# facebookresearch/multipathnet

Measured on NVIDIA H100. Metric: proposals/sec, higher is better.
Workload: dtype fp32 (wgmma split emulation, fp32 accumulate: 3 bf16 products per MAC, 2 fp16 products in fc6/fc7)

## Files before the change

### include/mpn_abi.h

```cpp
#ifndef MPN_ABI_H
#define MPN_ABI_H
#include <stdint.h>
#ifdef __cplusplus
extern "C" {
#endif

typedef struct mpn_ctx mpn_ctx;
typedef struct mpn_model mpn_model;

int mpn_ctx_create(int device, void *cuda_stream, mpn_ctx **out);
int mpn_ctx_create_stream(int device, int priority, mpn_ctx **out);
void *mpn_ctx_stream(const mpn_ctx *ctx);
int mpn_ctx_wait_ctx(mpn_ctx *ctx, mpn_ctx *other);
void mpn_ctx_destroy(mpn_ctx *ctx);
const char *mpn_last_error(const mpn_ctx *ctx);
int mpn_ctx_synchronize(mpn_ctx *ctx);
int64_t mpn_ctx_launch_count(const mpn_ctx *ctx);
const char *mpn_version(void);
int mpn_ctx_set_option(mpn_ctx *ctx, const char *name, int64_t value);
int mpn_ctx_profile_begin(mpn_ctx *ctx);
int mpn_ctx_profile_end(mpn_ctx *ctx, double *ms_by_cat, int64_t *launches_by_cat);
int mpn_ctx_timeline_begin(mpn_ctx *ctx, int32_t max_launches);
int mpn_ctx_timeline_end(mpn_ctx *ctx, uint64_t *stamps_min, uint64_t *stamps_max, int32_t *n_launches);

// ... 120 lines not shown
int mpn_model_detect_nms(mpn_model *m, const float *image, int32_t H, int32_t W,
                         const float *boxes, int64_t R, float im_scale, float W0, float H0,
                         float score_thresh, float nms_thr, float *scores, float *bboxes,
                         int32_t *keep_idx, int32_t *keep_counts);
int mpn_model_detect_nms_submit(mpn_model *m, const float *image, int32_t H, int32_t W,
                                const float *boxes, int64_t R, float im_scale, float W0, float H0,
                                float score_thresh, float nms_thr, float *scores, float *bboxes,
                                int32_t *keep_idx, int32_t *keep_counts, int32_t *ticket);
int mpn_model_detect_nms_submit_u8(mpn_model *m, const uint8_t *im_hwc, int32_t H0, int32_t W0,
                                   const mpn_image_transform *tf, double scale, double max_size, const float *boxes,
                                   int64_t R, float score_thresh, float nms_thr, float *scores, float *bboxes,
                                   int32_t *keep_idx, int32_t *keep_counts, int32_t *ticket);
int mpn_model_detect_nms_wait(mpn_model *m, int32_t ticket);
typedef struct mpn_test_opts {
  int32_t num_iter;
  int32_t use_rbox_scores;
  int32_t bbox_voting;
  float score_thresh;
  float nms_thr;
  float vote_thr;
  float vote_score_pow;
} mpn_test_opts;
int mpn_model_test_one(mpn_model *m, const float *image, int32_t H, int32_t W, const float *boxes, int64_t R,
                       float im_scale, float W0, float H0, const mpn_test_opts *opts, float *scores, float *bboxes,
                       int32_t *keep_idx, int32_t *keep_counts, float *voted);
int mpn_model_detect_nms_dev(mpn_model *m, const float *image_dev, int32_t H, int32_t W,
                             const float *boxes_dev, int64_t R, float im_scale, float W0, float H0,
                             float score_thresh, float nms_thr, float *scores_dev,
                             float *bboxes_dev, int32_t *keep_idx_dev, int32_t *keep_counts_dev);

int mpn_post_detect_dev(mpn_ctx *ctx, const float *scores_dev, const float *deltas_dev, const float *boxes_dev, int64_t R,
                        int32_t C, const float *mean4, const float *std4, float W0, float H0, float score_thresh,
                        float nms_thr, int32_t c_begin, int32_t c_end, float *bboxes_dev, int32_t *keep_idx_dev,
                        int32_t *keep_counts_dev);

enum { MPN_MAX_DET = 128, MPN_REC_FLOATS = 769, MPN_DIST_ID_BYTES = 128 };
int mpn_pack_detections_dev(mpn_ctx *ctx, const float *scores_dev, const float *bboxes_dev, int64_t R, int32_t C,
                            const int32_t *keep_idx_dev, const int32_t *keep_counts_dev, int64_t cap, int32_t top_k,
                            float *record_dev);
int mpn_pack_detections(mpn_ctx *ctx, const float *scores, const float *bboxes, int64_t R, int32_t C,
                        const int32_t *keep_idx, const int32_t *keep_counts, int64_t cap, int32_t top_k, float *record);
int mpn_select_boxes(mpn_ctx *ctx, const float *classes, const float *ys, int64_t R, int32_t C, const float *mean4,
                     const float *std4, float *out);
int mpn_select_boxes_dev(mpn_ctx *ctx, const float *classes_dev, const float *ys_dev, int64_t R, int32_t C,
                         const float *mean4, const float *std4, float *out_dev);
int mpn_model_set_detection_sink(mpn_model *m, float *records_dev, int64_t capacity, int32_t top_k);
int mpn_model_detection_sink_count(const mpn_model *m, int64_t *n_records);

int mpn_dist_unique_id(mpn_ctx *ctx, uint8_t *id);
int mpn_dist_init(mpn_ctx *ctx, const uint8_t *id, int32_t rank, int32_t world);
int mpn_dist_world(const mpn_ctx *ctx, int32_t *rank, int32_t *world);
int mpn_dist_all_gather_dev(mpn_ctx *ctx, const float *send_dev, int64_t n_floats, float *recv_dev);
int mpn_dist_all_gather(mpn_ctx *ctx, const float *send_dev, int64_t n_floats, float *recv_host);
int mpn_dist_destroy(mpn_ctx *ctx);
int mpn_dist_nccl_version(mpn_ctx *ctx, int32_t *version);

int mpn_coco_eval(mpn_ctx *ctx, int32_t n_images, const int64_t *image_ids, int32_t n_cats, const int64_t *cat_ids,
                  int64_t G, const int32_t *gt_img, const int32_t *gt_cat, const double *gt_box, const double *gt_area,
                  const int32_t *gt_crowd, int64_t D, const float *dets, double *precision, double *recall,
                  double *stats);

int mpn_model_get_pooled(mpn_model *m, int32_t tower, int64_t r0, int64_t n, float *out, int64_t capacity,
                         int64_t *R_total, int32_t *bins, int32_t *Ctot);
int mpn_model_get_trunk_slot(mpn_model *m, int32_t slot, float *out_nchw, int64_t capacity,
                             int32_t *C, int32_t *H, int32_t *W);
int mpn_model_get_slot_planes(mpn_model *m, int32_t tower, int32_t slot, int64_t r0, int64_t n, uint16_t *hi,
                              uint16_t *lo, uint8_t *q8, int32_t *e8, int64_t capacity, int32_t *fmt, int64_t *dims);
int mpn_model_get_head_outputs(mpn_model *m, float *cls_logits, float *bbox_raw, int64_t *R, int32_t *K);
int mpn_debug_detect_tail(mpn_ctx *ctx, const float *logits, int32_t K, int64_t R, int32_t C, int32_t do_softmax, const float *deltas,
                          const float *boxes, int32_t do_clamp, float W0, float H0, int32_t has_norm, const float *mean4,
                          const float *std4, float *scores, float *bboxes);
int mpn_model_set_conv_impl(mpn_model *m, int32_t impl);
int mpn_model_last_flops(const mpn_model *m, double *trunk_flops, double *head_flops);

int mpn_gemm_check(mpn_ctx *ctx, const float *A, const float *B, const float *bias, int64_t M,
                   int64_t N, int64_t K, int32_t relu, int32_t impl, float *C);
int mpn_gemm_bench(mpn_ctx *ctx, int64_t M, int64_t N, int64_t K, int32_t iters, double *ms_per_launch,
                   int32_t *bn, int32_t *cta_group, int32_t *splitk);
int mpn_linear_bench(mpn_ctx *ctx, int64_t M, int64_t N, int64_t K, int32_t w16, int32_t biasless, int32_t iters,
                     double *ms_per_launch, int32_t *bn, int32_t *splitk);
int mpn_conv_bench(mpn_ctx *ctx, int64_t N, int64_t Cin, int64_t H, int64_t W, int64_t Cout, int32_t k, int32_t stride,
                   int32_t pad, int32_t iters, double *ms_per_launch, int32_t *bn, int32_t *cta_group, int32_t *mode,
                   uint64_t *dbg16);
int mpn_debug_plan(int64_t N, int64_t Cin, int64_t H, int64_t W, int64_t Cout, int32_t k, int32_t stride, int32_t pad,
                   int32_t per_roi, int32_t sm_count, int32_t *out);
int mpn_debug_fp8(const float *h, int64_t n_samples, int64_t sample_elems, int32_t *e_out, uint8_t *q_out);
int mpn_conv_check(mpn_ctx *ctx, const float *x, int64_t N, int64_t Cin, int64_t H, int64_t W,
                   const float *w, const float *bias, int64_t Cout, int32_t kh, int32_t kw,
                   int32_t stride, int32_t pad, int32_t relu, int32_t impl, float *y);
int mpn_conv_check_view(mpn_ctx *ctx, const float *x, int64_t N, int64_t Cin, int64_t H, int64_t W, int64_t ld,
                        const float *w, const float *bias, int64_t Cout, int32_t kh, int32_t kw,
                        int32_t stride, int32_t pad, int32_t relu, int32_t impl, float *y);

typedef struct mpn_train_config {
  float lr, momentum, dampening, weight_decay;
  float dropout;
  float bbox_regression;
  uint64_t seed;
} mpn_train_config;
typedef struct mpn_train_spec {
  int32_t trunk_from;
  int32_t phase2;
  int32_t integral;
  int32_t n_fixed;
  const int32_t *fixed_weight;
  const float *const *fixed_scale;
} mpn_train_spec;
enum { MPN_OPTIM_SGD = 0, MPN_OPTIM_ADAM = 1, MPN_OPTIM_ADAMAX = 2, MPN_OPTIM_ADAGRAD = 3, MPN_OPTIM_RMSPROP = 4 };
typedef struct mpn_train_optim {
  int32_t method;
  double lr_decay, beta1, beta2, epsilon, alpha;
} mpn_train_optim;
int mpn_train_check_optim(const mpn_model_desc *d, const mpn_train_spec *s, const mpn_train_optim *o, char *msg, int32_t msg_cap);
int mpn_train_check(const mpn_model_desc *d, const mpn_train_spec *s, char *msg, int32_t msg_cap);
int mpn_model_train_begin_optim(mpn_model *m, const mpn_train_config *cfg, const mpn_train_spec *s, const mpn_train_optim *o);
int mpn_model_train_begin(mpn_model *m, const mpn_train_config *cfg, const mpn_train_spec *s);
int mpn_model_train_step(mpn_model *m, int32_t n_images, const float *const *images, const int32_t *image_hw,
                         const int32_t *rois_per_image, const float *boxes, const int32_t *labels, const float *bbox_targets,
                         float *losses);
int mpn_model_train_step_dev(mpn_model *m, int32_t n_images, const float *const *images_dev, const int32_t *image_hw,
                             const int32_t *rois_per_image, const float *boxes_dev, const int32_t *labels_dev,
                             const float *bbox_targets_dev, float *losses_dev);
int mpn_model_train_phase_ms(mpn_model *m, float *ms);
int mpn_model_train_select_head(mpn_model *m, int32_t k);
int mpn_model_train_set_lr(mpn_model *m, float lr);
int mpn_model_train_decay(mpn_model *m, float factor);
int mpn_model_train_get(mpn_model *m, int32_t weight, int32_t what, float *out, int64_t capacity);
int mpn_model_train_dropout_mask(mpn_model *m, int32_t tower, int32_t layer, uint8_t *out, int64_t capacity, int64_t *n_out);
int mpn_model_train_relu_gate(mpn_model *m, int32_t tower, int32_t layer, uint8_t *out, int64_t capacity, int64_t *n_out);
int mpn_model_train_outputs(mpn_model *m, float *cls_logits, float *bbox_deltas);
int mpn_model_train_trunk_slot(mpn_model *m, int32_t image, int32_t slot, float *out_nchw, int64_t capacity, int32_t *C,
                               int32_t *H, int32_t *W);
int mpn_debug_roi_backward_nhwc(mpn_ctx *ctx, const uint16_t *hi, const uint16_t *lo, int32_t H, int32_t W, int32_t C, const float *rois,
                                int64_t R, int32_t PW, int32_t PH, float scale, int32_t variant, const float *grad_out, float *grad);
int mpn_debug_pool_backward(mpn_ctx *ctx, const uint16_t *y_hi, const uint16_t *y_lo, int32_t H, int32_t W, int32_t C, const float *grad_pool,
                            float *grad);
int mpn_debug_conv_backward(mpn_ctx *ctx, int32_t n_images, const int32_t *image_hw, int32_t cin, int32_t cout, int32_t k, int32_t stride,
                            const uint16_t *x_hi, const uint16_t *x_lo, const float *g, const float *w, float *dw, float *dx);
int mpn_model_train_end(mpn_model *m);
int mpn_debug_dropout(uint64_t seed, uint32_t step, int32_t tower, int32_t layer, uint64_t elem0, int64_t n, float p, uint8_t *out);
int mpn_debug_criteria(const float *x, const float *d, const int32_t *labels, const float *t, int64_t R, int32_t C, float bbox_w,
                       float *gx, float *gd, float *losses);
int mpn_debug_sgd(float *w, const float *g, float *buf, int64_t n, float lr, float momentum, float dampening, float wd, int32_t first);
int mpn_debug_optim(float *w, const float *g, float *s1, float *s2, const float *a, int64_t n, const mpn_train_optim *o, float lr,
                    float momentum, float dampening, float wd, int64_t t);

typedef struct mpn_roidb mpn_roidb;
int mpn_roidb_create(mpn_ctx *ctx, int32_t n_images, const int64_t *ann_off, const double *ann_xywh, const double *ann_area,
                     const int32_t *ann_class, const int32_t *ann_flags, double min_area, const int64_t *prop_off,
                     const float *prop_box, const float *prop_score, int32_t best_number, double min_proposal_area,
                     int32_t num_classes, int32_t n_sets, const float *thresholds, mpn_roidb **out);
void mpn_roidb_destroy(mpn_roidb *db);
int mpn_roidb_counts(mpn_roidb *db, int32_t *counts, int64_t *n_rows);
int mpn_roidb_image_rows(mpn_roidb *db, int32_t image, float *boxes, float *overlap, int32_t *corr, int32_t *label, int64_t capacity,
                         int64_t *n_rows, int32_t *n_gt);
int mpn_roidb_list(mpn_roidb *db, int32_t set, int32_t kind, int32_t image, int32_t *rows, int64_t capacity, int64_t *n_out);
int mpn_roidb_regression_stats(mpn_roidb *db, int32_t set, int32_t n_first, float *mean, float *std_);
int mpn_sample_plan(const int32_t *n_bg, const int32_t *n_fg, int32_t n_images, uint64_t seed, uint32_t step, int32_t set, int32_t n_slots,
                    int32_t *image, int32_t *bg_src, int32_t *fg_src, int32_t *flip);
int mpn_integral_set(uint64_t seed, uint32_t step, int32_t n_sets, int32_t *set);
int mpn_train_images_size(int32_t H0, int32_t W0, double scale, double max_size, int32_t *h, int32_t *w, double *im_scale);
int mpn_roidb_sample_dev(mpn_roidb *db, int32_t set, uint64_t seed, uint32_t step, int32_t n_slots, const int32_t *bg_src,
                         const int32_t *fg_src, const int32_t *flip, const double *im_scale, const int32_t *width, int32_t bg_each,
                         int32_t fg_each, const float *mean, const float *std_, int32_t num_classes, float *boxes_dev,
                         int32_t *labels_dev, float *targets_dev, int32_t *rois_per_image);
int mpn_roidb_sample(mpn_roidb *db, int32_t set, uint64_t seed, uint32_t step, int32_t n_slots, const int32_t *plan,
// ... 32 lines not shown
```

### multipathnet_b200/_lib.py

```python
from __future__ import annotations

import ctypes as C
import os
from dataclasses import dataclass, field
from typing import List, Optional, Sequence

import numpy as np

_HERE = os.path.dirname(os.path.abspath(__file__))
LIB_PATH = os.path.join(_HERE, "libmpn_b200.so")
HEADER_PATH = os.path.join(os.path.dirname(_HERE), "include", "mpn_abi.h")

MPN_LAYER_CONV, MPN_LAYER_MAXPOOL, MPN_LAYER_AVGPOOL, MPN_LAYER_FLATTEN = 1, 2, 3, 4
MPN_MAX_DET, MPN_REC_FLOATS, MPN_DIST_ID_BYTES = 128, 769, 128
MPN_LAYER_LRN = 5


class MpnError(RuntimeError):
    pass


class CLayer(C.Structure):
    _fields_ = [(n, C.c_int32) for n in (
        "kind", "in_slot", "out_slot", "cin", "cout", "kh", "kw", "stride", "pad", "relu",
# ... 95 lines not shown
    "mpn_bbox_norm_dev": (C.c_int, [_vp, _vp, C.c_int64, C.c_int64, _vp, _vp]),
    "mpn_bbox_decode": (C.c_int, [_vp, _vp, _vp, C.c_int64, C.c_int64, _vp]),
    "mpn_roi_pool": (C.c_int, [_vp, _vp, C.c_int64, C.c_int64, C.c_int64, C.c_int64, _vp, C.c_int64,
                               C.c_int32, C.c_int32, C.c_float, C.c_int32, _vp, _vp]),
    "mpn_roi_pool_dev": (C.c_int, [_vp, _vp, C.c_int64, C.c_int64, C.c_int64, C.c_int64, _vp, C.c_int64,
                                   C.c_int32, C.c_int32, C.c_float, C.c_int32, _vp, _vp]),
    "mpn_roi_pool_backward": (C.c_int, [_vp, _vp, _vp, C.c_int64, C.c_int64, C.c_int64, C.c_int64, _vp, C.c_int64,
                                        C.c_int32, C.c_int32, C.c_float, C.c_int32, _vp]),
    "mpn_roi_pool_backward_dev": (C.c_int, [_vp, _vp, _vp, C.c_int64, C.c_int64, C.c_int64, C.c_int64, _vp, C.c_int64,
                                            C.c_int32, C.c_int32, C.c_float, C.c_int32, _vp]),
    "mpn_get_images_size": (C.c_int, [C.c_int32, C.c_int32, C.c_double, C.c_double, _i32p, _i32p, C.POINTER(C.c_double)]),
    "mpn_get_images": (C.c_int, [_vp, _vp, C.c_int32, C.c_int32, _vp, C.c_int32, C.c_int32, _vp]),
    "mpn_get_images_dev": (C.c_int, [_vp, _vp, C.c_int32, C.c_int32, _vp, C.c_int32, C.c_int32, _vp]),
    "mpn_get_images_u8": (C.c_int, [_vp, _vp, C.c_int32, C.c_int32, _vp, C.c_int32, C.c_int32, _vp]),
    "mpn_get_images_u8_dev": (C.c_int, [_vp, _vp, C.c_int32, C.c_int32, _vp, C.c_int32, C.c_int32, _vp]),
    "mpn_get_images_u8_flip": (C.c_int, [_vp, _vp, C.c_int32, C.c_int32, _vp, C.c_int32, C.c_int32, C.c_int32, _vp]),
    "mpn_get_images_u8_flip_dev": (C.c_int, [_vp, _vp, C.c_int32, C.c_int32, _vp, C.c_int32, C.c_int32, C.c_int32, _vp]),
    "mpn_roidb_create": (C.c_int, [_vp, C.c_int32, _vp, _vp, _vp, _vp, _vp, C.c_double, _vp, _vp, _vp, C.c_int32, C.c_double,
                                   C.c_int32, C.c_int32, _vp, C.POINTER(_vp)]),
    "mpn_roidb_destroy": (None, [_vp]),
    "mpn_roidb_counts": (C.c_int, [_vp, _vp, _i64p]),
    "mpn_roidb_image_rows": (C.c_int, [_vp, C.c_int32, _vp, _vp, _vp, _vp, C.c_int64, _i64p, _i32p]),
    "mpn_roidb_list": (C.c_int, [_vp, C.c_int32, C.c_int32, C.c_int32, _vp, C.c_int64, _i64p]),
    "mpn_roidb_regression_stats": (C.c_int, [_vp, C.c_int32, C.c_int32, _vp, _vp]),
    "mpn_sample_plan": (C.c_int, [_vp, _vp, C.c_int32, C.c_uint64, C.c_uint32, C.c_int32, C.c_int32, _vp, _vp, _vp, _vp]),
    "mpn_integral_set": (C.c_int, [C.c_uint64, C.c_uint32, C.c_int32, _i32p]),
    "mpn_train_images_size": (C.c_int, [C.c_int32, C.c_int32, C.c_double, C.c_double, _i32p, _i32p, C.POINTER(C.c_double)]),
    "mpn_roidb_sample_dev": (C.c_int, [_vp, C.c_int32, C.c_uint64, C.c_uint32, C.c_int32, _vp, _vp, _vp, _vp, _vp, C.c_int32, C.c_int32,
                                       _vp, _vp, C.c_int32, _vp, _vp, _vp, _vp]),
    "mpn_roidb_sample": (C.c_int, [_vp, C.c_int32, C.c_uint64, C.c_uint32, C.c_int32, _vp, _vp, _vp, _vp, C.c_double, C.c_double,
                                   C.c_int32, C.c_int32, _vp, _vp, C.c_int32, _vp, _vp]),
    "mpn_roidb_batch_host": (C.c_int, [_vp, _vp, _vp, _vp, _vp]),
    "mpn_model_train_step_batch": (C.c_int, [_vp, _vp, _vp]),
    "mpn_debug_attach_proposals": (C.c_int, [C.c_int64, _vp, _vp, _vp, _vp, C.c_double, C.c_int64, _vp, _vp, C.c_int32, C.c_double,
                                             C.c_int32, _vp, _vp, _vp, _vp, C.c_int64, _i64p, _i32p]),
    "mpn_debug_sample_rows": (C.c_int, [C.c_int64, _vp, _vp, _vp, C.c_double, C.c_int32, C.c_int32, _vp, _vp, C.c_int32, _vp, _vp]),
    "mpn_model_detect_nms_submit_u8": (C.c_int, [_vp, _vp, C.c_int32, C.c_int32, _vp, C.c_double, C.c_double, _vp, C.c_int64, C.c_float, C.c_float,
                                                 _vp, _vp, _vp, _vp, _i32p]),
    "mpn_model_trunk_image": (C.c_int, [_vp, _vp, C.c_int32, C.c_int32, _vp, C.c_double, C.c_double, C.POINTER(C.c_double), _i32p, _i32p]),
    "mpn_model_create": (C.c_int, [_vp, C.POINTER(CModelDesc), C.POINTER(_vp), _i64p, C.c_int32, C.POINTER(_vp)]),
    "mpn_model_destroy": (None, [_vp]),
    "mpn_model_trunk": (C.c_int, [_vp, _vp, C.c_int32, C.c_int32]),
    "mpn_model_trunk_dev": (C.c_int, [_vp, _vp, C.c_int32, C.c_int32]),
    "mpn_model_heads": (C.c_int, [_vp, _vp, C.c_int64, _vp, _vp]),
    "mpn_model_heads_dev": (C.c_int, [_vp, _vp, C.c_int64, _vp, _vp]),
    "mpn_model_detect": (C.c_int, [_vp, _vp, C.c_int32, C.c_int32, _vp, C.c_int64, C.c_float, C.c_int32, _vp, _vp]),
    "mpn_model_detect_nms": (C.c_int, [_vp, _vp, C.c_int32, C.c_int32, _vp, C.c_int64, C.c_float, C.c_float,
                                       C.c_float, C.c_float, C.c_float, _vp, _vp, _vp, _vp]),
    "mpn_model_detect_nms_submit": (C.c_int, [_vp, _vp, C.c_int32, C.c_int32, _vp, C.c_int64, C.c_float, C.c_float,
                                              C.c_float, C.c_float, C.c_float, _vp, _vp, _vp, _vp, _i32p]),
    "mpn_model_detect_nms_wait": (C.c_int, [_vp, C.c_int32]),
    "mpn_model_test_one": (C.c_int, [_vp, _vp, C.c_int32, C.c_int32, _vp, C.c_int64, C.c_float, C.c_float, C.c_float, C.POINTER(CTestOpts),
                                     _vp, _vp, _vp, _vp, _vp]),
    "mpn_model_detect_nms_dev": (C.c_int, [_vp, _vp, C.c_int32, C.c_int32, _vp, C.c_int64, C.c_float, C.c_float,
                                           C.c_float, C.c_float, C.c_float, _vp, _vp, _vp, _vp]),
    "mpn_post_detect_dev": (C.c_int, [_vp, _vp, _vp, _vp, C.c_int64, C.c_int32, _vp, _vp, C.c_float, C.c_float, C.c_float, C.c_float,
                                      C.c_int32, C.c_int32, _vp, _vp, _vp]),
    "mpn_pack_detections_dev": (C.c_int, [_vp, _vp, _vp, C.c_int64, C.c_int32, _vp, _vp, C.c_int64, C.c_int32, _vp]),
    "mpn_pack_detections": (C.c_int, [_vp, _vp, _vp, C.c_int64, C.c_int32, _vp, _vp, C.c_int64, C.c_int32, _vp]),
    "mpn_select_boxes": (C.c_int, [_vp, _vp, _vp, C.c_int64, C.c_int32, _vp, _vp, _vp]),
    "mpn_select_boxes_dev": (C.c_int, [_vp, _vp, _vp, C.c_int64, C.c_int32, _vp, _vp, _vp]),
    "mpn_model_set_detection_sink": (C.c_int, [_vp, _vp, C.c_int64, C.c_int32]),
    "mpn_model_detection_sink_count": (C.c_int, [_vp, _i64p]),
    "mpn_dist_unique_id": (C.c_int, [_vp, _vp]),
    "mpn_dist_init": (C.c_int, [_vp, _vp, C.c_int32, C.c_int32]),
    "mpn_dist_world": (C.c_int, [_vp, _i32p, _i32p]),
    "mpn_dist_all_gather_dev": (C.c_int, [_vp, _vp, C.c_int64, _vp]),
    "mpn_dist_all_gather": (C.c_int, [_vp, _vp, C.c_int64, _vp]),
    "mpn_dist_destroy": (C.c_int, [_vp]),
    "mpn_dist_nccl_version": (C.c_int, [_vp, _i32p]),
    "mpn_coco_eval": (C.c_int, [_vp, C.c_int32, _vp, C.c_int32, _vp, C.c_int64, _vp, _vp, _vp, _vp, _vp, C.c_int64, _vp, _vp, _vp, _vp]),
    "mpn_model_get_pooled":(C.c_int, [_vp, C.c_int32, C.c_int64, C.c_int64, _vp, C.c_int64, _i64p, _i32p, _i32p]),
    "mpn_model_get_trunk_slot": (C.c_int, [_vp, C.c_int32, _vp, C.c_int64, _i32p, _i32p, _i32p]),
    "mpn_model_get_slot_planes": (C.c_int, [_vp, C.c_int32, C.c_int32, C.c_int64, C.c_int64, _vp, _vp, _vp, _vp, C.c_int64, _i32p, _i64p]),
    "mpn_model_get_head_outputs": (C.c_int, [_vp, _vp, _vp, _i64p, _i32p]),
    "mpn_debug_detect_tail": (C.c_int, [_vp, _vp, C.c_int32, C.c_int64, C.c_int32, C.c_int32, _vp, _vp, C.c_int32, C.c_float, C.c_float,
                                        C.c_int32, _vp, _vp, _vp, _vp]),
    "mpn_model_set_conv_impl": (C.c_int, [_vp, C.c_int32]),
    "mpn_model_last_flops": (C.c_int, [_vp, C.POINTER(C.c_double), C.POINTER(C.c_double)]),
    "mpn_gemm_bench": (C.c_int, [_vp, C.c_int64, C.c_int64, C.c_int64, C.c_int32, C.POINTER(C.c_double), _i32p, _i32p, _i32p]),
    "mpn_linear_bench": (C.c_int, [_vp, C.c_int64, C.c_int64, C.c_int64, C.c_int32, C.c_int32, C.c_int32, C.POINTER(C.c_double), _i32p, _i32p]),
    "mpn_conv_bench": (C.c_int, [_vp, C.c_int64, C.c_int64, C.c_int64, C.c_int64, C.c_int64, C.c_int32, C.c_int32, C.c_int32, C.c_int32,
                                 C.POINTER(C.c_double), _i32p, _i32p, _i32p, C.POINTER(C.c_uint64)]),
    "mpn_debug_plan": (C.c_int, [C.c_int64, C.c_int64, C.c_int64, C.c_int64, C.c_int64, C.c_int32, C.c_int32, C.c_int32, C.c_int32, C.c_int32, _i32p]),
    "mpn_debug_fp8": (C.c_int, [_vp, C.c_int64, C.c_int64, _vp, _vp]),
    "mpn_gemm_check": (C.c_int, [_vp, _vp, _vp, _vp, C.c_int64, C.c_int64, C.c_int64, C.c_int32, C.c_int32, _vp]),
    "mpn_conv_check": (C.c_int, [_vp, _vp, C.c_int64, C.c_int64, C.c_int64, C.c_int64, _vp, _vp, C.c_int64,
                                 C.c_int32, C.c_int32, C.c_int32, C.c_int32, C.c_int32, C.c_int32, _vp]),
    "mpn_conv_check_view": (C.c_int, [_vp, _vp, C.c_int64, C.c_int64, C.c_int64, C.c_int64, C.c_int64, _vp, _vp, C.c_int64,
                                      C.c_int32, C.c_int32, C.c_int32, C.c_int32, C.c_int32, C.c_int32, _vp]),
    "mpn_train_check": (C.c_int, [C.POINTER(CModelDesc), C.POINTER(CTrainSpec), C.c_char_p, C.c_int32]),
    "mpn_model_train_begin": (C.c_int, [_vp, C.POINTER(CTrainConfig), C.POINTER(CTrainSpec)]),
    "mpn_train_check_optim": (C.c_int, [C.POINTER(CModelDesc), C.POINTER(CTrainSpec), C.POINTER(CTrainOptim), C.c_char_p, C.c_int32]),
    "mpn_model_train_begin_optim": (C.c_int, [_vp, C.POINTER(CTrainConfig), C.POINTER(CTrainSpec), C.POINTER(CTrainOptim)]),
    "mpn_model_train_step": (C.c_int, [_vp, C.c_int32, C.POINTER(_vp), _i32p, _i32p, _vp, _vp, _vp, _vp]),
    "mpn_model_train_step_dev": (C.c_int, [_vp, C.c_int32, C.POINTER(_vp), _i32p, _i32p, _vp, _vp, _vp, _vp]),
    "mpn_model_train_phase_ms": (C.c_int, [_vp, _f32p]),
    "mpn_model_train_select_head": (C.c_int, [_vp, C.c_int32]),
    "mpn_model_train_set_lr": (C.c_int, [_vp, C.c_float]),
    "mpn_model_train_decay": (C.c_int, [_vp, C.c_float]),
    "mpn_model_train_get": (C.c_int, [_vp, C.c_int32, C.c_int32, _vp, C.c_int64]),
    "mpn_model_train_dropout_mask": (C.c_int, [_vp, C.c_int32, C.c_int32, _vp, C.c_int64, _i64p]),
    "mpn_model_train_relu_gate": (C.c_int, [_vp, C.c_int32, C.c_int32, _vp, C.c_int64, _i64p]),
    "mpn_model_train_outputs": (C.c_int, [_vp, _vp, _vp]),
    "mpn_model_train_trunk_slot": (C.c_int, [_vp, C.c_int32, C.c_int32, _vp, C.c_int64, _i32p, _i32p, _i32p]),
    "mpn_model_train_end": (C.c_int, [_vp]),
    "mpn_debug_roi_backward_nhwc": (C.c_int, [_vp, _vp, _vp, C.c_int32, C.c_int32, C.c_int32, _vp, C.c_int64, C.c_int32, C.c_int32, C.c_float,
                                              C.c_int32, _vp, _vp]),
    "mpn_model_train_phase2": (C.c_int, [_vp, C.c_float]),
    "mpn_model_train_set": (C.c_int, [_vp, C.c_int32, C.c_int32, _vp, C.c_int64]),
    "mpn_model_train_get_state": (C.c_int, [_vp, C.POINTER(CTrainState)]),
    "mpn_model_train_set_state": (C.c_int, [_vp, C.POINTER(CTrainState)]),
    "mpn_debug_roi_backward_jobs": (C.c_int, [_vp, _vp, _vp, C.c_int32, C.c_int32, C.c_int32, _vp, C.c_int64, C.c_int32, C.c_int32, C.c_int32,
                                              C.c_int32, _i32p, _f32p, _i32p, _i64p, _i32p, C.POINTER(_vp), _vp, _vp, _vp]),
    "mpn_debug_pool_backward": (C.c_int, [_vp, _vp, _vp, C.c_int32, C.c_int32, C.c_int32, _vp, _vp]),
    "mpn_debug_conv_backward": (C.c_int, [_vp, C.c_int32, _i32p, C.c_int32, C.c_int32, C.c_int32, C.c_int32, _vp, _vp, _vp, _vp, _vp,
                                          _vp]),
    "mpn_debug_dropout": (C.c_int, [C.c_uint64, C.c_uint32, C.c_int32, C.c_int32, C.c_uint64, C.c_int64, C.c_float, _vp]),
    "mpn_debug_criteria": (C.c_int, [_vp, _vp, _vp, _vp, C.c_int64, C.c_int32, C.c_float, _vp, _vp, _vp]),
    "mpn_debug_sgd": (C.c_int, [_vp, _vp, _vp, C.c_int64, C.c_float, C.c_float, C.c_float, C.c_float, C.c_int32]),
    "mpn_debug_optim": (C.c_int, [_vp, _vp, _vp, _vp, _vp, C.c_int64, C.POINTER(CTrainOptim), C.c_float, C.c_float, C.c_float, C.c_float,
                                  C.c_int64]),
}

_lib = None


def load_library():
    global _lib
    if _lib is not None:
        return _lib
    if not os.path.exists(LIB_PATH):
        raise MpnError(
            f"{LIB_PATH} is missing: build it with `make` (or `python -c 'import __graft_entry__ as g; g.build()'`). "
            "There is no CPU or PyTorch fallback for this path.")
    lib = C.CDLL(LIB_PATH)
    for name, (res, args) in SIGNATURES.items():
        fn = getattr(lib, name)
        fn.restype = res
        fn.argtypes = args
    _lib = lib
    return lib


def _ptr(a) -> Optional[int]:
    if a is None:
        return None
    if isinstance(a, int):
        return a
    if isinstance(a, np.ndarray):
        return a.ctypes.data
    if hasattr(a, "data_ptr"):
        return a.data_ptr()
    raise TypeError(f"cannot take the address of {type(a)}")


def _f32(a) -> np.ndarray:
    return np.ascontiguousarray(a, dtype=np.float32)


class Context:

    def __init__(self, device: int = 0, stream: Optional[int] = None, own_stream: bool = False, priority: int = 0):
        self.lib = load_library()
        h = _vp()
        if own_stream:
# ... 166 lines not shown
        out = np.empty((3, h.value, w.value), np.float32)
        tf = CImageTransform.of(kind)
        self.check(self.lib.mpn_get_images(self.h, _ptr(im), im.shape[1], im.shape[2], C.addressof(tf), h.value, w.value, _ptr(out)),
                   "mpn_get_images")
        return out, float(s.value)

    def get_images_u8(self, im_hwc_u8, kind: str, scale: float = 600, max_size: float = 1000):
        im = np.ascontiguousarray(im_hwc_u8, dtype=np.uint8)
        if im.ndim != 3 or im.shape[2] != 3:
            raise ValueError("expected an H x W x 3 uint8 image")
        h, w, s = C.c_int32(), C.c_int32(), C.c_double()
        self.check(self.lib.mpn_get_images_size(im.shape[0], im.shape[1], float(scale), float(max_size), C.byref(h), C.byref(w), C.byref(s)),
                   "mpn_get_images_size")
        out = np.empty((3, h.value, w.value), np.float32)
        tf = CImageTransform.of(kind)
        self.check(self.lib.mpn_get_images_u8(self.h, _ptr(im), im.shape[0], im.shape[1], C.addressof(tf), h.value, w.value, _ptr(out)),
                   "mpn_get_images_u8")
        return out, float(s.value)

    def bbox_norm(self, deltas, mean, std) -> np.ndarray:
        d = _f32(deltas).copy()
        m, s = _f32(mean).reshape(4), _f32(std).reshape(4)
        self.check(self.lib.mpn_bbox_norm(self.h, _ptr(d), d.shape[0], d.shape[1], _ptr(m), _ptr(s)), "mpn_bbox_norm")
        return d

    def bbox_decode(self, deltas, boxes) -> np.ndarray:
        d, b = _f32(deltas), _f32(boxes)
        out = np.empty_like(d)
        self.check(self.lib.mpn_bbox_decode(self.h, _ptr(d), _ptr(b), d.shape[0], d.shape[1] // 4, _ptr(out)), "mpn_bbox_decode")
        return out

    def roi_pool(self, fmap, rois, pw: int, ph: int, scale: float, variant: int = 2, with_argmax: bool = False):
        f, r = _f32(fmap), _f32(rois)
        n, c, h, w = f.shape
        out = np.empty((r.shape[0], c, ph, pw), dtype=np.float32)
        am = np.empty(out.shape, dtype=np.int32) if with_argmax else None
        self.check(self.lib.mpn_roi_pool(self.h, _ptr(f), n, c, h, w, _ptr(r), r.shape[0], pw, ph, float(scale), variant,
                                         _ptr(out), _ptr(am)), "mpn_roi_pool")
        return (out, am) if with_argmax else out

    def roi_pool_backward(self, grad_out, argmax, rois, data_shape, pw: int, ph: int, scale: float, variant: int = 2) -> np.ndarray:
        g, r = _f32(grad_out), _f32(rois)
        am = np.ascontiguousarray(argmax, dtype=np.int32)
        n, c, h, w = (int(s) for s in data_shape)
        if g.shape != (r.shape[0], c, ph, pw) or am.shape != g.shape:
            raise ValueError(f"grad_out and argmax must be {(r.shape[0], c, ph, pw)}, got {g.shape} and {am.shape}")
        out = np.empty((n, c, h, w), dtype=np.float32)
        self.check(self.lib.mpn_roi_pool_backward(self.h, _ptr(g), _ptr(am), n, c, h, w, _ptr(r), r.shape[0], pw, ph, float(scale),
                                                  variant, _ptr(out)), "mpn_roi_pool_backward")
        return out

    def roi_pool_backward_dev(self, grad_out_dev, argmax_dev, N: int, C_: int, H: int, W: int, rois_dev, R: int, pw: int, ph: int,
                              scale: float, variant: int, grad_data_dev):
        self.check(self.lib.mpn_roi_pool_backward_dev(self.h, _ptr(grad_out_dev), _ptr(argmax_dev), int(N), int(C_), int(H), int(W),
                                                      _ptr(rois_dev), int(R), int(pw), int(ph), float(scale), int(variant),
                                                      _ptr(grad_data_dev)), "mpn_roi_pool_backward_dev")

    def gemm_check(self, A, B, bias=None, relu=False, impl=0) -> np.ndarray:
        A, B = _f32(A), _f32(B)
        m, k = A.shape
        n = B.shape[0]
        bias = None if bias is None else _f32(bias)
        out = np.empty((m, n), dtype=np.float32)
        self.check(self.lib.mpn_gemm_check(self.h, _ptr(A), _ptr(B), _ptr(bias), m, n, k, int(relu), impl, _ptr(out)), "mpn_gemm_check")
        return out

    def gemm_bench(self, M, N, K, iters=20):
        ms = C.c_double(); bn = C.c_int32(); cg = C.c_int32(); sk = C.c_int32()
        self.check(self.lib.mpn_gemm_bench(self.h, M, N, K, iters, C.byref(ms), C.byref(bn), C.byref(cg), C.byref(sk)), "mpn_gemm_bench")
        return ms.value, bn.value, cg.value, sk.value

    def linear_bench(self, M, N, K, w16=False, biasless=False, iters=20):
        ms = C.c_double(); bn = C.c_int32(); sk = C.c_int32()
        self.check(self.lib.mpn_linear_bench(self.h, M, N, K, int(w16), int(biasless), iters, C.byref(ms), C.byref(bn), C.byref(sk)),
                   "mpn_linear_bench")
        return ms.value, bn.value, sk.value

    def conv_bench(self, N, Cin, H, W, Cout, k=3, stride=1, pad=1, iters=20):
        ms = C.c_double(); bn = C.c_int32(); cg = C.c_int32(); mode = C.c_int32(); dbg = (C.c_uint64 * 16)()
        self.check(self.lib.mpn_conv_bench(self.h, N, Cin, H, W, Cout, k, stride, pad, iters, C.byref(ms), C.byref(bn), C.byref(cg),
                                           C.byref(mode), dbg), "mpn_conv_bench")
        return ms.value, bn.value, cg.value, mode.value, [int(x) for x in dbg]

    def conv_check(self, x, w, bias=None, stride=1, pad=0, relu=False, impl=0) -> np.ndarray:
        x, w = _f32(x), _f32(w)
        n, cin, h, ww = x.shape
        cout, _, kh, kw = w.shape
        bias = None if bias is None else _f32(bias)
        ho, wo = (h + 2 * pad - kh) // stride + 1, (ww + 2 * pad - kw) // stride + 1
        y = np.empty((n, cout, ho, wo), dtype=np.float32)
        self.check(self.lib.mpn_conv_check(self.h, _ptr(x), n, cin, h, ww, _ptr(w), _ptr(bias), cout, kh, kw, stride, pad,
                                           int(relu), impl, _ptr(y)), "mpn_conv_check")
        return y

    def conv_check_view(self, x, w, ld, bias=None, stride=1, pad=0, relu=False, impl=0) -> np.ndarray:
        x, w = _f32(x), _f32(w)
        n, cin, h, ww = x.shape
        cout, _, kh, kw = w.shape
        bias = None if bias is None else _f32(bias)
        ho, wo = (h + 2 * pad - kh) // stride + 1, (ww + 2 * pad - kw) // stride + 1
        y = np.empty((n, cout, ho, wo), dtype=np.float32)
        self.check(self.lib.mpn_conv_check_view(self.h, _ptr(x), n, cin, h, ww, int(ld), _ptr(w), _ptr(bias), cout, kh, kw, stride,
                                                pad, int(relu), impl, _ptr(y)), "mpn_conv_check_view")
        return y


@dataclass
class Layer:
    kind: int
    in_slot: int
    out_slot: int
    cin: int = 0
    cout: int = 0
    kh: int = 1
    kw: int = 1
    stride: int = 1
    pad: int = 0
    relu: int = 0
    residual_slot: int = -1
    ceil_mode: int = 0
    weight: int = -1
    bias: int = -1
    groups: int = 1

    def to_c(self) -> CLayer:
        if self.groups != 1 or self.kind == MPN_LAYER_LRN:
            raise MpnError("grouped convolution / LRN (CaffeNet, BASELINE configs[0]) is the CPU plumbing configuration; "
                           "it is not part of the GPU path")
        return CLayer(self.kind, self.in_slot, self.out_slot, self.cin, self.cout, self.kh, self.kw, self.stride,
                      self.pad, self.relu, self.residual_slot, self.ceil_mode, self.weight, self.bias)


@dataclass
class Tower:
    region: int
    levels: List[tuple]
    pooled_w: int
    pooled_h: int
    normalize: int
    layers: List[Layer]
    out_slot: int


@dataclass
class Head:
    col_begin: int
    col_len: int
    cout: int
    weight: int
    bias: int

    def to_c(self) -> CHead:
        return CHead(self.col_begin, self.col_len, self.cout, self.weight, self.bias)


@dataclass
class ModelSpec:
    name: str
    trunk_layers: List[Layer]
    towers: List[Tower]
    cls_heads: List[Head]
    bbox_head: Head
    num_classes: int
    weights: List[np.ndarray]
    roi_variant: int = 2
    no_softmax: int = 0
# ... 242 lines not shown
```

### multipathnet_b200/csrc/abi.cu

```cuda
#include "conv_gemm.cuh"
#include "roi.cuh"
#include <algorithm>
#include <mutex>

int mpn_nms_launch(mpn_ctx *, const float *, int, int, const int32_t *, const int32_t *, float, int32_t *, int32_t *);
int mpn_nms_dense_launch(mpn_ctx *, const float *, int, float, int32_t *, int32_t *);
int mpn_bbox_vote_launch(mpn_ctx *, const float *, int, const float *, int, float, float *);
int mpn_pack_detections_launch(mpn_ctx *, const float *, const float *, int, const int32_t *, const int32_t *, int, int, float *);
int mpn_gather_scored_range_launch(mpn_ctx *, const float *, const float *, int, int, int, int, float, float *, int32_t *, int32_t *);
int mpn_bbox_norm_decode_launch(mpn_ctx *, const float *, const float *, int64_t, int, int, float, float, float *, const float *, const float *);
int mpn_detect_tail_launch(mpn_ctx *, const float *, int64_t, int, int, int, float *, const float *, const float *, int, float, float,
                           float *, int, const float *, const float *);
int mpn_select_boxes_launch(mpn_ctx *, const float *, const float *, int64_t, int, const float *, const float *, float *);
int mpn_foveal_launch(mpn_ctx *, const float *, int64_t, float *);
int mpn_context_region_launch(mpn_ctx *, const float *, int64_t, float, float *);
int mpn_get_images_launch(mpn_ctx *, const float *, int32_t, int32_t, const mpn_image_transform *, int32_t, int32_t, float *);
int mpn_get_images_size_impl(int32_t, int32_t, double, double, int32_t *, int32_t *, double *);
int mpn_get_images_u8_launch(mpn_ctx *, const uint8_t *, int32_t, int32_t, const mpn_image_transform *, int32_t, int32_t, float *);
int mpn_get_images_u8_flip_launch(mpn_ctx *, const uint8_t *, int32_t, int32_t, const mpn_image_transform *, int32_t, int32_t, int32_t, float *);
int mpn_bbox_norm_launch(mpn_ctx *, float *, int64_t, int64_t, const float *, const float *);
int mpn_bbox_decode_launch(mpn_ctx *, const float *, const float *, int64_t, int, int, float, float, float *);
int mpn_split_rows_launch(mpn_ctx *, const float *, int64_t, int64_t, int64_t, __nv_bfloat16 *, __nv_bfloat16 *, int64_t);
int mpn_nchw_to_nhwc_split_launch(mpn_ctx *, const float *, int, int, int, int, DTensor &);
int mpn_nhwc_split_to_nchw_launch(mpn_ctx *, const DTensor &, float *);
// ... 725 lines not shown
  MPN_CUDA(ctx, cudaMemsetAsync(a.at<char>(o_bh), 0x3c, 2 * nb, ctx->stream));
  MPN_CUDA(ctx, cudaMemsetAsync(a.at<char>(o_bl), 0x30, 2 * nb, ctx->stream));
  ConvProblem p;
  p.x.hi = a.at<__nv_bfloat16>(o_ah); p.x.lo = a.at<__nv_bfloat16>(o_al); p.x.N = M; p.x.H = 1; p.x.W = 1; p.x.C = K; p.x.ld = K;
  p.w_hi = a.at<__nv_bfloat16>(o_bh); p.w_lo = a.at<__nv_bfloat16>(o_bl); p.Cout = (int)N; p.relu = 1;
  p.bf16 = ctx->opt_bf16 == 1 ? 1 : 0;
  p.m_invariant = per_roi; p.fill_split = fill_split;
  if (w16) {
    MPN_CHECK_ARG(ctx, !p.bf16, "the bf16 numerics do not take an fp16 weight plane");
    p.x.fmt = 1; p.w16 = p.w_hi; p.w16_inv_scale = 1.f; p.w_hi = p.w_lo = nullptr;
  }
  const int64_t Npad = (N + 7) / 8 * 8;
  (void)Npad;
  if (N % 8 == 0) { p.y.hi = a.at<__nv_bfloat16>(o_ch); p.y.lo = a.at<__nv_bfloat16>(o_cl); }
  else { p.y.f32 = a.at<float>(o_ch); }
  p.y.N = M; p.y.H = 1; p.y.W = 1; p.y.C = N; p.y.ld = N; p.y_f32_ld = N;
  if (!(N % 8 == 0)) MPN_CHECK_ARG(ctx, 4 * nc <= 2 * (2 * nc + 64), "internal");
  ConvPlan pl;
  MPN_TRY(conv_tc_plan(ctx, p, pl));
  if (bn) *bn = pl.BN; if (cta_group) *cta_group = 1; if (splitk) *splitk = pl.splitk;
  for (int i = 0; i < 3; ++i) MPN_TRY(conv_tc_launch(ctx, p, pl));
  cudaEvent_t e0, e1;
  MPN_CUDA(ctx, cudaEventCreate(&e0)); MPN_CUDA(ctx, cudaEventCreate(&e1));
  MPN_CUDA(ctx, cudaEventRecord(e0, ctx->stream));
  for (int i = 0; i < iters; ++i) MPN_TRY(conv_tc_launch(ctx, p, pl));
  MPN_CUDA(ctx, cudaEventRecord(e1, ctx->stream));
  MPN_CUDA(ctx, cudaEventSynchronize(e1));
  float ms = 0.f;
  MPN_CUDA(ctx, cudaEventElapsedTime(&ms, e0, e1));
  cudaEventDestroy(e0); cudaEventDestroy(e1);
  *ms_per_launch = (double)ms / iters;
  return MPN_OK;
}

int mpn_gemm_bench(mpn_ctx *ctx, int64_t M, int64_t N, int64_t K, int32_t iters, double *ms_per_launch, int32_t *bn,
                   int32_t *cta_group, int32_t *splitk) {
  return gemm_bench_impl(ctx, M, N, K, 0, 0, 0, iters, ms_per_launch, bn, cta_group, splitk);
}

int mpn_linear_bench(mpn_ctx *ctx, int64_t M, int64_t N, int64_t K, int32_t w16, int32_t biasless, int32_t iters,
                     double *ms_per_launch, int32_t *bn, int32_t *splitk) {
  return gemm_bench_impl(ctx, M, N, K, 1, w16 ? 1 : 0, biasless ? 1 : 0, iters, ms_per_launch, bn, nullptr, splitk);
}

int mpn_conv_bench(mpn_ctx *ctx, int64_t N, int64_t Cin, int64_t H, int64_t W, int64_t Cout, int32_t k, int32_t stride,
                   int32_t pad, int32_t iters, double *ms_per_launch, int32_t *bn, int32_t *cta_group, int32_t *mode,
                   uint64_t *dbg16) {
  if (!ctx) return MPN_ERR_ARG;
  MPN_CUDA(ctx, cudaSetDevice(ctx->device));
  MPN_CHECK_ARG(ctx, N > 0 && Cin % 8 == 0 && Cout % 8 == 0 && iters > 0 && ms_per_launch, "bad arguments");
  const int64_t Ho = (H + 2 * pad - k) / stride + 1, Wo = (W + 2 * pad - k) / stride + 1;
  const size_t nx = (size_t)(N * H * W * Cin), nw = (size_t)(Cout * conv_k_pad(Cin) * k * k), ny = (size_t)(N * Ho * Wo * Cout);
  Arena a{ctx};
  size_t o_xh = a.reserve(2 * nx), o_xl = a.reserve(2 * nx), o_wh = a.reserve(2 * nw), o_wl = a.reserve(2 * nw),
         o_yh = a.reserve(2 * ny), o_yl = a.reserve(2 * ny);
  MPN_TRY(a.commit());
  MPN_CUDA(ctx, cudaMemsetAsync(a.at<char>(o_xh), 0x3c, 2 * nx, ctx->stream));
  MPN_CUDA(ctx, cudaMemsetAsync(a.at<char>(o_xl), 0x30, 2 * nx, ctx->stream));
  MPN_CUDA(ctx, cudaMemsetAsync(a.at<char>(o_wh), 0x3c, 2 * nw, ctx->stream));
  MPN_CUDA(ctx, cudaMemsetAsync(a.at<char>(o_wl), 0x30, 2 * nw, ctx->stream));
  ConvProblem p;
  p.x.hi = a.at<__nv_bfloat16>(o_xh); p.x.lo = a.at<__nv_bfloat16>(o_xl); p.x.N = N; p.x.H = H; p.x.W = W; p.x.C = Cin; p.x.ld = Cin;
  p.w_hi = a.at<__nv_bfloat16>(o_wh); p.w_lo = a.at<__nv_bfloat16>(o_wl); p.Cout = (int)Cout; p.kh = k; p.kw = k; p.stride = stride; p.pad = pad; p.relu = 1;
  p.bf16 = ctx->opt_bf16 == 1 ? 1 : 0;
  p.y.hi = a.at<__nv_bfloat16>(o_yh); p.y.lo = a.at<__nv_bfloat16>(o_yl); p.y.N = N; p.y.H = Ho; p.y.W = Wo; p.y.C = Cout; p.y.ld = Cout;
  ConvPlan pl;
  MPN_TRY(conv_tc_plan(ctx, p, pl));
  if (bn) *bn = pl.BN; if (cta_group) *cta_group = 1; if (mode) *mode = pl.mode;
  for (int i = 0; i < 3; ++i) MPN_TRY(conv_tc_launch(ctx, p, pl));
  cudaEvent_t e0, e1;
  MPN_CUDA(ctx, cudaEventCreate(&e0)); MPN_CUDA(ctx, cudaEventCreate(&e1));
  MPN_CUDA(ctx, cudaEventRecord(e0, ctx->stream));
  for (int i = 0; i < iters; ++i) MPN_TRY(conv_tc_launch(ctx, p, pl));
  MPN_CUDA(ctx, cudaEventRecord(e1, ctx->stream));
  MPN_CUDA(ctx, cudaEventSynchronize(e1));
  float ms = 0.f;
  MPN_CUDA(ctx, cudaEventElapsedTime(&ms, e0, e1));
  cudaEventDestroy(e0); cudaEventDestroy(e1);
  *ms_per_launch = (double)ms / iters;
  if (dbg16) memset(dbg16, 0, 128);
  return MPN_OK;
}

int mpn_gemm_check(mpn_ctx *ctx, const float *A, const float *B, const float *bias, int64_t M, int64_t N, int64_t K,
                   int32_t relu, int32_t impl, float *C) {
  if (!ctx) return MPN_ERR_ARG;
  MPN_CUDA(ctx, cudaSetDevice(ctx->device));
  MPN_CHECK_ARG(ctx, A && B && C && M > 0 && N > 0 && K > 0, "bad arguments");
  MPN_CHECK_ARG(ctx, !(ctx->opt_fp8 == 1 && ctx->opt_bf16 == 1), "the \"fp8\" and \"bf16\" options are both on");
  const size_t na = (size_t)(M * K), nb = (size_t)(N * K), nc = (size_t)(M * N);
  const int64_t Kp = conv_k_pad(K);
  const size_t nbp = (size_t)(N * Kp);
  Arena a{ctx};
  size_t o_a = a.reserve(4 * na), o_b = a.reserve(4 * nb), o_bias = a.reserve(4 * (size_t)N), o_c = a.reserve(4 * nc),
         o_ah = a.reserve(2 * na), o_al = a.reserve(2 * na), o_bh = a.reserve(2 * nbp), o_bl = a.reserve(2 * nbp),
         o_a8 = a.reserve(na), o_ae = a.reserve(4 * (size_t)M), o_b8 = a.reserve(nbp), o_be = a.reserve(4 * (size_t)(N + 127) / 128 * 128);
  MPN_TRY(a.commit());
  MPN_CUDA(ctx, cudaMemcpyAsync(a.at<float>(o_a), A, 4 * na, cudaMemcpyHostToDevice, ctx->stream));
  MPN_CUDA(ctx, cudaMemcpyAsync(a.at<float>(o_b), B, 4 * nb, cudaMemcpyHostToDevice, ctx->stream));
  if (bias) MPN_CUDA(ctx, cudaMemcpyAsync(a.at<float>(o_bias), bias, 4 * (size_t)N, cudaMemcpyHostToDevice, ctx->stream));
  MPN_TRY(mpn_split_rows_launch(ctx, a.at<float>(o_a), M, K, K, a.at<__nv_bfloat16>(o_ah), a.at<__nv_bfloat16>(o_al), K));
  if (Kp != K) {
    MPN_CUDA(ctx, cudaMemsetAsync(a.at<__nv_bfloat16>(o_bh), 0, 2 * nbp, ctx->stream));
    MPN_CUDA(ctx, cudaMemsetAsync(a.at<__nv_bfloat16>(o_bl), 0, 2 * nbp, ctx->stream));
  }
  MPN_TRY(mpn_split_rows_launch(ctx, a.at<float>(o_b), N, K, K, a.at<__nv_bfloat16>(o_bh), a.at<__nv_bfloat16>(o_bl), Kp));
  ConvProblem p;
  p.x.hi = a.at<__nv_bfloat16>(o_ah); p.x.lo = a.at<__nv_bfloat16>(o_al); p.x.N = M; p.x.H = 1; p.x.W = 1; p.x.C = K; p.x.ld = K;
  p.w_hi = a.at<__nv_bfloat16>(o_bh); p.w_lo = a.at<__nv_bfloat16>(o_bl); p.bias = bias ? a.at<float>(o_bias) : nullptr;
  p.Cout = (int)N; p.relu = relu; p.bf16 = ctx->opt_bf16 == 1 ? 1 : 0;
  p.m_invariant = 1;
  p.y.f32 = a.at<float>(o_c); p.y.N = M; p.y.H = 1; p.y.W = 1; p.y.C = N; p.y.ld = N; p.y_f32_ld = N;
  if (ctx->opt_fp8 == 1 && impl != 2) {
    p.fp8 = 1;
    p.x8 = a.at<uint8_t>(o_a8); p.x8_exp = a.at<int>(o_ae); p.w8 = a.at<uint8_t>(o_b8); p.w8_exp = a.at<int>(o_be);
    MPN_TRY(mpn_fp8_quantize_launch(ctx, p.x, a.at<uint8_t>(o_a8), a.at<int>(o_ae)));
    MPN_TRY(mpn_fp8_weight_launch(ctx, p.w_hi, N, Kp, (N + 127) / 128 * 128, a.at<uint8_t>(o_b8), a.at<int>(o_be)));
  }
  if (impl == 1) { MPN_TRY(conv_ref_launch(ctx, p)); }
  else {
    if (impl == 2) {
      float amax = 0.f;
      MPN_TRY(mpn_absmax(ctx, a.at<float>(o_b), (int64_t)nb, &amax));
      int e = 0;
      if (amax > 0.f) { (void)frexpf(amax, &e); e = 14 - e; }
      const float sc = ldexpf(1.0f, e);
      MPN_TRY(mpn_weight_permute_half_launch(ctx, a.at<float>(o_b), N, (int)K, 1, 1, sc, a.at<void>(o_bh)));
      p.w16 = a.at<void>(o_bh); p.w16_inv_scale = 1.0f / sc; p.w_hi = p.w_lo = nullptr;
      MPN_TRY(mpn_split_rows_f16_launch(ctx, a.at<float>(o_a), M, K, K, a.at<__nv_bfloat16>(o_ah), a.at<__nv_bfloat16>(o_al), K));
      p.x.fmt = 1; p.bf16 = 0;
    }
    ConvPlan pl; MPN_TRY(conv_tc_plan(ctx, p, pl)); MPN_TRY(conv_tc_launch(ctx, p, pl));
  }
  MPN_CUDA(ctx, cudaMemcpyAsync(C, a.at<float>(o_c), 4 * nc, cudaMemcpyDeviceToHost, ctx->stream));
  if (ctx->opt_fp8 == 1) MPN_TRY(mpn_ovf_copy_async(ctx, ctx->stream));
  MPN_CUDA(ctx, cudaStreamSynchronize(ctx->stream));
  return ctx->opt_fp8 == 1 ? mpn_ovf_test(ctx) : MPN_OK;
}

}
```

### multipathnet_b200/csrc/conv_gemm.cuh

```cuda
#pragma once
#include "common.cuh"
#include <cuda.h>

struct OutSeg { int c0, c1; float *ptr; long long ld; };
struct OutScatter { int n = 0; OutSeg seg[8]; };

enum class OperandScheme : int { BF16X3 = 0, FP16X2 = 1, BF16X1 = 2, FP8X1 = 3 };

struct ConvProblem {
  DTensor x;
  const __nv_bfloat16 *w_hi = nullptr, *w_lo = nullptr;
  const float *bias = nullptr;
  int Cout = 0, kh = 1, kw = 1, stride = 1, pad = 0;
  int relu = 0;
  DTensor res;
  DTensor y;
  int64_t y_f32_ld = 0;
  DTensor pool;
  int pool_only = 0;
  int m_invariant = 0;
  const void *w16 = nullptr; float w16_inv_scale = 1.f;
  int bf16 = 0;
  int fp8 = 0;
  const uint8_t *x8 = nullptr; const int *x8_exp = nullptr;
  const uint8_t *w8 = nullptr; const int *w8_exp = nullptr;
  OutScatter scatter;
  int wide_k_split = 0;
  int fill_split = 0;
};

struct ConvPlan {
  CUtensorMap tmA_hi, tmA_lo, tmB_hi, tmB_lo;
  int BN = 0;
  int tn = 0, th = 0, tw = 0;
  int tiles_img = 0, tiles_h = 0, tiles_w = 0, tiles_n = 0;
  int splitk = 1, kb_per_split = 0;
  int mode = 0;
  int flat = 0;
  OperandScheme ops = OperandScheme::BF16X3;
  int valid = 0;
};

int conv_tc_plan(mpn_ctx *ctx, const ConvProblem &p, ConvPlan &plan);
int conv_tc_launch(mpn_ctx *ctx, const ConvProblem &p, const ConvPlan &plan);
int conv_ref_launch(mpn_ctx *ctx, const ConvProblem &p);
int conv_direct_nchw_launch(mpn_ctx *ctx, const float *x_nchw, int N, int Cin, int H, int W, const float *w,
                            const float *bias, int Cout, int kh, int kw, int stride, int pad, int relu,
                            DTensor &y, const float *w_host = nullptr, const float *bias_host = nullptr);
int conv1_tc_launch(mpn_ctx *ctx, const float *x_nchw, int N, int H, int W, const float *w_dev, const float *bias_dev, int relu,
                    DTensor &y);
double conv_flops(const ConvProblem &p);
int mpn_fp8_quantize_launch(mpn_ctx *ctx, const DTensor &x, uint8_t *q8, int *exps);
int mpn_fp8_weight_launch(mpn_ctx *ctx, const __nv_bfloat16 *w_hi, int64_t rows, int64_t K, int64_t rows_pad, uint8_t *q8, int *exps);
```

### multipathnet_b200/csrc/gemm_tc.cu

```cuda
#include "conv_gemm.cuh"
#include "wgmma.cuh"
#include "fp8_e4m3.cuh"
#include <algorithm>
#include <stdlib.h>
#include <string.h>

namespace {

constexpr int BM = 128;
constexpr int BK = 64;
constexpr int TC_THREADS = 384;
constexpr int CONS_THREADS = 256;
constexpr int A_TILE_BYTES = BM * BK * 2;
constexpr int SMEM_BUDGET = 196608;

__host__ __device__ constexpr int a_planes(OperandScheme ops) { return (ops == OperandScheme::BF16X1 || ops == OperandScheme::FP8X1) ? 1 : 2; }
__host__ __device__ constexpr int b_planes(OperandScheme ops) { return ops == OperandScheme::BF16X3 ? 2 : 1; }
__host__ __device__ constexpr int elem_bytes(OperandScheme ops) { return ops == OperandScheme::FP8X1 ? 1 : 2; }
__host__ __device__ constexpr int row_bytes(int BN, OperandScheme ops) { return (ops == OperandScheme::FP8X1 || BN == 256) ? 64 : 128; }
__host__ __device__ constexpr int stage_k(int BN, OperandScheme ops) { return row_bytes(BN, ops) / elem_bytes(ops); }
__host__ __device__ constexpr int kb_steps(int BN, OperandScheme ops) { return BK / stage_k(BN, ops); }
__host__ __device__ constexpr int a_tile_bytes(int BN, OperandScheme ops) { return BM * row_bytes(BN, ops); }
__host__ __device__ constexpr int stage_bytes(int BN, OperandScheme ops = OperandScheme::BF16X3) {
  return (a_planes(ops) * BM + b_planes(ops) * BN) * row_bytes(BN, ops);
// ... 375 lines not shown
        const int s = it % S; const uint32_t ph = (uint32_t)(it / S) & 1u;
        mbar_wait(full_bar(s), ph);
        if (it == 0 && e == 0) tl_min_stamp(p.tl_min, 2);
        const uint32_t sa = smem_base + (uint32_t)s * STAGE;
        auto desc = [](uint32_t a) { return row_bytes(BN, OPS) == 64 ? make_smem_desc_64b(a) : make_smem_desc(a); };
        const uint64_t a_hi = desc(sa + (uint32_t)g * (A_TILE / 2));
        const uint64_t a_lo = desc(sa + A_TILE + (uint32_t)g * (A_TILE / 2));
        const uint64_t b_hi = desc(sa + B_OFF);
        const uint64_t b_lo = desc(sa + B_OFF + B_TILE_BYTES);
        wgmma_fence_acc(acc);
        wgmma_fence();
        mma_kstep<BN, OPS>(acc, a_hi, a_lo, b_hi, b_lo, i == 0);
        wgmma_commit();
        wgmma_wait<1>();
        wgmma_fence_acc(acc);
        if (i > 0 && lane == 0) mbar_arrive(empty_bar((it - 1) % S));
      }
      wgmma_wait<0>();
      wgmma_fence_acc(acc);
      if (lane == 0) mbar_arrive(empty_bar((it - 1) % S));
    }
    if (e == 0) tl_max_stamp(p.tl_max, 0);
    const uint32_t t_epi = (p.tl_max && e == 0) ? (uint32_t)gtimer() : 0u;
    tile_epilogue<BN, OPS>(p, u, acc, g, wq, lane, so);
    if (e == 0) {
      tl_max_stamp(p.tl_max, 1);
      if (p.tl_max) atomicAdd(p.tl_max + 3, (unsigned long long)((uint32_t)gtimer() - t_epi));
    }
  }
}


constexpr int C1_THREADS = 256;
constexpr int C1_A_BYTES = 2 * A_TILE_BYTES;
constexpr int C1_B_BYTES = 2 * 64 * 128;
constexpr int C1_OUT_WARP = 16 * 128;
constexpr int C1_SMEM = 2 * C1_A_BYTES + C1_B_BYTES + (C1_THREADS / 32) * C1_OUT_WARP + 1024;

__device__ __forceinline__ void conv1_gather(const float *__restrict__ x, int pix, int pixels, int H, int W, int bhalf,
                                             float (&in)[16]) {
#pragma unroll
  for (int k = 0; k < 16; ++k) in[k] = 0.f;
  if (pix < pixels) {
    const int HW = H * W;
    const int n = pix / HW, rem = pix - n * HW;
    const int ho = rem / W, wo = rem - ho * W;
    const float *x0 = x + ((size_t)n * 3 * HW + (size_t)(ho - 1) * W + (wo - 1));
    const bool rok[3] = {ho >= 1, true, ho + 1 < H}, cok[3] = {wo >= 1, true, wo + 1 < W};
#pragma unroll
    for (int k = 0; k < 16; ++k) {
      const int kk = 16 * bhalf + k;
      if (kk < 27) {
        const int ci = kk / 9, r = (kk / 3) % 3, q = kk % 3;
        in[k] = (rok[r] && cok[q]) ? __ldg(x0 + ci * HW + r * W + q) : 0.f;
      }
    }
  }
}

__device__ __forceinline__ void conv1_store_plane(uint32_t so, const uint32_t (&v)[16], __nv_bfloat16 *out, int pix0,
                                                  int pixels, int lane) {
  const int r = lane >> 2;
  const uint32_t wr = so + (uint32_t)(r * 128 + 4 * (lane & 3));
  __syncwarp();
#pragma unroll
  for (int j = 0; j < 8; ++j) {
    const uint32_t a = wr + (uint32_t)((j ^ r) * 16);
    asm volatile("st.shared.b32 [%0], %1;" ::"r"(a), "r"(v[j]) : "memory");
    asm volatile("st.shared.b32 [%0], %1;" ::"r"(a + 8 * 128), "r"(v[8 + j]) : "memory");
  }
  __syncwarp();
  const int row0 = lane >> 3, ch = lane & 7;
  const uint32_t rd0 = so + (uint32_t)(row0 * 128 + ((ch ^ row0) * 16)), rd1 = so + (uint32_t)(row0 * 128 + ((ch ^ row0 ^ 4) * 16));
  __nv_bfloat16 *o = out + (size_t)(pix0 + row0) * 64 + ch * 8;
#pragma unroll
  for (int q = 0; q < 4; ++q) {
    uint4 d;
    asm volatile("ld.shared.v4.b32 {%0, %1, %2, %3}, [%4];" : "=r"(d.x), "=r"(d.y), "=r"(d.z), "=r"(d.w)
                 : "r"(((q & 1) ? rd1 : rd0) + (uint32_t)(q * 4 * 128)) : "memory");
    if (pix0 + row0 + 4 * q < pixels) *reinterpret_cast<uint4 *>(o + q * 4 * 64) = d;
  }
}

__global__ void __launch_bounds__(C1_THREADS, 2)
conv1_tc_kernel(const float *__restrict__ x, int N, int H, int W, const float *__restrict__ w, const float *__restrict__ bias,
                int relu, __nv_bfloat16 *__restrict__ out_hi, __nv_bfloat16 *__restrict__ out_lo) {
  extern __shared__ uint8_t smem_raw[];
  uint8_t *smem = reinterpret_cast<uint8_t *>((reinterpret_cast<uintptr_t>(smem_raw) + 1023) & ~(uintptr_t)1023);
  uint8_t *sB = smem + 2 * C1_A_BYTES;
  const int tid = threadIdx.x, lane = tid & 31, warp = tid >> 5;
  const uint32_t so = smem_u32(sB + C1_B_BYTES) + (uint32_t)(warp * C1_OUT_WARP);
  const uint32_t b_base = smem_u32(sB);
  const int g = tid >> 7;
  const int pixels = N * H * W;
  const int total_tiles = (pixels + BM - 1) / BM;
  asm volatile("griddepcontrol.wait;" ::: "memory");
  asm volatile("griddepcontrol.launch_dependents;" ::: "memory");
  const int c0 = 2 * (lane & 3);
  for (int i = tid; i < 64 * 4; i += C1_THREADS) {
    const int row = i >> 2, j = i & 3;
    uint32_t hh[4], ll[4];
#pragma unroll
    for (int q = 0; q < 4; ++q) {
      const int k0 = j * 8 + 2 * q;
      const float v0 = (k0 < 27) ? __ldg(w + row * 27 + k0) : 0.f, v1 = (k0 + 1 < 27) ? __ldg(w + row * 27 + k0 + 1) : 0.f;
      split_bf16x2(v0, v1, hh[q], ll[q]);
    }
    const uint32_t off = (uint32_t)row * 128u + (uint32_t)((j ^ (row & 7)) * 16);
    *reinterpret_cast<uint4 *>(sB + off) = make_uint4(hh[0], hh[1], hh[2], hh[3]);
    *reinterpret_cast<uint4 *>(sB + 64 * 128 + off) = make_uint4(ll[0], ll[1], ll[2], ll[3]);
  }
  const int brow = tid & 127, bhalf = tid >> 7;
  float in[16];
  conv1_gather(x, (int)blockIdx.x * BM + brow, pixels, H, W, bhalf, in);
  for (int tile = blockIdx.x, it = 0; tile < total_tiles; tile += gridDim.x, ++it) {
    uint8_t *sa = smem + (it & 1) * C1_A_BYTES;
    uint8_t *pa = sa + (size_t)brow * 128;
#pragma unroll
    for (int jj = 0; jj < 2; ++jj) {
      const int j = 2 * bhalf + jj;
      uint32_t hh[4], ll[4];
#pragma unroll
      for (int q = 0; q < 4; ++q) split_bf16x2(in[jj * 8 + 2 * q], in[jj * 8 + 2 * q + 1], hh[q], ll[q]);
      const int pj = (j ^ (brow & 7)) * 16;
      *reinterpret_cast<uint4 *>(pa + pj) = make_uint4(hh[0], hh[1], hh[2], hh[3]);
      *reinterpret_cast<uint4 *>(pa + A_TILE_BYTES + pj) = make_uint4(ll[0], ll[1], ll[2], ll[3]);
    }
    asm volatile("fence.proxy.async.shared::cta;" ::: "memory");
    __syncthreads();
    float acc[32];
#pragma unroll
    for (int i = 0; i < 32; ++i) acc[i] = 0.f;
    const uint32_t a_base = smem_u32(sa);
    const uint64_t a_hi = make_smem_desc(a_base + (uint32_t)g * (A_TILE_BYTES / 2));
    const uint64_t a_lo = make_smem_desc(a_base + A_TILE_BYTES + (uint32_t)g * (A_TILE_BYTES / 2));
    const uint64_t b_hi = make_smem_desc(b_base), b_lo = make_smem_desc(b_base + 64 * 128);
    wgmma_fence_acc(acc);
    wgmma_fence();
#pragma unroll
    for (int k = 0; k < 2; ++k) {
      const uint64_t adv = (uint64_t)((k * 16 * 2) >> 4);
      wgmma_nk16<64, false>(acc, a_lo + adv, b_hi + adv, k ? 1u : 0u);
      wgmma_nk16<64, false>(acc, a_hi + adv, b_lo + adv, 1u);
      wgmma_nk16<64, false>(acc, a_hi + adv, b_hi + adv, 1u);
    }
    wgmma_commit();
    const int next = tile + (int)gridDim.x;
    conv1_gather(x, next < total_tiles ? next * BM + brow : pixels, pixels, H, W, bhalf, in);
    wgmma_wait<0>();
    wgmma_fence_acc(acc);
#pragma unroll
    for (int j = 0; j < 8; ++j) {
      const float2 b = __ldg(reinterpret_cast<const float2 *>(bias + 8 * j + c0));
#pragma unroll
      for (int h = 0; h < 2; ++h) {
        float &f0 = acc[4 * j + 2 * h], &f1 = acc[4 * j + 2 * h + 1];
        f0 += b.x; f1 += b.y;
        if (relu) { f0 = fmaxf(f0, 0.f); f1 = fmaxf(f1, 0.f); }
      }
    }
    const int pix0 = tile * BM + 64 * g + 16 * (warp & 3);
#pragma unroll 1
    for (int plane = 0; plane < 2; ++plane) {
      uint32_t v[16];
#pragma unroll
      for (int j = 0; j < 8; ++j)
#pragma unroll
        for (int h = 0; h < 2; ++h) {
          uint32_t hi2, lo2;
          split_bf16x2(acc[4 * j + 2 * h], acc[4 * j + 2 * h + 1], hi2, lo2);
          v[8 * h + j] = plane ? lo2 : hi2;
        }
      conv1_store_plane(so, v, plane ? out_lo : out_hi, pix0, pixels, lane);
    }
  }
}

struct ReduceParams {
  const float *ws; long long split_stride; int splitk; long long pixels; int Cout;
  const float *bias; const __nv_bfloat16 *res_hi, *res_lo; long long res_ld; int relu;
  __nv_bfloat16 *out_hi, *out_lo; long long out_ld; float *out_f32; long long out_f32_ld;
  OutScatter scatter;
};
__global__ void __launch_bounds__(256) splitk_reduce_kernel(const ReduceParams r) {
  MPN_PDL_SYNC();
  const long long idx = (long long)blockIdx.x * blockDim.x + threadIdx.x;
  if (idx >= r.pixels * r.Cout) return;
  const long long pix = idx / r.Cout; const int c = (int)(idx - pix * r.Cout);
  float acc = 0.f;
  for (int s = 0; s < r.splitk; ++s) acc += r.ws[(long long)s * r.split_stride + idx];
  if (r.bias) acc += __ldg(r.bias + c);
  if (r.res_hi) acc += join_bf16(r.res_hi[pix * r.res_ld + c], r.res_lo[pix * r.res_ld + c]);
  if (r.relu) acc = fmaxf(acc, 0.f);
  if (r.out_hi) { __nv_bfloat16 h, l; split_bf16(acc, h, l); r.out_hi[pix * r.out_ld + c] = h; r.out_lo[pix * r.out_ld + c] = l; }
  if (r.scatter.n > 0) {
#pragma unroll 1
    for (int g = 0; g < r.scatter.n; ++g)
      if (c >= r.scatter.seg[g].c0 && c < r.scatter.seg[g].c1) { r.scatter.seg[g].ptr[pix * r.scatter.seg[g].ld + (c - r.scatter.seg[g].c0)] = acc; break; }
  } else if (r.out_f32) r.out_f32[pix * r.out_f32_ld + c] = acc;
}

typedef CUresult (*PFN_encodeTiled)(CUtensorMap *, CUtensorMapDataType, cuuint32_t, void *, const cuuint64_t *,
                                    const cuuint64_t *, const cuuint32_t *, const cuuint32_t *, CUtensorMapInterleave,
                                    CUtensorMapSwizzle, CUtensorMapL2promotion, CUtensorMapFloatOOBfill);
PFN_encodeTiled get_encode_fn() {
  static PFN_encodeTiled fn = nullptr;
  if (!fn) {
    void *p = nullptr; cudaDriverEntryPointQueryResult q;
    if (cudaGetDriverEntryPoint("cuTensorMapEncodeTiled", &p, cudaEnableDefault, &q) == cudaSuccess &&
        q == cudaDriverEntryPointSuccess)
      fn = reinterpret_cast<PFN_encodeTiled>(p);
  }
  return fn;
}

int encode_map(mpn_ctx *ctx, CUtensorMap *tm, const void *base, int rank, const cuuint64_t *dims,
               const cuuint64_t *strides_bytes , const cuuint32_t *box, const cuuint32_t *estr, int BN, OperandScheme ops) {
  const bool fp8 = ops == OperandScheme::FP8X1;
  PFN_encodeTiled fn = get_encode_fn();
  if (!fn) return mpn_fail(ctx, MPN_ERR_CUDA, "cuTensorMapEncodeTiled entry point unavailable");
  CUresult r = fn(tm, fp8 ? CU_TENSOR_MAP_DATA_TYPE_UINT8 : CU_TENSOR_MAP_DATA_TYPE_BFLOAT16, (cuuint32_t)rank, const_cast<void *>(base), dims,
                  strides_bytes, box, estr, CU_TENSOR_MAP_INTERLEAVE_NONE, row_bytes(BN, ops) == 64 ? CU_TENSOR_MAP_SWIZZLE_64B : CU_TENSOR_MAP_SWIZZLE_128B,
                  CU_TENSOR_MAP_L2_PROMOTION_L2_256B, CU_TENSOR_MAP_FLOAT_OOB_FILL_NONE);
  if (r != CUDA_SUCCESS) {
    char b[256];
    snprintf(b, sizeof b, "cuTensorMapEncodeTiled failed (%d): rank %d dims %llu %llu box %u %u", (int)r, rank,
             (unsigned long long)dims[0], (unsigned long long)dims[1], box[0], box[1]);
    return mpn_fail(ctx, MPN_ERR_CUDA, b);
  }
  return MPN_OK;
}

inline bool tc_use_pdl() {
  static const int on = [] { const char *e = getenv("MPN_TC_PDL"); return (e && e[0] == '0') ? 0 : 1; }();
  return on != 0;
}

template <int BN, OperandScheme OPS = OperandScheme::BF16X3>
int launch_bn(mpn_ctx *ctx, const ConvPlan &pl, const TcParams &tp) {
  const int smem = tc_smem_bytes(BN, OPS);
  constexpr int bslot = BN == 256 ? 2 : (BN == 128 ? 1 : 0);
  constexpr int slot = OPS == OperandScheme::FP16X2 ? 3 : (OPS == OperandScheme::BF16X1 ? 5 + bslot
                                                         : (OPS == OperandScheme::FP8X1 ? 8 + bslot : bslot));
  if (!ctx->tc_attr_set[slot]) {
    MPN_CUDA(ctx, cudaFuncSetAttribute(conv_gemm_tc_kernel<BN, OPS>, cudaFuncAttributeMaxDynamicSharedMemorySize, smem));
    ctx->tc_attr_set[slot] = 1;
  }
  const long long units = (long long)pl.tiles_img * pl.tiles_h * pl.tiles_w * pl.tiles_n * pl.splitk;
  MPN_CHECK_ARG(ctx, units > 0 && units < (1ll << 31), "conv_tc: grid size out of range");
  TcParams tpu = tp;
  tpu.units = (int)units;
  cudaLaunchConfig_t cfg = {};
  cfg.gridDim = dim3((unsigned)std::min<long long>(units, ctx->sm_count));
  cfg.blockDim = dim3(TC_THREADS); cfg.dynamicSmemBytes = (size_t)smem; cfg.stream = ctx->stream;
  cudaLaunchAttribute attr[1];
  int na = 0;
  if (tc_use_pdl()) {
    attr[na].id = cudaLaunchAttributeProgrammaticStreamSerialization;
    attr[na].val.programmaticStreamSerializationAllowed = 1;
    ++na;
  }
  cfg.attrs = attr; cfg.numAttrs = na;
  MPN_CUDA(ctx, cudaLaunchKernelEx(&cfg, conv_gemm_tc_kernel<BN, OPS>, pl.tmA_hi, pl.tmA_lo, pl.tmB_hi, pl.tmB_lo, tpu));
  MPN_LAUNCHED(ctx);
  return MPN_OK;
}

int launch_ops(mpn_ctx *ctx, const ConvPlan &pl, const TcParams &tp) {
  if (pl.ops == OperandScheme::FP16X2) return launch_bn<256, OperandScheme::FP16X2>(ctx, pl, tp);
  if (pl.ops == OperandScheme::FP8X1)
    return pl.BN == 128 ? launch_bn<128, OperandScheme::FP8X1>(ctx, pl, tp) : launch_bn<64, OperandScheme::FP8X1>(ctx, pl, tp);
  if (pl.ops == OperandScheme::BF16X1) {
    switch (pl.BN) {
      case 256: return launch_bn<256, OperandScheme::BF16X1>(ctx, pl, tp);
      case 128: return launch_bn<128, OperandScheme::BF16X1>(ctx, pl, tp);
      default: return launch_bn<64, OperandScheme::BF16X1>(ctx, pl, tp);
    }
  }
  switch (pl.BN) {
    case 256: return launch_bn<256>(ctx, pl, tp);
    case 128: return launch_bn<128>(ctx, pl, tp);
    default: return launch_bn<64>(ctx, pl, tp);
  }
}

}

int conv1_tc_launch(mpn_ctx *ctx, const float *x_nchw, int N, int H, int W, const float *w_dev, const float *bias_dev, int relu,
                    DTensor &y) {
  MPN_CHECK_ARG(ctx, y.hi && y.lo && y.C == 64 && y.ld % 8 == 0, "conv1_tc: output must be 64-channel split planes");
  MPN_CHECK_ARG(ctx, bias_dev, "conv1_tc: bias missing");
  MPN_CHECK_ARG(ctx, y.ld == 64 && (long long)N * H * W < (1ll << 31) - 256, "conv1_tc: dense 64-channel output and < 2^31 pixels");
  if (!ctx->tc_attr_set[4]) {
    MPN_CUDA(ctx, cudaFuncSetAttribute(conv1_tc_kernel, cudaFuncAttributeMaxDynamicSharedMemorySize, C1_SMEM));
    ctx->tc_attr_set[4] = 1;
  }
  const long long tiles = ((long long)N * H * W + BM - 1) / BM;
  cudaLaunchConfig_t cfg = {};
  cfg.gridDim = dim3((unsigned)std::min<long long>(tiles, 2ll * ctx->sm_count)); cfg.blockDim = dim3(C1_THREADS);
  cfg.dynamicSmemBytes = (size_t)C1_SMEM; cfg.stream = ctx->stream;
  cudaLaunchAttribute attr[1];
  int na = 0;
  if (tc_use_pdl()) { attr[na].id = cudaLaunchAttributeProgrammaticStreamSerialization; attr[na].val.programmaticStreamSerializationAllowed = 1; ++na; }
  cfg.attrs = attr; cfg.numAttrs = na;
  MPN_CUDA(ctx, cudaLaunchKernelEx(&cfg, conv1_tc_kernel, x_nchw, N, H, W, w_dev, bias_dev, relu, y.hi, y.lo));
  MPN_LAUNCHED(ctx);
  return MPN_OK;
}

double conv_flops(const ConvProblem &p) {
  const double Ho = (double)p.y.H, Wo = (double)p.y.W;
  return 2.0 * (double)p.x.C * p.Cout * p.kh * p.kw * Ho * Wo * (double)p.y.N;
}

static int conv_tc_plan_impl(mpn_ctx *ctx, int sm_count, const ConvProblem &p, ConvPlan &pl, bool choose_only) {
  pl.valid = 0;
  MPN_CHECK_ARG(ctx, choose_only || (p.x.hi && (p.x.lo || p.bf16) && ((p.w_hi && (p.w_lo || p.bf16)) || p.w16)),
                "conv_tc: operands must be split-bf16 (or an fp16 weight plane)");
  MPN_CHECK_ARG(ctx, !(p.w16 && p.bf16), "conv_tc: the bf16 numerics do not take an fp16 weight plane");
  MPN_CHECK_ARG(ctx, !(p.fp8 && (p.w16 || p.bf16)), "conv_tc: the fp8 numerics take neither an fp16 weight plane nor the bf16 numerics");
  MPN_CHECK_ARG(ctx, choose_only || !p.fp8 || (p.x8 && p.x8_exp && p.w8 && p.w8_exp), "conv_tc: the fp8 numerics need e4m3 planes and exponents");
  pl.ops = p.w16 ? OperandScheme::FP16X2 : (p.fp8 ? OperandScheme::FP8X1 : (p.bf16 ? OperandScheme::BF16X1 : OperandScheme::BF16X3));
  const bool w16 = pl.ops == OperandScheme::FP16X2, fp8 = pl.ops == OperandScheme::FP8X1;
  MPN_CHECK_ARG(ctx, choose_only || (p.x.fmt == 1) == w16, "conv_tc: fp16 activation planes go with the fp16 weight plane (and only with it)");
  MPN_CHECK_ARG(ctx, p.x.C % 8 == 0, "conv_tc: Cin must be a multiple of 8");
  MPN_CHECK_ARG(ctx, !fp8 || p.x.C % BK == 0, "conv_tc: the fp8 numerics need Cin a multiple of 64 (their quantizer groups are 64 channels wide)");
  MPN_CHECK_ARG(ctx, !w16 || p.x.C % BK == 0, "conv_tc: the fp16-weight path needs Cin a multiple of 64");
  const int cblocks = (int)(conv_k_pad(p.x.C) / BK);
  MPN_CHECK_ARG(ctx, p.x.ld % 8 == 0, "conv_tc: input pixel stride must be a multiple of 8 elements");
  MPN_CHECK_ARG(ctx, p.stride >= 1 && p.stride <= 2, "conv_tc: stride must be 1 or 2");
  const int Ho = (int)p.y.H, Wo = (int)p.y.W, N = (int)p.y.N;
  pl.flat = (p.kh == 1 && p.kw == 1 && p.stride == 1 && p.pad == 0) ? 1 : 0;
  pl.mode = 0; pl.splitk = 1;
  cuuint64_t dims[4], strides[3]; cuuint32_t box[4], estr[4];
  int gtn = 1, gth = 1, gtw = BM;
  if (!pl.flat) {
    double best = -1.0;
    for (int tw = 1; tw <= 128; tw <<= 1)
      for (int th = 1; th * tw <= 128; th <<= 1) {
        const int tn = 128 / (tw * th);
        if (tw * p.stride > 256 || th * p.stride > 256) continue;
        const long long tiles = (long long)((Wo + tw - 1) / tw) * ((Ho + th - 1) / th) * ((N + tn - 1) / tn);
        const double util = (double)N * Ho * Wo / (double)(tiles * 128) + 1e-6 * tw;
        if (util > best) { best = util; gtn = tn; gth = th; gtw = tw; }
      }
  }
  const long long P = (long long)p.x.N * p.x.H * p.x.W;
  {
    const bool r3_ok = (p.kh == 3 && p.kw == 3 && p.stride == 1 && p.pad == 1);
    const char *env3 = getenv("MPN_TC_R3");
    const char *env3m = getenv("MPN_TC_R3_MINPIX");
    const long long r3_minpix = env3m ? atoll(env3m) : 0;
    pl.mode = (r3_ok && !(env3 && env3[0] == '0') && P >= r3_minpix) ? 1 : 0;
  }
  const long long tiles_m = pl.flat ? (P + BM - 1) / BM
                                    : (pl.mode ? (long long)((Wo + 7) / 8) * ((Ho + 15) / 16) * N
                                               : (long long)((Wo + gtw - 1) / gtw) * ((Ho + gth - 1) / gth) * ((N + gtn - 1) / gtn));
  {
    const int taps = p.kh * p.kw;
    const double kblocks = (double)taps * (double)cblocks;
    double best = 1e300; int best_bn = 64;
    for (int bi = 0; bi < 3; ++bi) {
      const int bn = bi == 0 ? 256 : (bi == 1 ? 128 : 64);
      if (w16 && bn != 256) continue;
      if (fp8 && bn == 256) continue;
      if (!p.m_invariant && bn > 64 && bn > ((p.Cout + 63) / 64) * 64) continue;
      const int roi_bn = p.Cout > 128 ? 256 : (p.Cout > 64 ? 128 : 64);
      if (p.m_invariant && bn != (fp8 ? std::min(roi_bn, 128) : roi_bn)) continue;
      const long long units = tiles_m * ((p.Cout + bn - 1) / bn);
      const long long rounds = (units + sm_count - 1) / sm_count;
      const double mma = (w16 ? 2.0 : (pl.ops == OperandScheme::BF16X1 ? 1.0 : (fp8 ? 0.5 : 3.0))) * 128.0 * bn * 64.0 / 1024.0;
      const double ingest = ((double)a_planes(pl.ops) * 128 + (double)b_planes(pl.ops) * bn) * (fp8 ? 64.0 : 128.0) / 48.0;
      const double cost = (double)rounds * (kblocks * std::max(mma, ingest) + 1500.0 + 8.0 * bn);
      if (cost < best * 0.999) { best = cost; best_bn = bn; }
    }
    pl.BN = best_bn;
    pl.tiles_n = (p.Cout + pl.BN - 1) / pl.BN;
  }
  if (pl.flat) {
    pl.tn = 1; pl.th = 1; pl.tw = BM;
    pl.tiles_img = 1; pl.tiles_h = 1; pl.tiles_w = (int)((P + BM - 1) / BM);
    dims[0] = (cuuint64_t)p.x.C; dims[1] = (cuuint64_t)P; dims[2] = 1; dims[3] = 1;
    strides[0] = (cuuint64_t)p.x.ld * 2; strides[1] = (cuuint64_t)P * p.x.ld * 2; strides[2] = strides[1];
    box[0] = (cuuint32_t)stage_k(pl.BN, pl.ops); box[1] = BM; box[2] = 1; box[3] = 1;
    estr[0] = estr[1] = estr[2] = estr[3] = 1;
  } else {
    if (pl.mode == 1) { pl.tn = 1; pl.th = 16; pl.tw = 8; }
    else { pl.tn = gtn; pl.th = gth; pl.tw = gtw; }
// ... 29 lines not shown
  if (fp8) {
    const cuuint64_t C8 = (cuuint64_t)p.x.C;
    if (pl.flat) { strides[0] = C8; strides[1] = (cuuint64_t)P * C8; strides[2] = strides[1]; }
    else { strides[0] = C8; strides[1] = (cuuint64_t)p.x.W * C8; strides[2] = (cuuint64_t)p.x.H * p.x.W * C8; }
    bs[0] = (cuuint64_t)Ktot;
    MPN_TRY(encode_map(ctx, &pl.tmA_hi, p.x8, 4, dims, strides, box, estr, pl.BN, pl.ops));
    MPN_TRY(encode_map(ctx, &pl.tmB_hi, p.w8, 2, bd, bs, bb, be, pl.BN, pl.ops));
    pl.tmA_lo = pl.tmA_hi; pl.tmB_lo = pl.tmB_hi;
    pl.valid = 1;
    return MPN_OK;
  }
  MPN_TRY(encode_map(ctx, &pl.tmA_hi, p.x.hi, 4, dims, strides, box, estr, pl.BN, pl.ops));
  if (a_planes(pl.ops) == 2) { MPN_TRY(encode_map(ctx, &pl.tmA_lo, p.x.lo, 4, dims, strides, box, estr, pl.BN, pl.ops)); }
  else pl.tmA_lo = pl.tmA_hi;
  if (w16) {
    MPN_CHECK_ARG(ctx, pl.mode == 0 && pl.flat && pl.BN == 256, "conv_tc: the fp16-weight path is for wide flat GEMMs");
    MPN_TRY(encode_map(ctx, &pl.tmB_hi, p.w16, 2, bd, bs, bb, be, pl.BN, pl.ops));
    pl.tmB_lo = pl.tmB_hi;
  } else {
    MPN_TRY(encode_map(ctx, &pl.tmB_hi, p.w_hi, 2, bd, bs, bb, be, pl.BN, pl.ops));
    if (b_planes(pl.ops) == 2) { MPN_TRY(encode_map(ctx, &pl.tmB_lo, p.w_lo, 2, bd, bs, bb, be, pl.BN, pl.ops)); }
    else pl.tmB_lo = pl.tmB_hi;
  }
  pl.valid = 1;
  return MPN_OK;
}

int conv_tc_plan(mpn_ctx *ctx, const ConvProblem &p, ConvPlan &pl) { return conv_tc_plan_impl(ctx, ctx->sm_count, p, pl, false); }

int conv_tc_launch(mpn_ctx *ctx, const ConvProblem &p, const ConvPlan &pl) {
  MpnProfScope prof_scope__(ctx, MPN_CAT_CONV_TC);
  MPN_CHECK_ARG(ctx, pl.valid, "conv_tc_launch: invalid plan");
  TcParams tp;
  memset(&tp, 0, sizeof(tp));
  if (pl.flat) { tp.N = 1; tp.Ho = 1; tp.Wo = (int)(p.y.N * p.y.H * p.y.W); }
  else { tp.N = (int)p.y.N; tp.Ho = (int)p.y.H; tp.Wo = (int)p.y.W; }
  tp.Cout = p.Cout; tp.kh = p.kh; tp.kw = p.kw; tp.stride = p.stride; tp.pad = p.pad;
  tp.cblocks = (int)(conv_k_pad(p.x.C) / BK);
  tp.tn = pl.tn; tp.th = pl.th; tp.tw = pl.tw;
  tp.tiles_img = pl.tiles_img; tp.tiles_h = pl.tiles_h; tp.tiles_w = pl.tiles_w; tp.tiles_n = pl.tiles_n;
  tp.bias = p.bias;
  tp.res_hi = p.res.hi; tp.res_lo = p.res.lo; tp.res_ld = p.res.ld;
  tp.out_hi = p.y.hi; tp.out_lo = p.y.lo; tp.out_ld = p.y.ld;
  tp.out_f32 = p.y.f32; tp.out_f32_ld = p.y_f32_ld;
  tp.relu = p.relu;
  tp.splitk = pl.splitk; tp.kb_per_split = pl.kb_per_split; tp.split_stride = 0;
  tp.acc_scale = pl.ops == OperandScheme::FP16X2 ? p.w16_inv_scale : 1.f;
  tp.out_fmt = p.y.fmt; tp.ovf = nullptr;
  if (p.y.fmt) MPN_TRY(mpn_ovf_flag(ctx, &tp.ovf));
  if (pl.ops == OperandScheme::FP8X1) { tp.a_exp = p.x8_exp; tp.b_exp = p.w8_exp; tp.sample_pix = p.y.H * p.y.W; }
  MPN_CHECK_ARG(ctx, !p.pool.hi || p.pool.fmt == p.y.fmt, "conv_tc: pooled output must share the output's plane format");
  MPN_CHECK_ARG(ctx, !(p.y.fmt && pl.splitk > 1), "conv_tc: fp16 output planes are not written by the split-K reduce");
  MPN_CHECK_ARG(ctx, !p.res.hi || p.res.fmt == 0, "conv_tc: residual inputs are bf16 split planes");
  if (ctx->tl_on && ctx->tl_n < ctx->tl_cap) { tp.tl_min = ctx->tl_min + 4 * ctx->tl_n; tp.tl_max = ctx->tl_max + 4 * ctx->tl_n; ++ctx->tl_n; }
  if (p.pool.hi) {
    MPN_CHECK_ARG(ctx, pl.mode == 1 && pl.splitk == 1 && !p.res.hi && p.Cout % 8 == 0 && p.pool.ld % 8 == 0,
                  "conv_tc: fused pooling needs the 3x3 kernel, no residual, Cout multiple of 8");
    MPN_CHECK_ARG(ctx, p.pool.H == (p.y.H + 1) / 2 && p.pool.W == (p.y.W + 1) / 2 && p.pool.N == p.y.N, "conv_tc: pooled geometry mismatch");
    tp.pool_hi = p.pool.hi; tp.pool_lo = p.pool.lo; tp.pool_ld = p.pool.ld; tp.Hp = (int)p.pool.H; tp.Wp = (int)p.pool.W;
    if (p.pool_only) { tp.out_hi = tp.out_lo = nullptr; tp.out_f32 = nullptr; }
  }
  if (p.y.hi) MPN_CHECK_ARG(ctx, p.Cout % 8 == 0 && p.y.ld % 8 == 0, "conv_tc: split output needs Cout, ld multiples of 8");
  MPN_CHECK_ARG(ctx, p.scatter.n == 0 || pl.splitk > 1, "conv_tc: scattered outputs need a split-K plan");
  if (pl.splitk > 1) {
    const long long pixels = (long long)p.y.N * p.y.H * p.y.W;
    float *ws = nullptr;
    MPN_TRY(mpn_scratch3(ctx, sizeof(float) * (size_t)pl.splitk * pixels * p.Cout, (void **)&ws));
    tp.bias = nullptr; tp.res_hi = tp.res_lo = nullptr; tp.relu = 0; tp.out_hi = tp.out_lo = nullptr;
    tp.out_f32 = ws; tp.out_f32_ld = p.Cout; tp.split_stride = pixels * p.Cout;
    MPN_TRY(launch_ops(ctx, pl, tp));
    ReduceParams r;
    r.ws = ws; r.split_stride = tp.split_stride; r.splitk = pl.splitk; r.pixels = pixels; r.Cout = p.Cout;
    r.bias = p.bias; r.res_hi = p.res.hi; r.res_lo = p.res.lo; r.res_ld = p.res.ld; r.relu = p.relu;
    r.out_hi = p.y.hi; r.out_lo = p.y.lo; r.out_ld = p.y.ld; r.out_f32 = p.y.f32; r.out_f32_ld = p.y_f32_ld;
    r.scatter = p.scatter;
    const long long total = pixels * p.Cout;
    MPN_CUDA(ctx, mpn_launch_pdl(ctx, splitk_reduce_kernel, dim3((unsigned)((total + 255) / 256)), dim3(256), 0, r));
    MPN_LAUNCHED(ctx);
    return MPN_OK;
  }
  return launch_ops(ctx, pl, tp);
}

extern "C" int mpn_debug_plan(int64_t N, int64_t Cin, int64_t H, int64_t W, int64_t Cout, int32_t k, int32_t stride, int32_t pad,
                              int32_t per_roi, int32_t sm_count, int32_t *out) {
  if (!out || N <= 0 || Cin <= 0 || Cin % 8 || H <= 0 || W <= 0 || Cout <= 0 || k <= 0 || stride < 1 || stride > 2 || pad < 0 || sm_count < 2 ||
      per_roi < 0 || per_roi > 2)
    return MPN_ERR_ARG;
  ConvProblem p;
  p.x.N = N; p.x.H = H; p.x.W = W; p.x.C = Cin; p.x.ld = Cin;
  p.Cout = (int)Cout; p.kh = p.kw = k; p.stride = stride; p.pad = pad; p.m_invariant = per_roi ? 1 : 0;
  p.fill_split = per_roi == 2 ? 1 : 0;
  p.y.N = N; p.y.H = (H + 2 * pad - k) / stride + 1; p.y.W = (W + 2 * pad - k) / stride + 1; p.y.C = Cout; p.y.ld = Cout;
  if (p.y.H <= 0 || p.y.W <= 0) return MPN_ERR_ARG;
  ConvPlan pl;
  const int rc = conv_tc_plan_impl(nullptr, sm_count, p, pl, true);
  if (rc != MPN_OK) return rc;
  out[0] = pl.mode; out[1] = 1; out[2] = pl.BN; out[3] = pl.splitk; out[4] = 0; out[5] = pl.tn; out[6] = pl.th; out[7] = pl.tw;
  return MPN_OK;
}
```

### multipathnet_b200/csrc/model.cu

```cuda
#include "conv_gemm.cuh"
#include "roi.cuh"
#include <algorithm>
#include <cmath>
#include <map>
#include <memory>
#include <set>
#include "train_rule.cuh"

int mpn_maxpool_launch(mpn_ctx *, const DTensor &, int, int, int, DTensor &);
int mpn_avgpool_launch(mpn_ctx *, const DTensor &, DTensor &);
int mpn_weight_permute_split_launch(mpn_ctx *, const float *, int64_t, int, int, int, __nv_bfloat16 *, __nv_bfloat16 *, int);
int mpn_nhwc_split_to_nchw_launch(mpn_ctx *, const DTensor &, float *);
int mpn_project_rois_launch(mpn_ctx *, const float *, int64_t, float, float *);
int mpn_get_images_launch(mpn_ctx *, const float *, int32_t, int32_t, const mpn_image_transform *, int32_t, int32_t, float *);
int mpn_get_images_size_impl(int32_t, int32_t, double, double, int32_t *, int32_t *, double *);
int mpn_get_images_u8_launch(mpn_ctx *, const uint8_t *, int32_t, int32_t, const mpn_image_transform *, int32_t, int32_t, float *);
int mpn_bbox_norm_launch(mpn_ctx *, float *, int64_t, int64_t, const float *, const float *);
int mpn_bbox_decode_launch(mpn_ctx *, const float *, const float *, int64_t, int, int, float, float, float *);
int mpn_softmax_mean_launch(mpn_ctx *, const float *, int64_t, int, int, int, float *);
int mpn_detect_tail_launch(mpn_ctx *, const float *, int64_t, int, int, int, float *, const float *, const float *, int, float, float,
                           float *, int, const float *, const float *);
int mpn_gather_scored_launch(mpn_ctx *, const float *, const float *, int, int, float, float *, int32_t *, int32_t *);
int mpn_nms_launch(mpn_ctx *, const float *, int, int, const int32_t *, const int32_t *, float, int32_t *, int32_t *);
int mpn_pack_detections_launch(mpn_ctx *, const float *, const float *, int, const int32_t *, const int32_t *, int, int, float *);
// ... 7 lines not shown
int mpn_train_rois5_launch(mpn_ctx *, const float *, int64_t, float *);
int mpn_train_dropout_launch(mpn_ctx *, const DTensor &, int64_t, int64_t, uint64_t, uint32_t, int, int, float);
int mpn_train_dropout_mask_launch(mpn_ctx *, int64_t, uint64_t, uint32_t, int, int, float, uint8_t *);
int mpn_train_gate_mask_launch(mpn_ctx *, const DTensor &, int64_t, int64_t, uint8_t *);
int mpn_train_gate_split_launch(mpn_ctx *, float *, int64_t, int64_t, int64_t, const DTensor *, float, __nv_bfloat16 *, __nv_bfloat16 *,
                                int64_t, int64_t);
int mpn_train_transpose_launch(mpn_ctx *, const float *, const __nv_bfloat16 *, const __nv_bfloat16 *, int64_t, int64_t, int64_t, int, int, int,
                               __nv_bfloat16 *, __nv_bfloat16 *, int64_t, int64_t);
int mpn_train_colsum_launch(mpn_ctx *, const float *, int64_t, int64_t, int64_t, float *);
int mpn_train_sgd_launch(mpn_ctx *, int, float *, const float *, float *, int64_t, float, float, float, float, int, float *, const mpn_optim_step &);
int mpn_train_scale_launch(mpn_ctx *, float *, int64_t, float);
int mpn_train_sgd_split_launch(mpn_ctx *, int, float *, const float *, float *, int, int, int, float, float, float, float, int, __nv_bfloat16 *,
                               __nv_bfloat16 *, __nv_bfloat16 *, __nv_bfloat16 *, int64_t, int64_t, int, const float *, float *,
                               const mpn_optim_step &);
int mpn_train_split_planes_launch(mpn_ctx *, const float *, int, int, int, __nv_bfloat16 *, __nv_bfloat16 *, __nv_bfloat16 *, __nv_bfloat16 *,
                                  int64_t, int64_t, int);
int mpn_train_pool_gate_split_launch(mpn_ctx *, const float *, const DTensor &, float *, __nv_bfloat16 *, __nv_bfloat16 *);
int mpn_train_tap_transpose_launch(mpn_ctx *, const DTensor &, int, int, int, int64_t, int64_t, __nv_bfloat16 *, __nv_bfloat16 *, int64_t,
                                   int64_t);
int mpn_train_col2im_add_launch(mpn_ctx *, const float *, const DTensor &, int, int, int, int64_t, int64_t, float *);
int mpn_train_avgpool_backward_launch(mpn_ctx *, const float *, int64_t, int64_t, int, int, float *);
int mpn_train_add_launch(mpn_ctx *, float *, const float *, int64_t);
int mpn_train_gemm(mpn_ctx *, const __nv_bfloat16 *, const __nv_bfloat16 *, int64_t, int64_t, int64_t, const __nv_bfloat16 *,
                   const __nv_bfloat16 *, int64_t, float *, int64_t, int = 0, int = 0);

namespace {

struct DevBuf {
  void *p = nullptr; size_t bytes = 0;
  DevBuf() = default;
  DevBuf(const DevBuf &) = delete;
  DevBuf &operator=(const DevBuf &) = delete;
  DevBuf(DevBuf &&o) noexcept : p(o.p), bytes(o.bytes) { o.p = nullptr; o.bytes = 0; }
  DevBuf &operator=(DevBuf &&o) noexcept {
    if (this != &o) {
      if (p) cudaFree(p);
      p = o.p; bytes = o.bytes; o.p = nullptr; o.bytes = 0;
    }
    return *this;
  }
  ~DevBuf() { if (p) cudaFree(p); }
  int ensure(mpn_ctx *ctx, size_t n) {
    if (n <= bytes) return MPN_OK;
    if (p) { cudaFree(p); p = nullptr; bytes = 0; }
    MPN_CUDA(ctx, cudaMalloc(&p, n));
    bytes = n;
    return MPN_OK;
  }
};

struct SplitBuf {
  DevBuf hi, lo;
  int ensure(mpn_ctx *ctx, size_t elems, bool with_lo = true) {
    MPN_TRY(hi.ensure(ctx, elems * 2 + 256));
    return with_lo ? lo.ensure(ctx, elems * 2 + 256) : MPN_OK;
  }
};

struct WeightDev {
  DevBuf hi, lo;
  DevBuf h16; float h16_scale = 0.f;
  DevBuf f32;
  DevBuf q8, e8; bool has8 = false;
  int64_t n = 0;
  int64_t row = 0;
};

struct Fp8Buf {
  DevBuf q, e;
  int ensure(mpn_ctx *ctx, const DTensor &x) {
    MPN_TRY(q.ensure(ctx, (size_t)(x.N * x.H * x.W * x.C) + 256));
    return e.ensure(ctx, sizeof(int) * (size_t)x.N + 256);
  }
};

struct LayerExec {
  mpn_layer L;
  ConvProblem prob;
  ConvPlan plan;
  bool is_direct = false;
  DTensor in, out;
  bool fused_pool = false, pool_only = false;
  DTensor pool_out_t;
  bool quant = false;
};

struct TrainParam {
  int w = -1; int64_t n = 0; bool bias = false;
  int cout = 0, cin = 0, kh = 1, kw = 1;
  DevBuf grad, buf, buf2;
  __nv_bfloat16 *wt_hi = nullptr, *wt_lo = nullptr; int64_t wt_ld = 0, wt_col0 = 0; bool flip = false;
  int head = -1;
  bool fixed = false; DevBuf a2;
  bool idle = false;
};
struct TrainState {
  mpn_train_config cfg;
  mpn_train_optim optim = {MPN_OPTIM_SGD, 0.0, 0.0, 0.0, 0.0, 0.0};
  int trunk_from = 0;
  int phase2_from = 0; bool phase2 = false;
  uint32_t step = 0;
  int head = 0, last_head = 0;
  bool plan = false;
  bool bf16 = false;
  int64_t last_R = 0; int last_images = 0;
  std::vector<TrainParam> params; std::map<int, int> param_of;
  std::vector<DevBuf> images;
  DevBuf boxes, rois5, labels, targets, losses, dlogits, dbbox, dconcat, dx[2];
  SplitBuf opA, opGT, opXT;
  std::vector<std::unique_ptr<SplitBuf>> wt_bufs;
  std::vector<std::map<int, std::unique_ptr<SplitBuf>>> img_bufs; std::vector<std::map<int, DTensor>> img_slots;
  std::vector<std::unique_ptr<DevBuf>> dpooled;
  DevBuf roi_argmax, roi_ab;
  SplitBuf grad_split, opTap;
  std::set<int> fixed;
  std::vector<bool> graph_tower;
  std::vector<std::unique_ptr<DevBuf>> grad_bufs; std::multimap<size_t, DevBuf *> grad_free;
  DevBuf dtmp;
  cudaEvent_t ev[5] = {};
  ~TrainState() { for (cudaEvent_t e : ev) if (e) cudaEventDestroy(e); }
};

int pool_out(int in, int k, int s, int p, int ceil_mode) {
  int o = ceil_mode ? (in + 2 * p - k + s - 1) / s + 1 : (in + 2 * p - k) / s + 1;
  if (ceil_mode && (o - 1) * s >= in + p) --o;
  return o;
}

}

struct mpn_model {
  mpn_ctx *ctx = nullptr;
  mpn_model_desc d;
  std::vector<mpn_layer> trunk_layers, tower_layers;
  std::vector<mpn_tower> towers;
  std::vector<mpn_head> cls_heads;
  std::vector<std::unique_ptr<WeightDev>> weights;
  std::vector<int64_t> w_elems;
  std::vector<std::vector<float>> w_host_small;
  std::vector<int> w_prepared;
  int conv_impl = 0;

  int tH = 0, tW = 0; bool trunk_valid = false;
  std::vector<LayerExec> trunk_exec;
  std::map<int, DTensor> trunk_slots; std::map<int, std::unique_ptr<SplitBuf>> trunk_bufs;
  std::map<int, std::unique_ptr<Fp8Buf>> trunk_q8;
  DevBuf image_dev, raw_image_dev;
  int merged_w = -1, merged_b = -1;
  bool merged_stale = false;
  std::set<int> elided_slots;
  double trunk_flops = 0, head_flops = 0;
  struct Pyramid { std::vector<std::unique_ptr<DevBuf>> lv; int nlev = 1; };
  std::map<int, Pyramid> pyramids;

  int64_t hR = 0; bool heads_planned = false;
  struct TowerExec {
    std::unique_ptr<SplitBuf> pooled_buf; DTensor pooled; int ctot = 0;
    std::vector<LayerExec> layers; std::map<int, DTensor> slots; std::map<int, std::unique_ptr<SplitBuf>> bufs;
    int out_features = 0, col_off = 0;
    std::map<int, int> slot_fmt;
    std::map<int, std::unique_ptr<Fp8Buf>> q8;
  };
  std::vector<TowerExec> tex;
  SplitBuf concat_buf; int concat_width = 0;
  std::vector<LayerExec> head_exec;
  DevBuf rois_dev, boxes_dev, cls_logits, bbox_raw, scores_dev, bboxes_dev;
  DevBuf sb_dev, src_idx_dev, counts_dev, keep_idx_dev, keep_counts_dev;
  RoiJobs jobs;
  struct PipeSlot {
    DevBuf image, raw_u8, boxes, scores, bboxes, keep_idx, keep_counts;
    cudaEvent_t h2d = nullptr, compute = nullptr, done = nullptr;
    bool busy = false; int ticket = -1;
  };
  PipeSlot pipe[2];
  cudaStream_t s_h2d = nullptr, s_d2h = nullptr;
  int next_ticket = 0;
  DevBuf to_pass_scores, to_pass_bboxes, to_new_boxes, to_scores, to_bboxes, to_sb, to_src, to_counts, to_keep, to_keep_counts, to_voted;
  float *sink = nullptr; int64_t sink_cap = 0, sink_n = 0; int sink_top_k = 100;
  std::unique_ptr<TrainState> train;
  bool plan_split_only = false;
  bool plan_train_bf16 = false, trunk_train_bf16 = false;
  ~mpn_model() {
    for (auto &q : pipe) { if (q.h2d) cudaEventDestroy(q.h2d); if (q.compute) cudaEventDestroy(q.compute); if (q.done) cudaEventDestroy(q.done); }
    if (s_h2d) cudaStreamDestroy(s_h2d);
    if (s_d2h) cudaStreamDestroy(s_d2h);
  }
};

namespace {

int upload_weight_raw(mpn_model *m, int idx, const float *host, int64_t n) {
  WeightDev &w = *m->weights[idx];
  w.n = n;
  MPN_TRY(w.f32.ensure(m->ctx, sizeof(float) * (size_t)std::max<int64_t>(n, 1)));
  MPN_CUDA(m->ctx, cudaMemcpyAsync(w.f32.p, host, sizeof(float) * (size_t)n, cudaMemcpyHostToDevice, m->ctx->stream));
  return MPN_OK;
}

int prepare_conv_weight(mpn_model *m, int idx, int Cout, int Cin, int kh, int kw, bool flat = false) {
  mpn_ctx *ctx = m->ctx;
  MPN_CHECK_ARG(ctx, idx >= 0 && idx < (int)m->weights.size(), "layer weight index out of range");
  WeightDev &w = *m->weights[idx];
  MPN_CHECK_ARG(ctx, w.n == (int64_t)Cout * Cin * kh * kw, "weight element count does not match layer geometry");
  if (m->w_prepared[idx] == 1) return MPN_OK;
  MPN_CHECK_ARG(ctx, m->w_prepared[idx] == 0, "weight already prepared as an fp16 plane");
  w.row = conv_weight_row(Cin, kh, kw, flat ? 1 : 0);
  const size_t elems = (size_t)((int64_t)Cout * w.row);
  MPN_TRY(w.hi.ensure(ctx, elems * 2 + 256));
  MPN_TRY(w.lo.ensure(ctx, elems * 2 + 256));
  MPN_TRY(mpn_weight_permute_split_launch(ctx, (const float *)w.f32.p, Cout, Cin, kh, kw, (__nv_bfloat16 *)w.hi.p,
                                          (__nv_bfloat16 *)w.lo.p, flat ? 1 : 0));
  m->w_prepared[idx] = 1;
  if (!m->train || !m->train->param_of.count(idx)) { cudaFree(w.f32.p); w.f32.p = nullptr; w.f32.bytes = 0; }
  return MPN_OK;
}

int prepare_conv_weight_w16(mpn_model *m, int idx, int Cout, int Cin, int kh, int kw) {
  mpn_ctx *ctx = m->ctx;
  MPN_CHECK_ARG(ctx, idx >= 0 && idx < (int)m->weights.size(), "layer weight index out of range");
  WeightDev &w = *m->weights[idx];
  MPN_CHECK_ARG(ctx, w.n == (int64_t)Cout * Cin * kh * kw, "weight element count does not match layer geometry");
  if (m->w_prepared[idx] == 2) return MPN_OK;
  MPN_CHECK_ARG(ctx, m->w_prepared[idx] == 0, "weight already prepared in the split-bf16 layout");
  float amax = 0.f;
  MPN_TRY(mpn_absmax(ctx, (const float *)w.f32.p, w.n, &amax));
  MPN_CHECK_ARG(ctx, std::isfinite(amax), "weight holds a non-finite value");
  int e = 0;
  if (amax > 0.f) { (void)std::frexp(amax, &e); e = 14 - e; }
  e = std::max(-60, std::min(60, e));
  w.h16_scale = std::ldexp(1.0f, e);
  MPN_TRY(w.h16.ensure(ctx, (size_t)w.n * 2 + 256));
  MPN_TRY(mpn_weight_permute_half_launch(ctx, (const float *)w.f32.p, Cout, Cin, kh, kw, w.h16_scale, w.h16.p));
  m->w_prepared[idx] = 2;
// ... 79 lines not shown
  if (e.quant) MPN_TRY(mpn_fp8_quantize_launch(m->ctx, e.prob.x, const_cast<uint8_t *>(e.prob.x8), const_cast<int *>(e.prob.x8_exp)));
  if (m->conv_impl == 1) return conv_ref_launch(m->ctx, e.prob);
  return conv_tc_launch(m->ctx, e.prob, e.plan);
}

int plan_trunk(mpn_model *m, int H, int W) {
  mpn_ctx *ctx = m->ctx;
  m->trunk_exec.clear(); m->trunk_slots.clear();
  m->trunk_flops = 0;
  MPN_CHECK_ARG(ctx, !(ctx->opt_fp8 == 1 && ctx->opt_bf16 == 1), "the \"fp8\" and \"bf16\" options are both on");
  const bool fp8 = ctx->opt_fp8 == 1;
  std::set<int> quantized;
  DTensor img; img.N = 1; img.H = H; img.W = W; img.C = 3; img.ld = 3;
  m->trunk_slots[0] = img;
  for (const mpn_layer &L : m->trunk_layers) {
    MPN_CHECK_ARG(ctx, m->trunk_slots.count(L.in_slot), "trunk layer reads an undefined slot");
    const DTensor in = m->trunk_slots[L.in_slot];
    LayerExec e; e.L = L;
    DTensor out; out.N = in.N;
    if (L.kind == MPN_LAYER_CONV) {
      MPN_CHECK_ARG(ctx, L.cin == in.C, "trunk conv cin does not match its input");
      out.H = (in.H + 2 * L.pad - L.kh) / L.stride + 1; out.W = (in.W + 2 * L.pad - L.kw) / L.stride + 1; out.C = L.cout;
    } else if (L.kind == MPN_LAYER_MAXPOOL) {
      out.H = pool_out((int)in.H, L.kh, L.stride, L.pad, L.ceil_mode);
      out.W = pool_out((int)in.W, L.kw, L.stride, L.pad, L.ceil_mode); out.C = in.C;
    } else {
      return mpn_fail(ctx, MPN_ERR_ARG, "unsupported trunk layer kind");
    }
    MPN_CHECK_ARG(ctx, out.H > 0 && out.W > 0, "trunk layer output is empty");
    MPN_CHECK_ARG(ctx, L.out_slot > 0, "trunk layers may not write slot 0");
    auto &buf = m->trunk_bufs[L.out_slot];
    if (!buf) buf.reset(new SplitBuf());
    MPN_TRY(buf->ensure(ctx, (size_t)(out.N * out.H * out.W * out.C)));
    out = make_split_view(*buf, out.N, out.H, out.W, out.C);
    if (L.kind == MPN_LAYER_CONV) {
      if (L.in_slot == 0) {
        e.is_direct = true; e.in = in; e.out = out;
        MPN_CHECK_ARG(ctx, L.weight >= 0 && m->weights[L.weight]->n == (int64_t)L.cout * L.cin * L.kh * L.kw,
                      "first-layer weight size mismatch");
      } else {
        DTensor o2 = out;
        Fp8Buf *q8 = nullptr;
        if (fp8) {
          auto &qb = m->trunk_q8[L.in_slot];
          if (!qb) qb.reset(new Fp8Buf());
          q8 = qb.get();
          e.quant = quantized.insert(L.in_slot).second;
        }
        MPN_TRY(build_conv(m, e, in, o2, 0, 0, 0, false, q8));
        if (L.residual_slot >= 0) {
          MPN_CHECK_ARG(ctx, m->trunk_slots.count(L.residual_slot), "residual slot undefined");
          e.prob.res = m->trunk_slots[L.residual_slot];
        }
      }
      m->trunk_flops += 2.0 * L.cin * L.cout * L.kh * L.kw * (double)out.H * out.W * out.N;
    } else {
      e.in = in; e.out = out;
    }
    m->trunk_slots[L.out_slot] = out;
    quantized.erase(L.out_slot);
    m->trunk_exec.push_back(e);
  }
  {
    const char *envf = getenv("MPN_TC_FUSE_POOL");
    const bool allow = !(envf && envf[0] == '0');
    for (size_t i = 0; allow && i + 1 < m->trunk_exec.size(); ++i) {
      LayerExec &c = m->trunk_exec[i]; const LayerExec &q = m->trunk_exec[i + 1];
      if (c.L.kind != MPN_LAYER_CONV || c.is_direct || q.L.kind != MPN_LAYER_MAXPOOL) continue;
      if (q.L.in_slot != c.L.out_slot || q.L.kh != 2 || q.L.kw != 2 || q.L.stride != 2 || q.L.pad != 0) continue;
      if (c.plan.mode != 1 || c.plan.splitk != 1 || c.L.residual_slot >= 0 || (c.L.cout % 8) != 0) continue;
      if (q.out.H != (c.out.H + 1) / 2 || q.out.W != (c.out.W + 1) / 2) continue;
      bool other_reader = false;
      for (size_t j = 0; j < m->trunk_exec.size(); ++j) {
        if (j == i + 1) continue;
        const mpn_layer &L2 = m->trunk_exec[j].L;
        if (j > i && (L2.in_slot == c.L.out_slot || L2.residual_slot == c.L.out_slot)) other_reader = true;
      }
      for (const mpn_tower &T : m->towers)
        for (int l = 0; l < T.n_levels; ++l) if (T.level_slot[l] == c.L.out_slot) other_reader = true;
      if (m->train && m->train->trunk_from > 0 && (int)i >= m->train->trunk_from) other_reader = true;
      c.fused_pool = true; c.pool_only = !other_reader; c.pool_out_t = q.out;
    }
  }
  for (const mpn_tower &T : m->towers)
    for (int l = 0; l < T.n_levels; ++l) {
      const int slot = T.level_slot[l];
      MPN_CHECK_ARG(ctx, m->trunk_slots.count(slot) && slot > 0, "tower level reads an undefined trunk slot");
      const DTensor &f = m->trunk_slots[slot];
      mpn_model::Pyramid &P = m->pyramids[slot];
      const double rs = T.region == 0 ? 1.0 : (T.region == 1 ? 1.5 : (T.region == 2 ? 2.0 : 4.0));
      const long long max_bin = std::min<long long>(std::min(f.H, f.W),
          (long long)std::ceil(rs * (double)std::max(f.H, f.W) / (double)std::min(T.pooled_h, T.pooled_w)) + 2);
      int nlev = 1;
      while (nlev < ROI_MAX_LEVELS && (1ll << nlev) <= max_bin) ++nlev;
      nlev = std::max(nlev, P.nlev);
      P.nlev = nlev;
      P.lv.resize(nlev);
      for (int k = 0; k < nlev; ++k) {
        if (!P.lv[k]) P.lv[k].reset(new DevBuf());
        MPN_TRY(P.lv[k]->ensure(ctx, sizeof(float) * (size_t)(f.N * f.H * f.W * f.C) + 256));
      }
    }
  m->tH = H; m->tW = W; m->trunk_valid = false; m->heads_planned = false;
  m->trunk_train_bf16 = m->plan_train_bf16;
  return MPN_OK;
}

int run_trunk(mpn_model *m, const float *image_dev) {
  mpn_ctx *ctx = m->ctx;
  m->elided_slots.clear();
  for (size_t li = 0; li < m->trunk_exec.size(); ++li) {
    LayerExec &e = m->trunk_exec[li];
    const mpn_layer &L = e.L;
    if (e.fused_pool && m->conv_impl == 0) {
      if (e.quant) MPN_TRY(mpn_fp8_quantize_launch(ctx, e.prob.x, const_cast<uint8_t *>(e.prob.x8), const_cast<int *>(e.prob.x8_exp)));
      ConvProblem pf = e.prob;
      pf.pool = e.pool_out_t; pf.pool_only = e.pool_only ? 1 : 0;
      MPN_TRY(conv_tc_launch(ctx, pf, e.plan));
      if (e.pool_only) m->elided_slots.insert(L.out_slot);
      ++li;
      continue;
    }
    if (L.kind == MPN_LAYER_CONV) {
      if (e.is_direct) {
        const float *bias = L.bias >= 0 ? (const float *)m->weights[L.bias]->f32.p : nullptr;
        MPN_TRY(conv_direct_nchw_launch(ctx, image_dev, 1, L.cin, (int)e.in.H, (int)e.in.W,
                                        (const float *)m->weights[L.weight]->f32.p, bias, L.cout, L.kh, L.kw, L.stride,
                                        L.pad, L.relu, e.out,
                                        m->w_host_small[L.weight].empty() ? nullptr : m->w_host_small[L.weight].data(),
                                        (L.bias >= 0 && !m->w_host_small[L.bias].empty()) ? m->w_host_small[L.bias].data() : nullptr));
      } else {
        MPN_TRY(run_conv(m, e));
      }
    } else {
      MPN_TRY(mpn_maxpool_launch(ctx, e.in, L.kh, L.stride, L.pad, e.out));
    }
  }
  for (auto &kv : m->pyramids) {
    const DTensor &f = m->trunk_slots[kv.first];
    float *lv[ROI_MAX_LEVELS] = {nullptr};
    for (int k = 0; k < kv.second.nlev; ++k) lv[k] = (float *)kv.second.lv[k]->p;
    int too_big = 0;
    MPN_TRY(mpn_maxpyr_all_launch(ctx, f.hi, f.lo, (int)f.N, (int)f.H, (int)f.W, (int)f.C, f.ld, kv.second.nlev, lv, &too_big));
    if (!too_big) continue;
    MPN_TRY(mpn_pyr_level0_launch(ctx, f.hi, f.lo, (int)f.N, (int)f.H, (int)f.W, (int)f.C, f.ld, lv[0]));
    for (int k = 1; k < kv.second.nlev; ++k)
      MPN_TRY(mpn_maxpyr_launch(ctx, lv[k - 1], (int)f.N, (int)f.H, (int)f.W, (int)f.C, 1 << (k - 1), lv[k]));
  }
  m->trunk_valid = true;
  return MPN_OK;
}

int plan_heads(mpn_model *m, int64_t R) {
  mpn_ctx *ctx = m->ctx;
  const int C = m->d.num_classes;
  m->head_flops = 0;
  MPN_CHECK_ARG(ctx, !(ctx->opt_fp8 == 1 && ctx->opt_bf16 == 1), "the \"fp8\" and \"bf16\" options are both on");
  const bool fp8 = ctx->opt_fp8 == 1;
  m->tex.clear(); m->tex.resize(m->towers.size());
  m->jobs.n = 0;
  int width = 0;
  std::vector<int> feat(m->towers.size(), 0);
  for (size_t t = 0; t < m->towers.size(); ++t) {
    const mpn_tower &T = m->towers[t];
    int f = -1;
    for (int i = 0; i < T.n_layers; ++i) {
      const mpn_layer &L = m->tower_layers[T.first_layer + i];
      if (L.out_slot == T.out_slot) f = (L.kind == MPN_LAYER_CONV) ? L.cout : -2;
    }
    MPN_CHECK_ARG(ctx, f != -1, "tower out_slot is never written");
    feat[t] = f;
  }
  for (size_t t = 0; t < m->towers.size(); ++t) {
    const mpn_tower &T = m->towers[t];
    mpn_model::TowerExec &X = m->tex[t];
    X.ctot = 0;
    for (int l = 0; l < T.n_levels; ++l) {
      MPN_CHECK_ARG(ctx, m->trunk_slots.count(T.level_slot[l]) && T.level_slot[l] > 0, "tower level reads an undefined trunk slot");
      X.ctot += (int)m->trunk_slots[T.level_slot[l]].C;
    }
    X.pooled_buf.reset(new SplitBuf());
    MPN_TRY(X.pooled_buf->ensure(ctx, (size_t)R * T.pooled_h * T.pooled_w * X.ctot));
    X.pooled = make_split_view(*X.pooled_buf, R, T.pooled_h, T.pooled_w, X.ctot);
    int ch_off = 0;
    for (int l = 0; l < T.n_levels; ++l) {
      MPN_CHECK_ARG(ctx, m->jobs.n < MAX_ROI_JOBS, "too many (tower, level) ROI jobs");
      const DTensor &f = m->trunk_slots[T.level_slot[l]];
      RoiJob &j = m->jobs.j[m->jobs.n++];
      j.H = (int)f.H; j.W = (int)f.W; j.C = (int)f.C; j.scale = T.level_scale[l];
      j.region = T.region; j.out_hi = X.pooled.hi; j.out_lo = X.pooled.lo; j.out_ld = X.ctot; j.out_ch_off = ch_off;
      j.normalize = T.normalize; j.out_fmt = 0; j.ovf = nullptr; j.tower = (int)t;
      const mpn_model::Pyramid &P = m->pyramids[T.level_slot[l]];
      j.nlev = P.nlev;
      for (int k = 0; k < ROI_MAX_LEVELS; ++k) j.lv[k] = (const float *)P.lv[std::min(k, P.nlev - 1)]->p;
      ch_off += (int)f.C;
    }
    std::map<int, DTensor> shp; shp[0] = X.pooled;
    for (int i = 0; i < T.n_layers; ++i) {
      const mpn_layer &L = m->tower_layers[T.first_layer + i];
      MPN_CHECK_ARG(ctx, shp.count(L.in_slot), "tower layer reads an undefined slot");
      const DTensor in = shp[L.in_slot]; DTensor out; out.N = R;
      if (L.kind == MPN_LAYER_CONV) {
        MPN_CHECK_ARG(ctx, L.cin == in.C, "tower conv cin does not match its input");
        out.H = (in.H + 2 * L.pad - L.kh) / L.stride + 1; out.W = (in.W + 2 * L.pad - L.kw) / L.stride + 1; out.C = L.cout;
      } else if (L.kind == MPN_LAYER_FLATTEN) { out.H = 1; out.W = 1; out.C = in.H * in.W * in.C; }
      else if (L.kind == MPN_LAYER_AVGPOOL) { out.H = 1; out.W = 1; out.C = in.C; }
      else if (L.kind == MPN_LAYER_MAXPOOL) {
        out.H = pool_out((int)in.H, L.kh, L.stride, L.pad, L.ceil_mode); out.W = pool_out((int)in.W, L.kw, L.stride, L.pad, L.ceil_mode);
        out.C = in.C;
      } else return mpn_fail(ctx, MPN_ERR_ARG, "unsupported tower layer kind");
      shp[L.out_slot] = out;
    }
    {
// ... 592 lines not shown
  MPN_TRY(m->boxes_dev.ensure(ctx, sizeof(float) * 4 * (size_t)R));
  MPN_TRY(m->to_pass_scores.ensure(ctx, bs * n_it)); MPN_TRY(m->to_pass_bboxes.ensure(ctx, bb * n_it));
  MPN_TRY(m->to_new_boxes.ensure(ctx, sizeof(float) * 4 * (size_t)R));
  MPN_TRY(m->to_scores.ensure(ctx, sizeof(float) * (size_t)n_out * C)); MPN_TRY(m->to_bboxes.ensure(ctx, sizeof(float) * (size_t)n_out * 4 * C));
  MPN_TRY(m->to_sb.ensure(ctx, sizeof(float) * 5 * (size_t)(C - 1) * n_out)); MPN_TRY(m->to_src.ensure(ctx, sizeof(int32_t) * (size_t)(C - 1) * n_out));
  MPN_TRY(m->to_counts.ensure(ctx, sizeof(int32_t) * (size_t)C)); MPN_TRY(m->to_keep.ensure(ctx, sizeof(int32_t) * (size_t)(C - 1) * n_out));
  MPN_TRY(m->to_keep_counts.ensure(ctx, sizeof(int32_t) * (size_t)C));
  if (o->bbox_voting) MPN_TRY(m->to_voted.ensure(ctx, sizeof(float) * 5 * (size_t)(C - 1) * n_out));
  MPN_CUDA(ctx, cudaMemcpyAsync(m->image_dev.p, image, sizeof(float) * 3 * (size_t)H * W, cudaMemcpyHostToDevice, ctx->stream));
  MPN_CUDA(ctx, cudaMemcpyAsync(m->boxes_dev.p, boxes, sizeof(float) * 4 * (size_t)R, cudaMemcpyHostToDevice, ctx->stream));
  MPN_TRY(mpn_model_trunk_dev(m, (const float *)m->image_dev.p, H, W));
  auto ps = [&](int it) { return (float *)((char *)m->to_pass_scores.p + bs * it); };
  auto pb = [&](int it) { return (float *)((char *)m->to_pass_bboxes.p + bb * it); };
  MPN_TRY(run_detect_pass(m, (const float *)m->boxes_dev.p, R, im_scale, 1, W0, H0, ps(0), pb(0)));
  for (int it = 1; it < n_it; ++it) {
    MPN_TRY(mpn_select_boxes_launch(ctx, ps(it - 1), pb(it - 1), R, C, nullptr, nullptr, (float *)m->to_new_boxes.p));
    MPN_TRY(run_detect_pass(m, (const float *)m->to_new_boxes.p, R, im_scale, 0, 0.f, 0.f, ps(it), pb(it)));
  }
  const int s0 = o->use_rbox_scores ? 1 : 0, n_blocks = n_it - s0;
  MPN_CUDA(ctx, cudaMemcpyAsync(m->to_scores.p, ps(s0), bs * n_blocks, cudaMemcpyDeviceToDevice, ctx->stream));
  MPN_CUDA(ctx, cudaMemcpyAsync(m->to_bboxes.p, pb(0), bb * n_blocks, cudaMemcpyDeviceToDevice, ctx->stream));
  MPN_TRY(mpn_gather_scored_launch(ctx, (const float *)m->to_scores.p, (const float *)m->to_bboxes.p, (int)n_out, C, o->score_thresh,
                                   (float *)m->to_sb.p, (int32_t *)m->to_src.p, (int32_t *)m->to_counts.p));
  MPN_TRY(mpn_nms_launch(ctx, (const float *)m->to_sb.p, (int)n_out, C - 1, (const int32_t *)m->to_counts.p, (const int32_t *)m->to_src.p,
                         o->nms_thr, (int32_t *)m->to_keep.p, (int32_t *)m->to_keep_counts.p));
  if (o->bbox_voting)
    MPN_TRY(mpn_bbox_vote_batched_launch(ctx, (const float *)m->to_sb.p, (const int32_t *)m->to_counts.p, (const int32_t *)m->to_keep.p,
                                         (const int32_t *)m->to_keep_counts.p, (const float *)m->to_scores.p, (const float *)m->to_bboxes.p, C,
                                         (int)n_out, o->vote_thr, o->vote_score_pow, (float *)m->to_voted.p));
  if (scores) MPN_CUDA(ctx, cudaMemcpyAsync(scores, m->to_scores.p, sizeof(float) * (size_t)n_out * C, cudaMemcpyDeviceToHost, ctx->stream));
  if (bboxes) MPN_CUDA(ctx, cudaMemcpyAsync(bboxes, m->to_bboxes.p, sizeof(float) * (size_t)n_out * 4 * C, cudaMemcpyDeviceToHost, ctx->stream));
  if (keep_idx) MPN_CUDA(ctx, cudaMemcpyAsync(keep_idx, m->to_keep.p, sizeof(int32_t) * (size_t)(C - 1) * n_out, cudaMemcpyDeviceToHost, ctx->stream));
  if (keep_counts) MPN_CUDA(ctx, cudaMemcpyAsync(keep_counts, m->to_keep_counts.p, sizeof(int32_t) * (size_t)(C - 1), cudaMemcpyDeviceToHost, ctx->stream));
  if (voted && o->bbox_voting) MPN_CUDA(ctx, cudaMemcpyAsync(voted, m->to_voted.p, sizeof(float) * 5 * (size_t)(C - 1) * n_out, cudaMemcpyDeviceToHost, ctx->stream));
  MPN_TRY(mpn_ovf_copy_async(ctx, ctx->stream));
  MPN_CUDA(ctx, cudaStreamSynchronize(ctx->stream));
  return mpn_ovf_test(ctx);
}

int mpn_model_set_detection_sink(mpn_model *m, float *records_dev, int64_t capacity, int32_t top_k) {
  if (!m) return MPN_ERR_ARG;
  mpn_ctx *ctx = m->ctx;
  MPN_CHECK_ARG(ctx, !records_dev || (capacity > 0 && top_k >= 1 && top_k <= MPN_MAX_DET), "detection sink: capacity > 0 and 1 <= top_k <= MPN_MAX_DET");
  m->sink = records_dev; m->sink_cap = records_dev ? capacity : 0; m->sink_n = 0; m->sink_top_k = records_dev ? top_k : 100;
  return MPN_OK;
}

int mpn_model_detection_sink_count(const mpn_model *m, int64_t *n_records) {
  if (!m || !n_records) return MPN_ERR_ARG;
  *n_records = m->sink_n;
  return MPN_OK;
}

int mpn_model_get_pooled(mpn_model *m, int32_t tower, int64_t r0, int64_t n, float *out, int64_t capacity, int64_t *R_total,
                         int32_t *bins, int32_t *Ctot) {
  if (!m) return MPN_ERR_ARG;
  mpn_ctx *ctx = m->ctx;
  MPN_CUDA(ctx, cudaSetDevice(ctx->device));
  MPN_CHECK_ARG(ctx, m->heads_planned && tower >= 0 && tower < (int)m->tex.size(), "no heads pass yet, or unknown tower");
  const DTensor &t = m->tex[tower].pooled;
  const int64_t row = t.H * t.W * t.C;
  if (R_total) *R_total = t.N;
  if (bins) *bins = (int32_t)(t.H * t.W);
  if (Ctot) *Ctot = (int32_t)t.C;
  if (!out) return MPN_OK;
  MPN_CHECK_ARG(ctx, r0 >= 0 && n > 0 && r0 + n <= t.N && capacity >= n * row, "row range outside the pooled tensor, or buffer too small");
  void *tmp = nullptr;
  MPN_TRY(mpn_scratch(ctx, sizeof(float) * (size_t)(n * row), &tmp));
  MPN_TRY(mpn_join_rows_launch(ctx, t.hi + r0 * row, t.lo + r0 * row, n, row, row, t.fmt, (float *)tmp));
  MPN_CUDA(ctx, cudaMemcpyAsync(out, tmp, sizeof(float) * (size_t)(n * row), cudaMemcpyDeviceToHost, ctx->stream));
  MPN_TRY(mpn_ovf_copy_async(ctx, ctx->stream));
  MPN_CUDA(ctx, cudaStreamSynchronize(ctx->stream));
  return mpn_ovf_test(ctx);
}

int mpn_model_get_trunk_slot(mpn_model *m, int32_t slot, float *out_nchw, int64_t capacity, int32_t *C, int32_t *H,
                             int32_t *W) {
  if (!m) return MPN_ERR_ARG;
  mpn_ctx *ctx = m->ctx;
  MPN_CUDA(ctx, cudaSetDevice(ctx->device));
  MPN_CHECK_ARG(ctx, m->trunk_valid && slot > 0 && m->trunk_slots.count(slot), "unknown trunk slot or no trunk forward yet");
  MPN_CHECK_ARG(ctx, !m->elided_slots.count(slot),
                "trunk slot was fused into the following max pool and never written (mpn_model_set_conv_impl(m, 2) disables the fusion)");
  const DTensor &t = m->trunk_slots[slot];
  const int64_t n = t.N * t.C * t.H * t.W;
  if (C) *C = (int32_t)t.C; if (H) *H = (int32_t)t.H; if (W) *W = (int32_t)t.W;
  if (!out_nchw) return MPN_OK;
  MPN_CHECK_ARG(ctx, capacity >= n, "output buffer too small");
  void *tmp = nullptr;
  MPN_TRY(mpn_scratch(ctx, sizeof(float) * (size_t)n, &tmp));
  MPN_TRY(mpn_nhwc_split_to_nchw_launch(ctx, t, (float *)tmp));
  MPN_CUDA(ctx, cudaMemcpyAsync(out_nchw, tmp, sizeof(float) * (size_t)n, cudaMemcpyDeviceToHost, ctx->stream));
  MPN_CUDA(ctx, cudaStreamSynchronize(ctx->stream));
  return MPN_OK;
}

int mpn_model_get_slot_planes(mpn_model *m, int32_t tower, int32_t slot, int64_t r0, int64_t n, uint16_t *hi, uint16_t *lo,
                              uint8_t *q8, int32_t *e8, int64_t capacity, int32_t *fmt, int64_t *dims) {
  if (!m) return MPN_ERR_ARG;
  mpn_ctx *ctx = m->ctx;
  MPN_CUDA(ctx, cudaSetDevice(ctx->device));
  const DTensor *t = nullptr;
  const Fp8Buf *qb = nullptr;
  if (tower == -1) {
    MPN_CHECK_ARG(ctx, m->trunk_valid && slot > 0 && m->trunk_slots.count(slot), "unknown trunk slot or no trunk forward yet");
    MPN_CHECK_ARG(ctx, !m->elided_slots.count(slot), "trunk slot was fused into the following max pool and never written");
    t = &m->trunk_slots[slot];
    for (const LayerExec &e : m->trunk_exec)
      if (e.L.kind == MPN_LAYER_CONV && !e.is_direct && e.prob.fp8 && e.L.in_slot == slot) qb = m->trunk_q8[slot].get();
  } else {
    MPN_CHECK_ARG(ctx, m->heads_planned && tower >= 0 && tower < (int)m->tex.size(), "no heads pass yet, or unknown tower");
    mpn_model::TowerExec &X = m->tex[tower];
    MPN_CHECK_ARG(ctx, X.slots.count(slot), "unknown tower slot");
    t = &X.slots[slot];
    auto it = X.q8.find(slot);
    if (it != X.q8.end()) qb = it->second.get();
  }
  const int64_t px = t->H * t->W;
  if (fmt) *fmt = t->fmt;
  if (dims) { dims[0] = t->N; dims[1] = t->H; dims[2] = t->W; dims[3] = t->C; }
  if (!hi) return MPN_OK;
  MPN_CHECK_ARG(ctx, lo && r0 >= 0 && n > 0 && r0 + n <= t->N, "rows outside the slot, or lo plane missing");
  MPN_CHECK_ARG(ctx, capacity >= n * px * t->C, "output buffer too small");
  MPN_CHECK_ARG(ctx, !(q8 || e8) || (q8 && e8 && qb), "the current plan keeps no e4m3 plane for this slot");
  const size_t w = sizeof(uint16_t) * (size_t)t->C, pitch = sizeof(uint16_t) * (size_t)t->ld, rows = (size_t)(n * px);
  const __nv_bfloat16 *src[2] = {t->hi + r0 * px * t->ld, t->lo + r0 * px * t->ld};
  uint16_t *dst[2] = {hi, lo};
  for (int p = 0; p < 2; ++p) {
    if (t->ld == t->C) MPN_CUDA(ctx, cudaMemcpyAsync(dst[p], src[p], w * rows, cudaMemcpyDeviceToHost, ctx->stream));
    else MPN_CUDA(ctx, cudaMemcpy2DAsync(dst[p], w, src[p], pitch, w, rows, cudaMemcpyDeviceToHost, ctx->stream));
  }
  if (q8) {
    MPN_CUDA(ctx, cudaMemcpyAsync(q8, (const uint8_t *)qb->q.p + r0 * px * t->C, (size_t)(n * px * t->C), cudaMemcpyDeviceToHost, ctx->stream));
    MPN_CUDA(ctx, cudaMemcpyAsync(e8, (const int *)qb->e.p + r0, sizeof(int32_t) * (size_t)n, cudaMemcpyDeviceToHost, ctx->stream));
  }
  MPN_CUDA(ctx, cudaStreamSynchronize(ctx->stream));
  return MPN_OK;
}

int mpn_model_get_head_outputs(mpn_model *m, float *cls_logits, float *bbox_raw, int64_t *R, int32_t *K) {
  if (!m) return MPN_ERR_ARG;
  mpn_ctx *ctx = m->ctx;
  MPN_CUDA(ctx, cudaSetDevice(ctx->device));
  MPN_CHECK_ARG(ctx, m->heads_planned, "no heads pass yet");
  const int C = m->d.num_classes, nk = (int)m->cls_heads.size();
  if (R) *R = m->hR;
  if (K) *K = nk;
  if (cls_logits)
    MPN_CUDA(ctx, cudaMemcpyAsync(cls_logits, m->cls_logits.p, sizeof(float) * (size_t)nk * m->hR * C, cudaMemcpyDeviceToHost, ctx->stream));
  if (bbox_raw)
    MPN_CUDA(ctx, cudaMemcpyAsync(bbox_raw, m->bbox_raw.p, sizeof(float) * (size_t)m->hR * 4 * C, cudaMemcpyDeviceToHost, ctx->stream));
  MPN_CUDA(ctx, cudaStreamSynchronize(ctx->stream));
  return MPN_OK;
}

}


int mpn_model_n_cls_heads(const mpn_model *m) { return (int)m->cls_heads.size(); }

static bool fixed_conv_ok(const mpn_layer &L) {
  return L.kind == MPN_LAYER_CONV && L.kh == L.kw && (L.kh == 1 || L.kh == 3) && (L.stride == 1 || L.stride == 2) &&
         L.pad == (L.kh - 1) / 2 && L.weight >= 0 && L.cout > 0 && L.cout % 64 == 0;
}
static const char *const FIXED_CONV_MSG = "training: a fixed-batch-norm layer must be a 1x1 or 3x3 convolution with stride 1 or 2, pad "
                                          "(k - 1) / 2 and a multiple of 64 output channels";
static const char *const TAIL_MSG = "training: a trained layer must read a multiple of 64 input channels (a Linear after a FLATTEN: "
                                    "channels x pooled area); a layer with a K tail, such as NIN's 96-channel block 1, runs forward only";
static bool recorded(const std::set<int> *rec, const mpn_layer &L) {
  return rec && L.kind == MPN_LAYER_CONV && L.weight >= 0 && rec->count(L.weight);
}
static bool graph_tower(const mpn_model_desc *d, const mpn_tower &T, const std::set<int> *rec) {
  for (int i = 0; i < T.n_layers; ++i) if (recorded(rec, d->tower_layers[T.first_layer + i])) return true;
  return false;
}

static int train_check_graph(const mpn_model_desc *d, bool integral, const char **msg, const std::set<int> *rec) {
  *msg = nullptr;
  if (d->n_cls_heads < 1) { *msg = "training: the graph has no class head"; return MPN_ERR_ARG; }
  if (d->n_cls_heads != 1 && !integral) {
    *msg = "training: an integral head (K > 1 class heads) trains only with the integral loss (mpn_train_spec.integral = 1, "
           "Trainer(integral=True))";
    return MPN_ERR_ARG;
  }
  std::set<int> seen;
  auto own = [&](int w) { if (w < 0) return true; return seen.insert(w).second; };
  for (int t = 0; t < d->n_towers; ++t) {
    const mpn_tower &T = d->towers[t];
    const bool graph = graph_tower(d, T, rec);
// ... 1280 lines not shown
```

### multipathnet_b200/csrc/wgmma.cuh

```cuda
#pragma once
#include <stdint.h>

__device__ __forceinline__ void wgmma_bf16_n64(float (&d)[32], uint64_t da, uint64_t db, uint32_t scale_d) {
  asm volatile("{\n.reg .pred p;\nsetp.ne.b32 p, %34, 0;\n"
               "wgmma.mma_async.sync.aligned.m64n64k16.f32.bf16.bf16 {%0, %1, %2, %3, %4, %5, %6, %7, %8, %9, %10, %11, %12, %13, %14, %15, %16, %17, %18, %19, %20, %21, %22, %23, %24, %25, %26, %27, %28, %29, %30, %31}, %32, %33, p, 1, 1, 0, 0;\n}\n"
               : "+f"(d[0]), "+f"(d[1]), "+f"(d[2]), "+f"(d[3]), "+f"(d[4]), "+f"(d[5]), "+f"(d[6]), "+f"(d[7]), "+f"(d[8]), "+f"(d[9]), "+f"(d[10]), "+f"(d[11]), "+f"(d[12]), "+f"(d[13]), "+f"(d[14]), "+f"(d[15]), "+f"(d[16]), "+f"(d[17]), "+f"(d[18]), "+f"(d[19]), "+f"(d[20]), "+f"(d[21]), "+f"(d[22]), "+f"(d[23]), "+f"(d[24]), "+f"(d[25]), "+f"(d[26]), "+f"(d[27]), "+f"(d[28]), "+f"(d[29]), "+f"(d[30]), "+f"(d[31])
               : "l"(da), "l"(db), "r"(scale_d));
}
__device__ __forceinline__ void wgmma_bf16_n128(float (&d)[64], uint64_t da, uint64_t db, uint32_t scale_d) {
  asm volatile("{\n.reg .pred p;\nsetp.ne.b32 p, %66, 0;\n"
               "wgmma.mma_async.sync.aligned.m64n128k16.f32.bf16.bf16 {%0, %1, %2, %3, %4, %5, %6, %7, %8, %9, %10, %11, %12, %13, %14, %15, %16, %17, %18, %19, %20, %21, %22, %23, %24, %25, %26, %27, %28, %29, %30, %31, %32, %33, %34, %35, %36, %37, %38, %39, %40, %41, %42, %43, %44, %45, %46, %47, %48, %49, %50, %51, %52, %53, %54, %55, %56, %57, %58, %59, %60, %61, %62, %63}, %64, %65, p, 1, 1, 0, 0;\n}\n"
               : "+f"(d[0]), "+f"(d[1]), "+f"(d[2]), "+f"(d[3]), "+f"(d[4]), "+f"(d[5]), "+f"(d[6]), "+f"(d[7]), "+f"(d[8]), "+f"(d[9]), "+f"(d[10]), "+f"(d[11]), "+f"(d[12]), "+f"(d[13]), "+f"(d[14]), "+f"(d[15]), "+f"(d[16]), "+f"(d[17]), "+f"(d[18]), "+f"(d[19]), "+f"(d[20]), "+f"(d[21]), "+f"(d[22]), "+f"(d[23]), "+f"(d[24]), "+f"(d[25]), "+f"(d[26]), "+f"(d[27]), "+f"(d[28]), "+f"(d[29]), "+f"(d[30]), "+f"(d[31]), "+f"(d[32]), "+f"(d[33]), "+f"(d[34]), "+f"(d[35]), "+f"(d[36]), "+f"(d[37]), "+f"(d[38]), "+f"(d[39]), "+f"(d[40]), "+f"(d[41]), "+f"(d[42]), "+f"(d[43]), "+f"(d[44]), "+f"(d[45]), "+f"(d[46]), "+f"(d[47]), "+f"(d[48]), "+f"(d[49]), "+f"(d[50]), "+f"(d[51]), "+f"(d[52]), "+f"(d[53]), "+f"(d[54]), "+f"(d[55]), "+f"(d[56]), "+f"(d[57]), "+f"(d[58]), "+f"(d[59]), "+f"(d[60]), "+f"(d[61]), "+f"(d[62]), "+f"(d[63])
               : "l"(da), "l"(db), "r"(scale_d));
}
__device__ __forceinline__ void wgmma_bf16_n256(float (&d)[128], uint64_t da, uint64_t db, uint32_t scale_d) {
  asm volatile("{\n.reg .pred p;\nsetp.ne.b32 p, %130, 0;\n"
               "wgmma.mma_async.sync.aligned.m64n256k16.f32.bf16.bf16 {%0, %1, %2, %3, %4, %5, %6, %7, %8, %9, %10, %11, %12, %13, %14, %15, %16, %17, %18, %19, %20, %21, %22, %23, %24, %25, %26, %27, %28, %29, %30, %31, %32, %33, %34, %35, %36, %37, %38, %39, %40, %41, %42, %43, %44, %45, %46, %47, %48, %49, %50, %51, %52, %53, %54, %55, %56, %57, %58, %59, %60, %61, %62, %63, %64, %65, %66, %67, %68, %69, %70, %71, %72, %73, %74, %75, %76, %77, %78, %79, %80, %81, %82, %83, %84, %85, %86, %87, %88, %89, %90, %91, %92, %93, %94, %95, %96, %97, %98, %99, %100, %101, %102, %103, %104, %105, %106, %107, %108, %109, %110, %111, %112, %113, %114, %115, %116, %117, %118, %119, %120, %121, %122, %123, %124, %125, %126, %127}, %128, %129, p, 1, 1, 0, 0;\n}\n"
               : "+f"(d[0]), "+f"(d[1]), "+f"(d[2]), "+f"(d[3]), "+f"(d[4]), "+f"(d[5]), "+f"(d[6]), "+f"(d[7]), "+f"(d[8]), "+f"(d[9]), "+f"(d[10]), "+f"(d[11]), "+f"(d[12]), "+f"(d[13]), "+f"(d[14]), "+f"(d[15]), "+f"(d[16]), "+f"(d[17]), "+f"(d[18]), "+f"(d[19]), "+f"(d[20]), "+f"(d[21]), "+f"(d[22]), "+f"(d[23]), "+f"(d[24]), "+f"(d[25]), "+f"(d[26]), "+f"(d[27]), "+f"(d[28]), "+f"(d[29]), "+f"(d[30]), "+f"(d[31]), "+f"(d[32]), "+f"(d[33]), "+f"(d[34]), "+f"(d[35]), "+f"(d[36]), "+f"(d[37]), "+f"(d[38]), "+f"(d[39]), "+f"(d[40]), "+f"(d[41]), "+f"(d[42]), "+f"(d[43]), "+f"(d[44]), "+f"(d[45]), "+f"(d[46]), "+f"(d[47]), "+f"(d[48]), "+f"(d[49]), "+f"(d[50]), "+f"(d[51]), "+f"(d[52]), "+f"(d[53]), "+f"(d[54]), "+f"(d[55]), "+f"(d[56]), "+f"(d[57]), "+f"(d[58]), "+f"(d[59]), "+f"(d[60]), "+f"(d[61]), "+f"(d[62]), "+f"(d[63]), "+f"(d[64]), "+f"(d[65]), "+f"(d[66]), "+f"(d[67]), "+f"(d[68]), "+f"(d[69]), "+f"(d[70]), "+f"(d[71]), "+f"(d[72]), "+f"(d[73]), "+f"(d[74]), "+f"(d[75]), "+f"(d[76]), "+f"(d[77]), "+f"(d[78]), "+f"(d[79]), "+f"(d[80]), "+f"(d[81]), "+f"(d[82]), "+f"(d[83]), "+f"(d[84]), "+f"(d[85]), "+f"(d[86]), "+f"(d[87]), "+f"(d[88]), "+f"(d[89]), "+f"(d[90]), "+f"(d[91]), "+f"(d[92]), "+f"(d[93]), "+f"(d[94]), "+f"(d[95]), "+f"(d[96]), "+f"(d[97]), "+f"(d[98]), "+f"(d[99]), "+f"(d[100]), "+f"(d[101]), "+f"(d[102]), "+f"(d[103]), "+f"(d[104]), "+f"(d[105]), "+f"(d[106]), "+f"(d[107]), "+f"(d[108]), "+f"(d[109]), "+f"(d[110]), "+f"(d[111]), "+f"(d[112]), "+f"(d[113]), "+f"(d[114]), "+f"(d[115]), "+f"(d[116]), "+f"(d[117]), "+f"(d[118]), "+f"(d[119]), "+f"(d[120]), "+f"(d[121]), "+f"(d[122]), "+f"(d[123]), "+f"(d[124]), "+f"(d[125]), "+f"(d[126]), "+f"(d[127])
               : "l"(da), "l"(db), "r"(scale_d));
}
__device__ __forceinline__ void wgmma_f16_n64(float (&d)[32], uint64_t da, uint64_t db, uint32_t scale_d) {
  asm volatile("{\n.reg .pred p;\nsetp.ne.b32 p, %34, 0;\n"
               "wgmma.mma_async.sync.aligned.m64n64k16.f32.f16.f16 {%0, %1, %2, %3, %4, %5, %6, %7, %8, %9, %10, %11, %12, %13, %14, %15, %16, %17, %18, %19, %20, %21, %22, %23, %24, %25, %26, %27, %28, %29, %30, %31}, %32, %33, p, 1, 1, 0, 0;\n}\n"
               : "+f"(d[0]), "+f"(d[1]), "+f"(d[2]), "+f"(d[3]), "+f"(d[4]), "+f"(d[5]), "+f"(d[6]), "+f"(d[7]), "+f"(d[8]), "+f"(d[9]), "+f"(d[10]), "+f"(d[11]), "+f"(d[12]), "+f"(d[13]), "+f"(d[14]), "+f"(d[15]), "+f"(d[16]), "+f"(d[17]), "+f"(d[18]), "+f"(d[19]), "+f"(d[20]), "+f"(d[21]), "+f"(d[22]), "+f"(d[23]), "+f"(d[24]), "+f"(d[25]), "+f"(d[26]), "+f"(d[27]), "+f"(d[28]), "+f"(d[29]), "+f"(d[30]), "+f"(d[31])
               : "l"(da), "l"(db), "r"(scale_d));
}
__device__ __forceinline__ void wgmma_f16_n128(float (&d)[64], uint64_t da, uint64_t db, uint32_t scale_d) {
  asm volatile("{\n.reg .pred p;\nsetp.ne.b32 p, %66, 0;\n"
               "wgmma.mma_async.sync.aligned.m64n128k16.f32.f16.f16 {%0, %1, %2, %3, %4, %5, %6, %7, %8, %9, %10, %11, %12, %13, %14, %15, %16, %17, %18, %19, %20, %21, %22, %23, %24, %25, %26, %27, %28, %29, %30, %31, %32, %33, %34, %35, %36, %37, %38, %39, %40, %41, %42, %43, %44, %45, %46, %47, %48, %49, %50, %51, %52, %53, %54, %55, %56, %57, %58, %59, %60, %61, %62, %63}, %64, %65, p, 1, 1, 0, 0;\n}\n"
               : "+f"(d[0]), "+f"(d[1]), "+f"(d[2]), "+f"(d[3]), "+f"(d[4]), "+f"(d[5]), "+f"(d[6]), "+f"(d[7]), "+f"(d[8]), "+f"(d[9]), "+f"(d[10]), "+f"(d[11]), "+f"(d[12]), "+f"(d[13]), "+f"(d[14]), "+f"(d[15]), "+f"(d[16]), "+f"(d[17]), "+f"(d[18]), "+f"(d[19]), "+f"(d[20]), "+f"(d[21]), "+f"(d[22]), "+f"(d[23]), "+f"(d[24]), "+f"(d[25]), "+f"(d[26]), "+f"(d[27]), "+f"(d[28]), "+f"(d[29]), "+f"(d[30]), "+f"(d[31]), "+f"(d[32]), "+f"(d[33]), "+f"(d[34]), "+f"(d[35]), "+f"(d[36]), "+f"(d[37]), "+f"(d[38]), "+f"(d[39]), "+f"(d[40]), "+f"(d[41]), "+f"(d[42]), "+f"(d[43]), "+f"(d[44]), "+f"(d[45]), "+f"(d[46]), "+f"(d[47]), "+f"(d[48]), "+f"(d[49]), "+f"(d[50]), "+f"(d[51]), "+f"(d[52]), "+f"(d[53]), "+f"(d[54]), "+f"(d[55]), "+f"(d[56]), "+f"(d[57]), "+f"(d[58]), "+f"(d[59]), "+f"(d[60]), "+f"(d[61]), "+f"(d[62]), "+f"(d[63])
               : "l"(da), "l"(db), "r"(scale_d));
}
__device__ __forceinline__ void wgmma_f16_n256(float (&d)[128], uint64_t da, uint64_t db, uint32_t scale_d) {
  asm volatile("{\n.reg .pred p;\nsetp.ne.b32 p, %130, 0;\n"
               "wgmma.mma_async.sync.aligned.m64n256k16.f32.f16.f16 {%0, %1, %2, %3, %4, %5, %6, %7, %8, %9, %10, %11, %12, %13, %14, %15, %16, %17, %18, %19, %20, %21, %22, %23, %24, %25, %26, %27, %28, %29, %30, %31, %32, %33, %34, %35, %36, %37, %38, %39, %40, %41, %42, %43, %44, %45, %46, %47, %48, %49, %50, %51, %52, %53, %54, %55, %56, %57, %58, %59, %60, %61, %62, %63, %64, %65, %66, %67, %68, %69, %70, %71, %72, %73, %74, %75, %76, %77, %78, %79, %80, %81, %82, %83, %84, %85, %86, %87, %88, %89, %90, %91, %92, %93, %94, %95, %96, %97, %98, %99, %100, %101, %102, %103, %104, %105, %106, %107, %108, %109, %110, %111, %112, %113, %114, %115, %116, %117, %118, %119, %120, %121, %122, %123, %124, %125, %126, %127}, %128, %129, p, 1, 1, 0, 0;\n}\n"
               : "+f"(d[0]), "+f"(d[1]), "+f"(d[2]), "+f"(d[3]), "+f"(d[4]), "+f"(d[5]), "+f"(d[6]), "+f"(d[7]), "+f"(d[8]), "+f"(d[9]), "+f"(d[10]), "+f"(d[11]), "+f"(d[12]), "+f"(d[13]), "+f"(d[14]), "+f"(d[15]), "+f"(d[16]), "+f"(d[17]), "+f"(d[18]), "+f"(d[19]), "+f"(d[20]), "+f"(d[21]), "+f"(d[22]), "+f"(d[23]), "+f"(d[24]), "+f"(d[25]), "+f"(d[26]), "+f"(d[27]), "+f"(d[28]), "+f"(d[29]), "+f"(d[30]), "+f"(d[31]), "+f"(d[32]), "+f"(d[33]), "+f"(d[34]), "+f"(d[35]), "+f"(d[36]), "+f"(d[37]), "+f"(d[38]), "+f"(d[39]), "+f"(d[40]), "+f"(d[41]), "+f"(d[42]), "+f"(d[43]), "+f"(d[44]), "+f"(d[45]), "+f"(d[46]), "+f"(d[47]), "+f"(d[48]), "+f"(d[49]), "+f"(d[50]), "+f"(d[51]), "+f"(d[52]), "+f"(d[53]), "+f"(d[54]), "+f"(d[55]), "+f"(d[56]), "+f"(d[57]), "+f"(d[58]), "+f"(d[59]), "+f"(d[60]), "+f"(d[61]), "+f"(d[62]), "+f"(d[63]), "+f"(d[64]), "+f"(d[65]), "+f"(d[66]), "+f"(d[67]), "+f"(d[68]), "+f"(d[69]), "+f"(d[70]), "+f"(d[71]), "+f"(d[72]), "+f"(d[73]), "+f"(d[74]), "+f"(d[75]), "+f"(d[76]), "+f"(d[77]), "+f"(d[78]), "+f"(d[79]), "+f"(d[80]), "+f"(d[81]), "+f"(d[82]), "+f"(d[83]), "+f"(d[84]), "+f"(d[85]), "+f"(d[86]), "+f"(d[87]), "+f"(d[88]), "+f"(d[89]), "+f"(d[90]), "+f"(d[91]), "+f"(d[92]), "+f"(d[93]), "+f"(d[94]), "+f"(d[95]), "+f"(d[96]), "+f"(d[97]), "+f"(d[98]), "+f"(d[99]), "+f"(d[100]), "+f"(d[101]), "+f"(d[102]), "+f"(d[103]), "+f"(d[104]), "+f"(d[105]), "+f"(d[106]), "+f"(d[107]), "+f"(d[108]), "+f"(d[109]), "+f"(d[110]), "+f"(d[111]), "+f"(d[112]), "+f"(d[113]), "+f"(d[114]), "+f"(d[115]), "+f"(d[116]), "+f"(d[117]), "+f"(d[118]), "+f"(d[119]), "+f"(d[120]), "+f"(d[121]), "+f"(d[122]), "+f"(d[123]), "+f"(d[124]), "+f"(d[125]), "+f"(d[126]), "+f"(d[127])
               : "l"(da), "l"(db), "r"(scale_d));
}

__device__ __forceinline__ void wgmma_e4m3_n64(float (&d)[32], uint64_t da, uint64_t db, uint32_t scale_d) {
  asm volatile("{\n.reg .pred p;\nsetp.ne.b32 p, %34, 0;\n"
               "wgmma.mma_async.sync.aligned.m64n64k32.f32.e4m3.e4m3 {%0, %1, %2, %3, %4, %5, %6, %7, %8, %9, %10, %11, %12, %13, %14, %15, %16, %17, %18, %19, %20, %21, %22, %23, %24, %25, %26, %27, %28, %29, %30, %31}, %32, %33, p, 1, 1;\n}\n"
               : "+f"(d[0]), "+f"(d[1]), "+f"(d[2]), "+f"(d[3]), "+f"(d[4]), "+f"(d[5]), "+f"(d[6]), "+f"(d[7]), "+f"(d[8]), "+f"(d[9]), "+f"(d[10]), "+f"(d[11]), "+f"(d[12]), "+f"(d[13]), "+f"(d[14]), "+f"(d[15]), "+f"(d[16]), "+f"(d[17]), "+f"(d[18]), "+f"(d[19]), "+f"(d[20]), "+f"(d[21]), "+f"(d[22]), "+f"(d[23]), "+f"(d[24]), "+f"(d[25]), "+f"(d[26]), "+f"(d[27]), "+f"(d[28]), "+f"(d[29]), "+f"(d[30]), "+f"(d[31])
               : "l"(da), "l"(db), "r"(scale_d));
}
__device__ __forceinline__ void wgmma_e4m3_n128(float (&d)[64], uint64_t da, uint64_t db, uint32_t scale_d) {
  asm volatile("{\n.reg .pred p;\nsetp.ne.b32 p, %66, 0;\n"
               "wgmma.mma_async.sync.aligned.m64n128k32.f32.e4m3.e4m3 {%0, %1, %2, %3, %4, %5, %6, %7, %8, %9, %10, %11, %12, %13, %14, %15, %16, %17, %18, %19, %20, %21, %22, %23, %24, %25, %26, %27, %28, %29, %30, %31, %32, %33, %34, %35, %36, %37, %38, %39, %40, %41, %42, %43, %44, %45, %46, %47, %48, %49, %50, %51, %52, %53, %54, %55, %56, %57, %58, %59, %60, %61, %62, %63}, %64, %65, p, 1, 1;\n}\n"
               : "+f"(d[0]), "+f"(d[1]), "+f"(d[2]), "+f"(d[3]), "+f"(d[4]), "+f"(d[5]), "+f"(d[6]), "+f"(d[7]), "+f"(d[8]), "+f"(d[9]), "+f"(d[10]), "+f"(d[11]), "+f"(d[12]), "+f"(d[13]), "+f"(d[14]), "+f"(d[15]), "+f"(d[16]), "+f"(d[17]), "+f"(d[18]), "+f"(d[19]), "+f"(d[20]), "+f"(d[21]), "+f"(d[22]), "+f"(d[23]), "+f"(d[24]), "+f"(d[25]), "+f"(d[26]), "+f"(d[27]), "+f"(d[28]), "+f"(d[29]), "+f"(d[30]), "+f"(d[31]), "+f"(d[32]), "+f"(d[33]), "+f"(d[34]), "+f"(d[35]), "+f"(d[36]), "+f"(d[37]), "+f"(d[38]), "+f"(d[39]), "+f"(d[40]), "+f"(d[41]), "+f"(d[42]), "+f"(d[43]), "+f"(d[44]), "+f"(d[45]), "+f"(d[46]), "+f"(d[47]), "+f"(d[48]), "+f"(d[49]), "+f"(d[50]), "+f"(d[51]), "+f"(d[52]), "+f"(d[53]), "+f"(d[54]), "+f"(d[55]), "+f"(d[56]), "+f"(d[57]), "+f"(d[58]), "+f"(d[59]), "+f"(d[60]), "+f"(d[61]), "+f"(d[62]), "+f"(d[63])
               : "l"(da), "l"(db), "r"(scale_d));
}
template <int N> __device__ __forceinline__ void wgmma_e4m3_nk32(float (&d)[N / 2], uint64_t da, uint64_t db, uint32_t scale_d) {
  static_assert(N == 64 || N == 128, "fp8 tiles are 64 or 128 channels wide");
  if constexpr (N == 64) wgmma_e4m3_n64(d, da, db, scale_d); else wgmma_e4m3_n128(d, da, db, scale_d);
}

template <int N, bool F16> __device__ __forceinline__ void wgmma_nk16(float (&d)[N / 2], uint64_t da, uint64_t db, uint32_t scale_d) {
  if constexpr (F16) {
    if constexpr (N == 64) wgmma_f16_n64(d, da, db, scale_d); else if constexpr (N == 128) wgmma_f16_n128(d, da, db, scale_d); else wgmma_f16_n256(d, da, db, scale_d);
  } else {
    if constexpr (N == 64) wgmma_bf16_n64(d, da, db, scale_d); else if constexpr (N == 128) wgmma_bf16_n128(d, da, db, scale_d); else wgmma_bf16_n256(d, da, db, scale_d);
  }
}
__device__ __forceinline__ void wgmma_fence() { asm volatile("wgmma.fence.sync.aligned;" ::: "memory"); }
__device__ __forceinline__ void wgmma_commit() { asm volatile("wgmma.commit_group.sync.aligned;" ::: "memory"); }
template <int K> __device__ __forceinline__ void wgmma_wait() { asm volatile("wgmma.wait_group.sync.aligned %0;" ::"n"(K) : "memory"); }
template <int R> __device__ __forceinline__ void wgmma_fence_acc(float (&d)[R]) {
#pragma unroll
  for (int i = 0; i < R; ++i) asm volatile("" : "+f"(d[i])::"memory");
}
```

Measured before the change: 416,000.

## Fuse first conv, second conv and max pool into one persistent kernel

Adds a persistent kernel that computes conv1 (3->64) into a shared-memory halo tile and feeds it straight into the 64->64 3x3 conv with fused max pool. The full-resolution conv1 activation is no longer written to or read back from global memory, and one launch is removed. Conv1 is materialised lazily only if a debug accessor asks for that slot. The cost is redundant halo recompute of conv1, a large shared-memory footprint that allows only one CTA per SM, and register-sourced wgmma for the first layer.

```diff
diff --git a/include/mpn_abi.h b/include/mpn_abi.h
--- a/include/mpn_abi.h
+++ b/include/mpn_abi.h
@@ -226,6 +226,10 @@
 int mpn_conv_bench(mpn_ctx *ctx, int64_t N, int64_t Cin, int64_t H, int64_t W, int64_t Cout, int32_t k, int32_t stride,
                    int32_t pad, int32_t iters, double *ms_per_launch, int32_t *bn, int32_t *cta_group, int32_t *mode,
                    uint64_t *dbg16);
+int mpn_debug_conv1_block(mpn_ctx *ctx, const float *x, int64_t N, int64_t H, int64_t W, const float *w1, const float *b1,
+                          const float *w2, const float *b2, int32_t fused, int32_t iters, uint16_t *pool_hi, uint16_t *pool_lo,
+                          double *ms_per_launch);
+int mpn_debug_conv1_block_smem(int32_t *bytes);
 int mpn_debug_plan(int64_t N, int64_t Cin, int64_t H, int64_t W, int64_t Cout, int32_t k, int32_t stride, int32_t pad,
                    int32_t per_roi, int32_t sm_count, int32_t *out);
 int mpn_debug_fp8(const float *h, int64_t n_samples, int64_t sample_elems, int32_t *e_out, uint8_t *q_out);
diff --git a/multipathnet_b200/_lib.py b/multipathnet_b200/_lib.py
--- a/multipathnet_b200/_lib.py
+++ b/multipathnet_b200/_lib.py
@@ -201,6 +201,9 @@
     "mpn_linear_bench": (C.c_int, [_vp, C.c_int64, C.c_int64, C.c_int64, C.c_int32, C.c_int32, C.c_int32, C.POINTER(C.c_double), _i32p, _i32p]),
     "mpn_conv_bench": (C.c_int, [_vp, C.c_int64, C.c_int64, C.c_int64, C.c_int64, C.c_int64, C.c_int32, C.c_int32, C.c_int32, C.c_int32,
                                  C.POINTER(C.c_double), _i32p, _i32p, _i32p, C.POINTER(C.c_uint64)]),
+    "mpn_debug_conv1_block": (C.c_int, [_vp, _vp, C.c_int64, C.c_int64, C.c_int64, _vp, _vp, _vp, _vp, C.c_int32, C.c_int32, _vp, _vp,
+                                        C.POINTER(C.c_double)]),
+    "mpn_debug_conv1_block_smem": (C.c_int, [_i32p]),
     "mpn_debug_plan": (C.c_int, [C.c_int64, C.c_int64, C.c_int64, C.c_int64, C.c_int64, C.c_int32, C.c_int32, C.c_int32, C.c_int32, C.c_int32, _i32p]),
     "mpn_debug_fp8": (C.c_int, [_vp, C.c_int64, C.c_int64, _vp, _vp]),
     "mpn_gemm_check": (C.c_int, [_vp, _vp, _vp, _vp, C.c_int64, C.c_int64, C.c_int64, C.c_int32, C.c_int32, _vp]),
@@ -533,6 +536,17 @@
                                            C.byref(mode), dbg), "mpn_conv_bench")
         return ms.value, bn.value, cg.value, mode.value, [int(x) for x in dbg]
 
+    def conv1_block(self, x, w1, b1, w2, b2, fused: bool, iters: int = 0):
+        x = _f32(x)
+        n, _, h, w = x.shape
+        hi = np.zeros((n, (h + 1) // 2, (w + 1) // 2, 64), np.uint16)
+        lo = np.zeros_like(hi)
+        ms = C.c_double(0.0)
+        args = [_f32(a) for a in (w1, b1, w2, b2)]
+        self.check(self.lib.mpn_debug_conv1_block(self.h, _ptr(x), n, h, w, *[_ptr(a) for a in args], 1 if fused else 0, iters,
+                                                  _ptr(hi), _ptr(lo), C.byref(ms)), "mpn_debug_conv1_block")
+        return hi, lo, (ms.value if iters > 0 else None)
+
     def conv_check(self, x, w, bias=None, stride=1, pad=0, relu=False, impl=0) -> np.ndarray:
         x, w = _f32(x), _f32(w)
         n, cin, h, ww = x.shape
diff --git a/multipathnet_b200/csrc/abi.cu b/multipathnet_b200/csrc/abi.cu
--- a/multipathnet_b200/csrc/abi.cu
+++ b/multipathnet_b200/csrc/abi.cu
@@ -831,6 +831,63 @@
   return MPN_OK;
 }
 
+int mpn_debug_conv1_block(mpn_ctx *ctx, const float *x, int64_t N, int64_t H, int64_t W, const float *w1, const float *b1,
+                          const float *w2, const float *b2, int32_t fused, int32_t iters, uint16_t *pool_hi, uint16_t *pool_lo,
+                          double *ms_per_launch) {
+  if (!ctx) return MPN_ERR_ARG;
+  MPN_CUDA(ctx, cudaSetDevice(ctx->device));
+  MPN_CHECK_ARG(ctx, x && w1 && b1 && w2 && b2 && N > 0 && H > 0 && W > 0 && N * H * W < (1ll << 30) && iters >= 0 &&
+                     (fused == 0 || fused == 1), "bad arguments");
+  const int64_t Hp = (H + 1) / 2, Wp = (W + 1) / 2;
+  const size_t nx = (size_t)(N * 3 * H * W), ny = (size_t)(N * H * W * 64), np = (size_t)(N * Hp * Wp * 64);
+  Arena a{ctx};
+  size_t o_x = a.reserve(4 * nx), o_w1 = a.reserve(4 * 64 * 27), o_b1 = a.reserve(4 * 64), o_w2 = a.reserve(4 * 64 * 64 * 9),
+         o_b2 = a.reserve(4 * 64), o_wh = a.reserve(2 * 64 * 576), o_wl = a.reserve(2 * 64 * 576),
+         o_yh = a.reserve(fused ? 0 : 2 * ny), o_yl = a.reserve(fused ? 0 : 2 * ny), o_ph = a.reserve(2 * np), o_pl = a.reserve(2 * np);
+  MPN_TRY(a.commit());
+  MPN_CUDA(ctx, cudaMemcpyAsync(a.at<float>(o_x), x, 4 * nx, cudaMemcpyHostToDevice, ctx->stream));
+  MPN_CUDA(ctx, cudaMemcpyAsync(a.at<float>(o_w1), w1, 4 * 64 * 27, cudaMemcpyHostToDevice, ctx->stream));
+  MPN_CUDA(ctx, cudaMemcpyAsync(a.at<float>(o_b1), b1, 4 * 64, cudaMemcpyHostToDevice, ctx->stream));
+  MPN_CUDA(ctx, cudaMemcpyAsync(a.at<float>(o_w2), w2, 4 * 64 * 64 * 9, cudaMemcpyHostToDevice, ctx->stream));
+  MPN_CUDA(ctx, cudaMemcpyAsync(a.at<float>(o_b2), b2, 4 * 64, cudaMemcpyHostToDevice, ctx->stream));
+  MPN_TRY(mpn_weight_permute_split_launch(ctx, a.at<float>(o_w2), 64, 64, 3, 3, a.at<__nv_bfloat16>(o_wh), a.at<__nv_bfloat16>(o_wl), 0));
+  DTensor y;
+  y.hi = fused ? nullptr : a.at<__nv_bfloat16>(o_yh); y.lo = fused ? nullptr : a.at<__nv_bfloat16>(o_yl);
+  y.N = N; y.H = H; y.W = W; y.C = 64; y.ld = 64;
+  ConvProblem p;
+  p.x = y; p.w_hi = a.at<__nv_bfloat16>(o_wh); p.w_lo = a.at<__nv_bfloat16>(o_wl); p.bias = a.at<float>(o_b2);
+  p.Cout = 64; p.kh = p.kw = 3; p.stride = 1; p.pad = 1; p.relu = 1;
+  p.y.N = N; p.y.H = H; p.y.W = W; p.y.C = 64; p.y.ld = 64;
+  p.pool.hi = a.at<__nv_bfloat16>(o_ph); p.pool.lo = a.at<__nv_bfloat16>(o_pl);
+  p.pool.N = N; p.pool.H = Hp; p.pool.W = Wp; p.pool.C = 64; p.pool.ld = 64; p.pool_only = 1;
+  if (fused) { p.x.hi = a.at<__nv_bfloat16>(o_wh); p.x.lo = a.at<__nv_bfloat16>(o_wl); }
+  ConvPlan pl;
+  MPN_TRY(conv_tc_plan(ctx, p, pl));
+  auto run = [&]() -> int {
+    if (fused) return conv1_block_launch(ctx, a.at<float>(o_x), (int)N, (int)H, (int)W, a.at<float>(o_w1), a.at<float>(o_b1), 1, p, pl);
+    MPN_TRY(conv1_tc_launch(ctx, a.at<float>(o_x), (int)N, (int)H, (int)W, a.at<float>(o_w1), a.at<float>(o_b1), 1, y));
+    return conv_tc_launch(ctx, p, pl);
+  };
+  MPN_TRY(run());
+  if (iters > 0) {
+    for (int i = 0; i < 2; ++i) MPN_TRY(run());
+    cudaEvent_t e0, e1;
+    MPN_CUDA(ctx, cudaEventCreate(&e0)); MPN_CUDA(ctx, cudaEventCreate(&e1));
+    MPN_CUDA(ctx, cudaEventRecord(e0, ctx->stream));
+    for (int i = 0; i < iters; ++i) MPN_TRY(run());
+    MPN_CUDA(ctx, cudaEventRecord(e1, ctx->stream));
+    MPN_CUDA(ctx, cudaEventSynchronize(e1));
+    float ms = 0.f;
+    MPN_CUDA(ctx, cudaEventElapsedTime(&ms, e0, e1));
+    cudaEventDestroy(e0); cudaEventDestroy(e1);
+    if (ms_per_launch) *ms_per_launch = (double)ms / iters;
+  }
+  if (pool_hi) MPN_CUDA(ctx, cudaMemcpyAsync(pool_hi, p.pool.hi, 2 * np, cudaMemcpyDeviceToHost, ctx->stream));
+  if (pool_lo) MPN_CUDA(ctx, cudaMemcpyAsync(pool_lo, p.pool.lo, 2 * np, cudaMemcpyDeviceToHost, ctx->stream));
+  MPN_CUDA(ctx, cudaStreamSynchronize(ctx->stream));
+  return MPN_OK;
+}
+
 int mpn_gemm_check(mpn_ctx *ctx, const float *A, const float *B, const float *bias, int64_t M, int64_t N, int64_t K,
                    int32_t relu, int32_t impl, float *C) {
   if (!ctx) return MPN_ERR_ARG;
diff --git a/multipathnet_b200/csrc/conv_gemm.cuh b/multipathnet_b200/csrc/conv_gemm.cuh
--- a/multipathnet_b200/csrc/conv_gemm.cuh
+++ b/multipathnet_b200/csrc/conv_gemm.cuh
@@ -49,6 +49,9 @@
                             DTensor &y, const float *w_host = nullptr, const float *bias_host = nullptr);
 int conv1_tc_launch(mpn_ctx *ctx, const float *x_nchw, int N, int H, int W, const float *w_dev, const float *bias_dev, int relu,
                     DTensor &y);
+int conv1_block_launch(mpn_ctx *ctx, const float *x_nchw, int N, int H, int W, const float *w1_dev, const float *b1_dev,
+                       int relu1, const ConvProblem &p2, const ConvPlan &pl2);
+int conv1_block_smem_bytes();
 double conv_flops(const ConvProblem &p);
 int mpn_fp8_quantize_launch(mpn_ctx *ctx, const DTensor &x, uint8_t *q8, int *exps);
 int mpn_fp8_weight_launch(mpn_ctx *ctx, const __nv_bfloat16 *w_hi, int64_t rows, int64_t K, int64_t rows_pad, uint8_t *q8, int *exps);
diff --git a/multipathnet_b200/csrc/gemm_tc.cu b/multipathnet_b200/csrc/gemm_tc.cu
--- a/multipathnet_b200/csrc/gemm_tc.cu
+++ b/multipathnet_b200/csrc/gemm_tc.cu
@@ -481,6 +481,22 @@
   }
 }
 
+__device__ __forceinline__ void conv1_stage_b(const float *__restrict__ w, uint8_t *sB, int tid, int nthreads) {
+  for (int i = tid; i < 64 * 4; i += nthreads) {
+    const int row = i >> 2, j = i & 3;
+    uint32_t hh[4], ll[4];
+#pragma unroll
+    for (int q = 0; q < 4; ++q) {
+      const int k0 = j * 8 + 2 * q;
+      const float v0 = (k0 < 27) ? __ldg(w + row * 27 + k0) : 0.f, v1 = (k0 + 1 < 27) ? __ldg(w + row * 27 + k0 + 1) : 0.f;
+      split_bf16x2(v0, v1, hh[q], ll[q]);
+    }
+    const uint32_t off = (uint32_t)row * 128u + (uint32_t)((j ^ (row & 7)) * 16);
+    *reinterpret_cast<uint4 *>(sB + off) = make_uint4(hh[0], hh[1], hh[2], hh[3]);
+    *reinterpret_cast<uint4 *>(sB + 64 * 128 + off) = make_uint4(ll[0], ll[1], ll[2], ll[3]);
+  }
+}
+
 __global__ void __launch_bounds__(C1_THREADS, 2)
 conv1_tc_kernel(const float *__restrict__ x, int N, int H, int W, const float *__restrict__ w, const float *__restrict__ bias,
                 int relu, __nv_bfloat16 *__restrict__ out_hi, __nv_bfloat16 *__restrict__ out_lo) {
@@ -496,19 +512,7 @@
   asm volatile("griddepcontrol.wait;" ::: "memory");
   asm volatile("griddepcontrol.launch_dependents;" ::: "memory");
   const int c0 = 2 * (lane & 3);
-  for (int i = tid; i < 64 * 4; i += C1_THREADS) {
-    const int row = i >> 2, j = i & 3;
-    uint32_t hh[4], ll[4];
-#pragma unroll
-    for (int q = 0; q < 4; ++q) {
-      const int k0 = j * 8 + 2 * q;
-      const float v0 = (k0 < 27) ? __ldg(w + row * 27 + k0) : 0.f, v1 = (k0 + 1 < 27) ? __ldg(w + row * 27 + k0 + 1) : 0.f;
-      split_bf16x2(v0, v1, hh[q], ll[q]);
-    }
-    const uint32_t off = (uint32_t)row * 128u + (uint32_t)((j ^ (row & 7)) * 16);
-    *reinterpret_cast<uint4 *>(sB + off) = make_uint4(hh[0], hh[1], hh[2], hh[3]);
-    *reinterpret_cast<uint4 *>(sB + 64 * 128 + off) = make_uint4(ll[0], ll[1], ll[2], ll[3]);
-  }
+  conv1_stage_b(w, sB, tid, C1_THREADS);
   const int brow = tid & 127, bhalf = tid >> 7;
   float in[16];
   conv1_gather(x, (int)blockIdx.x * BM + brow, pixels, H, W, bhalf, in);
@@ -572,6 +576,208 @@
         }
       conv1_store_plane(so, v, plane ? out_lo : out_hi, pix0, pixels, lane);
     }
+  }
+}
+
+constexpr int CB_WG = 2;
+constexpr int CB_THREADS = 128 * CB_WG;
+constexpr int CB_B2_TAP = 2 * 64 * 128;
+constexpr int CB_B2_BYTES = 9 * CB_B2_TAP;
+constexpr int CB_WIN = 3 * 12 * 12;
+constexpr int CB_WIN_REGS = (CB_WIN + 127) / 128;
+constexpr int CB_HALO = 100;
+constexpr int CB_PIX_WORDS = 36;
+constexpr int CB_HALO_BYTES = 2 * CB_HALO * CB_PIX_WORDS * 4;
+static_assert(CB_HALO_BYTES >= 4 * EPI_WARP_BYTES, "the epilogue buffers live in the halo buffer");
+constexpr int CB_SMEM = CB_B2_BYTES + C1_B_BYTES + CB_WG * CB_HALO_BYTES + CB_WG * CB_WIN * 4 + 1024 ;
+static_assert(CB_SMEM <= 227 * 1024, "first block: shared memory beyond the 227 KB per CTA");
+
+struct Conv1BlockParams {
+  const float *x; int N, H, W;
+  const float *w1, *b1; int relu1;
+  const __nv_bfloat16 *w2_hi, *w2_lo;
+};
+
+__device__ __forceinline__ void cb_bar(int wg) {
+  asm volatile("bar.sync %0, 128;" ::"r"(wg + 1) : "memory");
+}
+
+__device__ __forceinline__ float cb_window_value(const Conv1BlockParams &c, int n, int y0, int x0, int i) {
+  if (i >= CB_WIN) return 0.f;
+  const int ci = i / 144, rem = i - ci * 144, wy = rem / 12, wx = rem - wy * 12;
+  const int y = y0 - 2 + wy, x = x0 - 2 + wx;
+  return (y >= 0 && y < c.H && x >= 0 && x < c.W) ? __ldg(c.x + (((size_t)n * 3 + ci) * c.H + y) * c.W + x) : 0.f;
+}
+
+__global__ void __launch_bounds__(CB_THREADS, 1)
+conv1_block_kernel(const Conv1BlockParams c, const TcParams p) {
+  extern __shared__ uint8_t smem_raw[];
+  uint8_t *smem = reinterpret_cast<uint8_t *>((reinterpret_cast<uintptr_t>(smem_raw) + 1023) & ~(uintptr_t)1023);
+  uint8_t *sB2 = smem, *sB1 = smem + CB_B2_BYTES;
+  const int tid = threadIdx.x, wg = tid >> 7, t = tid & 127, w = t >> 5, lane = tid & 31;
+  float *win = reinterpret_cast<float *>(sB1 + C1_B_BYTES + CB_WG * CB_HALO_BYTES) + wg * CB_WIN;
+  uint32_t *halo = reinterpret_cast<uint32_t *>(sB1 + C1_B_BYTES + wg * CB_HALO_BYTES);
+  const uint32_t so = smem_u32(halo) + (uint32_t)(w * EPI_WARP_BYTES);
+  asm volatile("griddepcontrol.wait;" ::: "memory");
+  asm volatile("griddepcontrol.launch_dependents;" ::: "memory");
+  for (int i = tid; i < 9 * 64 * 8; i += CB_THREADS) {
+    const int tap = i / 512, row = (i >> 3) & 63, j = i & 7;
+    const size_t src = (size_t)row * (9 * 64) + tap * 64 + j * 8;
+    const uint32_t off = (uint32_t)(tap * CB_B2_TAP + row * 128 + ((j ^ (row & 7)) * 16));
+    *reinterpret_cast<uint4 *>(sB2 + off) = __ldg(reinterpret_cast<const uint4 *>(c.w2_hi + src));
+    *reinterpret_cast<uint4 *>(sB2 + off + 64 * 128) = __ldg(reinterpret_cast<const uint4 *>(c.w2_lo + src));
+  }
+  conv1_stage_b(c.w1, sB1, tid, CB_THREADS);
+  asm volatile("fence.proxy.async.shared::cta;" ::: "memory");
+  __syncthreads();
+
+  const int r0 = lane >> 2, cq = lane & 3;
+  int koff[8];
+#pragma unroll
+  for (int e = 0; e < 8; ++e) {
+    const int k = 16 * (e >> 2) + 8 * ((e >> 1) & 1) + 2 * cq + (e & 1);
+    const int ci = k / 9, r = (k / 3) % 3, q = k % 3;
+    koff[e] = k < 27 ? ci * 144 + r * 12 + q : -1;
+  }
+  const uint64_t b1_hi = make_smem_desc(smem_u32(sB1)), b1_lo = make_smem_desc(smem_u32(sB1) + 64 * 128);
+  const int units = 2 * p.units;
+  const int stride = (int)gridDim.x * CB_WG;
+  int unit = (int)blockIdx.x * CB_WG + wg;
+  float pre[CB_WIN_REGS];
+  auto unit_origin = [&](int u, UnitPos &up, int &y0, int &x0) {
+    up = unit_pos(p, u >> 1);
+    y0 = up.thi * 16 + 8 * (u & 1); x0 = up.twi * 8;
+  };
+  if (unit < units) {
+    UnitPos up; int y0, x0;
+    unit_origin(unit, up, y0, x0);
+#pragma unroll
+    for (int q = 0; q < CB_WIN_REGS; ++q) pre[q] = cb_window_value(c, up.tni, y0, x0, t + 128 * q);
+  }
+  for (; unit < units; unit += stride) {
+    UnitPos up; int y0, x0;
+    unit_origin(unit, up, y0, x0);
+    const int half = unit & 1;
+    cb_bar(wg);
+#pragma unroll
+    for (int q = 0; q < CB_WIN_REGS; ++q)
+      if (t + 128 * q < CB_WIN) win[t + 128 * q] = pre[q];
+    cb_bar(wg);
+    if (unit + stride < units) {
+      UnitPos un; int yn, xn;
+      unit_origin(unit + stride, un, yn, xn);
+#pragma unroll
+      for (int q = 0; q < CB_WIN_REGS; ++q) pre[q] = cb_window_value(c, un.tni, yn, xn, t + 128 * q);
+    }
+    uint32_t a1h[2][4], a1l[2][4];
+    float acc1[32];
+#pragma unroll 1
+    for (int b = 0; b < 2; ++b) {
+      int base[2];
+#pragma unroll
+      for (int i = 0; i < 2; ++i) {
+        const int q = min(64 * b + 16 * w + r0 + 8 * i, CB_HALO - 1);
+        base[i] = (q / 10) * 12 + q % 10;
+      }
+#pragma unroll
+      for (int s2 = 0; s2 < 2; ++s2)
+#pragma unroll
+        for (int h = 0; h < 2; ++h)
+#pragma unroll
+          for (int i = 0; i < 2; ++i) {
+            const int e = 4 * s2 + 2 * h;
+            const float v0 = koff[e] >= 0 ? win[base[i] + koff[e]] : 0.f;
+            const float v1 = koff[e + 1] >= 0 ? win[base[i] + koff[e + 1]] : 0.f;
+            split_bf16x2(v0, v1, a1h[s2][2 * h + i], a1l[s2][2 * h + i]);
+          }
+#pragma unroll
+      for (int i = 0; i < 32; ++i) acc1[i] = 0.f;
+      wgmma_fence();
+#pragma unroll
+      for (int s2 = 0; s2 < 2; ++s2) {
+        const uint64_t adv = (uint64_t)((s2 * 16 * 2) >> 4);
+        wgmma_bf16_n64_rs(acc1, a1l[s2], b1_hi + adv, s2 ? 1u : 0u);
+        wgmma_bf16_n64_rs(acc1, a1h[s2], b1_lo + adv, 1u);
+        wgmma_bf16_n64_rs(acc1, a1h[s2], b1_hi + adv, 1u);
+      }
+      wgmma_commit();
+      wgmma_wait<0>();
+      wgmma_fence_acc(acc1); wgmma_fence_regs(a1h); wgmma_fence_regs(a1l);
+#pragma unroll
+      for (int i = 0; i < 2; ++i) {
+        const int q = 64 * b + 16 * w + r0 + 8 * i;
+        const int py = y0 - 1 + q / 10, px = x0 - 1 + q % 10;
+        const bool ok = py >= 0 && py < c.H && px >= 0 && px < c.W;
+        uint32_t hv[8], lv[8];
+#pragma unroll
+        for (int j = 0; j < 8; ++j) {
+          const float2 bb = __ldg(reinterpret_cast<const float2 *>(c.b1 + 8 * j + 2 * cq));
+          float f0 = acc1[4 * j + 2 * i] + bb.x, f1 = acc1[4 * j + 2 * i + 1] + bb.y;
+          if (c.relu1) { f0 = fmaxf(f0, 0.f); f1 = fmaxf(f1, 0.f); }
+          split_bf16x2(f0, f1, hv[j], lv[j]);
+          if (!ok) { hv[j] = 0u; lv[j] = 0u; }
+        }
+        if (q < CB_HALO) {
+          uint4 *dh = reinterpret_cast<uint4 *>(halo + q * CB_PIX_WORDS + 8 * cq);
+          uint4 *dl = reinterpret_cast<uint4 *>(halo + (CB_HALO + q) * CB_PIX_WORDS + 8 * cq);
+          dh[0] = make_uint4(hv[0], hv[1], hv[2], hv[3]); dh[1] = make_uint4(hv[4], hv[5], hv[6], hv[7]);
+          dl[0] = make_uint4(lv[0], lv[1], lv[2], lv[3]); dl[1] = make_uint4(lv[4], lv[5], lv[6], lv[7]);
+        }
+      }
+    }
+    cb_bar(wg);
+    float acc[32];
+#pragma unroll
+    for (int i = 0; i < 32; ++i) acc[i] = 0.f;
+    uint32_t a2h[2][4][4], a2l[2][4][4];
+    auto load_a2 = [&](int tap, uint32_t (&ah)[4][4], uint32_t (&al)[4][4]) {
+      const int khi = tap / 3, kwi = tap - 3 * khi;
+#pragma unroll
+      for (int i = 0; i < 2; ++i) {
+        const int q = (2 * w + i + khi) * 10 + r0 + kwi;
+#pragma unroll
+        for (int pl = 0; pl < 2; ++pl) {
+          const uint4 *src = reinterpret_cast<const uint4 *>(halo + (pl * CB_HALO + q) * CB_PIX_WORDS + 8 * cq);
+          const uint4 u0 = src[0], u1 = src[1];
+          const uint32_t v[8] = {u0.x, u0.y, u0.z, u0.w, u1.x, u1.y, u1.z, u1.w};
+#pragma unroll
+          for (int j = 0; j < 8; ++j) (pl ? al : ah)[j >> 1][2 * (j & 1) + i] = v[j];
+        }
+      }
+    };
+    auto conv12 = [&](int tap, uint32_t (&ah)[4][4], uint32_t (&al)[4][4]) {
+      const uint32_t bt = smem_u32(sB2) + (uint32_t)(tap * CB_B2_TAP);
+      const uint64_t b2_hi = make_smem_desc(bt), b2_lo = make_smem_desc(bt + 64 * 128);
+      wgmma_fence();
+#pragma unroll
+      for (int s2 = 0; s2 < 4; ++s2) {
+        const uint64_t adv = (uint64_t)((s2 * 16 * 2) >> 4);
+        wgmma_bf16_n64_rs(acc, al[s2], b2_hi + adv, (tap == 0 && s2 == 0) ? 0u : 1u);
+        wgmma_bf16_n64_rs(acc, ah[s2], b2_lo + adv, 1u);
+        wgmma_bf16_n64_rs(acc, ah[s2], b2_hi + adv, 1u);
+      }
+      wgmma_commit();
+    };
+    auto step = [&](int tap, uint32_t (&ch)[4][4], uint32_t (&cl)[4][4], uint32_t (&nh)[4][4], uint32_t (&nl)[4][4]) {
+      conv12(tap, ch, cl);
+      if (tap < 8) {
+        wgmma_wait<1>();
+        wgmma_fence_regs(nh); wgmma_fence_regs(nl);
+        load_a2(tap + 1, nh, nl);
+      }
+    };
+    load_a2(0, a2h[0], a2l[0]);
+#pragma unroll 1
+    for (int tap = 0; tap < 8; tap += 2) {
+      step(tap, a2h[0], a2l[0], a2h[1], a2l[1]);
+      step(tap + 1, a2h[1], a2l[1], a2h[0], a2l[0]);
+    }
+    step(8, a2h[0], a2l[0], a2h[1], a2l[1]);
+    wgmma_wait<0>();
+    wgmma_fence_acc(acc);
+    wgmma_fence_regs(a2h[0]); wgmma_fence_regs(a2l[0]); wgmma_fence_regs(a2h[1]); wgmma_fence_regs(a2l[1]);
+    cb_bar(wg);
+    tile_epilogue<64, OperandScheme::BF16X3>(p, up, acc, half, w, lane, so);
   }
 }
 
@@ -703,6 +909,50 @@
   if (tc_use_pdl()) { attr[na].id = cudaLaunchAttributeProgrammaticStreamSerialization; attr[na].val.programmaticStreamSerializationAllowed = 1; ++na; }
   cfg.attrs = attr; cfg.numAttrs = na;
   MPN_CUDA(ctx, cudaLaunchKernelEx(&cfg, conv1_tc_kernel, x_nchw, N, H, W, w_dev, bias_dev, relu, y.hi, y.lo));
+  MPN_LAUNCHED(ctx);
+  return MPN_OK;
+}
+
+int conv1_block_smem_bytes() { return CB_SMEM; }
+
+int conv1_block_launch(mpn_ctx *ctx, const float *x_nchw, int N, int H, int W, const float *w1_dev, const float *b1_dev,
+                       int relu1, const ConvProblem &p2, const ConvPlan &pl2) {
+  MpnProfScope prof_scope__(ctx, MPN_CAT_CONV_TC);
+  MPN_CHECK_ARG(ctx, pl2.valid && pl2.mode == 1 && pl2.BN == 64 && pl2.splitk == 1 && pl2.ops == OperandScheme::BF16X3 &&
+                     pl2.tiles_n == 1 && pl2.tn == 1 && pl2.th == 16 && pl2.tw == 8,
+                "conv1_block: conv1_2 must have a BF16X3 mode-1 plan with 64-wide tiles");
+  MPN_CHECK_ARG(ctx, p2.x.C == 64 && p2.Cout == 64 && p2.kh == 3 && p2.kw == 3 && p2.stride == 1 && p2.pad == 1 &&
+                     !p2.bf16 && !p2.fp8 && !p2.w16 && !p2.res.hi && p2.w_hi && p2.w_lo && p2.bias,
+                "conv1_block: conv1_2 must be a 3x3 / pad 1 64 -> 64 convolution with a bias, default numerics");
+  MPN_CHECK_ARG(ctx, p2.pool.hi && p2.pool.lo && p2.pool_only && p2.pool.fmt == 0 && p2.pool.ld % 8 == 0 &&
+                     p2.pool.N == N && p2.pool.H == (H + 1) / 2 && p2.pool.W == (W + 1) / 2 && p2.y.H == H && p2.y.W == W,
+                "conv1_block: conv1_2's output must be pooled only (2x2/2 ceil) into split bf16 planes");
+  MPN_CHECK_ARG(ctx, w1_dev && b1_dev, "conv1_block: conv1_1's weights and bias are needed");
+  if (!ctx->tc_attr_set[11]) {
+    MPN_CUDA(ctx, cudaFuncSetAttribute(conv1_block_kernel, cudaFuncAttributeMaxDynamicSharedMemorySize, CB_SMEM));
+    ctx->tc_attr_set[11] = 1;
+  }
+  Conv1BlockParams c;
+  c.x = x_nchw; c.N = N; c.H = H; c.W = W; c.w1 = w1_dev; c.b1 = b1_dev; c.relu1 = relu1;
+  c.w2_hi = p2.w_hi; c.w2_lo = p2.w_lo;
+  TcParams tp;
+  memset(&tp, 0, sizeof(tp));
+  tp.N = N; tp.Ho = H; tp.Wo = W; tp.Cout = 64; tp.kh = tp.kw = 3; tp.stride = 1; tp.pad = 1; tp.cblocks = 1;
+  tp.tn = pl2.tn; tp.th = pl2.th; tp.tw = pl2.tw;
+  tp.tiles_img = pl2.tiles_img; tp.tiles_h = pl2.tiles_h; tp.tiles_w = pl2.tiles_w; tp.tiles_n = 1;
+  tp.bias = p2.bias; tp.relu = p2.relu; tp.splitk = 1; tp.kb_per_split = 9; tp.acc_scale = 1.f;
+  tp.pool_hi = p2.pool.hi; tp.pool_lo = p2.pool.lo; tp.pool_ld = p2.pool.ld; tp.Hp = (int)p2.pool.H; tp.Wp = (int)p2.pool.W;
+  const long long tiles = (long long)pl2.tiles_img * pl2.tiles_h * pl2.tiles_w;
+  MPN_CHECK_ARG(ctx, tiles > 0 && 2 * tiles < (1ll << 31), "conv1_block: grid size out of range");
+  tp.units = (int)tiles;
+  cudaLaunchConfig_t cfg = {};
+  cfg.gridDim = dim3((unsigned)std::min<long long>((2 * tiles + CB_WG - 1) / CB_WG, ctx->sm_count));
+  cfg.blockDim = dim3(CB_THREADS); cfg.dynamicSmemBytes = (size_t)CB_SMEM; cfg.stream = ctx->stream;
+  cudaLaunchAttribute attr[1];
+  int na = 0;
+  if (tc_use_pdl()) { attr[na].id = cudaLaunchAttributeProgrammaticStreamSerialization; attr[na].val.programmaticStreamSerializationAllowed = 1; ++na; }
+  cfg.attrs = attr; cfg.numAttrs = na;
+  MPN_CUDA(ctx, cudaLaunchKernelEx(&cfg, conv1_block_kernel, c, tp));
   MPN_LAUNCHED(ctx);
   return MPN_OK;
 }
@@ -898,6 +1148,12 @@
   return launch_ops(ctx, pl, tp);
 }
 
+extern "C" int mpn_debug_conv1_block_smem(int32_t *bytes) {
+  if (!bytes) return MPN_ERR_ARG;
+  *bytes = CB_SMEM;
+  return MPN_OK;
+}
+
 extern "C" int mpn_debug_plan(int64_t N, int64_t Cin, int64_t H, int64_t W, int64_t Cout, int32_t k, int32_t stride, int32_t pad,
                               int32_t per_roi, int32_t sm_count, int32_t *out) {
   if (!out || N <= 0 || Cin <= 0 || Cin % 8 || H <= 0 || W <= 0 || Cout <= 0 || k <= 0 || stride < 1 || stride > 2 || pad < 0 || sm_count < 2 ||
diff --git a/multipathnet_b200/csrc/model.cu b/multipathnet_b200/csrc/model.cu
--- a/multipathnet_b200/csrc/model.cu
+++ b/multipathnet_b200/csrc/model.cu
@@ -113,6 +113,7 @@
   DTensor in, out;
   bool fused_pool = false, pool_only = false;
   DTensor pool_out_t;
+  bool first_block = false;
   bool quant = false;
 };
 
@@ -180,6 +181,7 @@
   int merged_w = -1, merged_b = -1;
   bool merged_stale = false;
   std::set<int> elided_slots;
+  int first_block_slot = -1; const float *first_block_image = nullptr;
   double trunk_flops = 0, head_flops = 0;
   struct Pyramid { std::vector<std::unique_ptr<DevBuf>> lv; int nlev = 1; };
   std::map<int, Pyramid> pyramids;
@@ -425,6 +427,25 @@
       c.fused_pool = true; c.pool_only = !other_reader; c.pool_out_t = q.out;
     }
   }
+  if (m->trunk_exec.size() >= 3) {
+    LayerExec &a = m->trunk_exec[0]; const LayerExec &b = m->trunk_exec[1];
+    const mpn_layer &A = a.L, &B = b.L;
+    const char *e1 = getenv("MPN_CONV1_TC");
+    bool ok = !(e1 && e1[0] == '0') && a.is_direct && A.cin == 3 && A.cout == 64 && A.kh == 3 && A.kw == 3 &&
+              A.stride == 1 && A.pad == 1 && A.bias >= 0 && a.out.ld == 64 &&
+              B.kind == MPN_LAYER_CONV && !b.is_direct && B.in_slot == A.out_slot && B.cin == 64 && B.cout == 64 &&
+              B.kh == 3 && B.kw == 3 && B.stride == 1 && B.pad == 1 && B.residual_slot < 0 && B.bias >= 0 &&
+              b.fused_pool && b.pool_only && b.plan.mode == 1 && b.plan.BN == 64 && b.plan.splitk == 1 &&
+              b.plan.ops == OperandScheme::BF16X3 && !b.prob.bf16 && !b.prob.fp8 && !b.prob.w16 && !b.quant;
+    for (size_t j = 2; ok && j < m->trunk_exec.size(); ++j) {
+      const mpn_layer &L2 = m->trunk_exec[j].L;
+      if (L2.in_slot == A.out_slot || L2.residual_slot == A.out_slot) ok = false;
+    }
+    for (const mpn_tower &T : m->towers)
+      for (int l = 0; l < T.n_levels; ++l) if (T.level_slot[l] == A.out_slot) ok = false;
+    if (m->train && m->train->trunk_from == 1) ok = false;
+    a.first_block = ok;
+  }
   for (const mpn_tower &T : m->towers)
     for (int l = 0; l < T.n_levels; ++l) {
       const int slot = T.level_slot[l];
@@ -449,12 +470,41 @@
   return MPN_OK;
 }
 
+static int run_first_layer(mpn_model *m, LayerExec &e, const float *image_dev) {
+  const mpn_layer &L = e.L;
+  const float *bias = L.bias >= 0 ? (const float *)m->weights[L.bias]->f32.p : nullptr;
+  return conv_direct_nchw_launch(m->ctx, image_dev, 1, L.cin, (int)e.in.H, (int)e.in.W,
+                                 (const float *)m->weights[L.weight]->f32.p, bias, L.cout, L.kh, L.kw, L.stride,
+                                 L.pad, L.relu, e.out,
+                                 m->w_host_small[L.weight].empty() ? nullptr : m->w_host_small[L.weight].data(),
+                                 (L.bias >= 0 && !m->w_host_small[L.bias].empty()) ? m->w_host_small[L.bias].data() : nullptr);
+}
+
+static int materialise_slot(mpn_model *m, int slot) {
+  if (slot != m->first_block_slot) return MPN_OK;
+  MPN_TRY(run_first_layer(m, m->trunk_exec[0], m->first_block_image));
+  m->first_block_slot = -1;
+  return MPN_OK;
+}
+
 int run_trunk(mpn_model *m, const float *image_dev) {
   mpn_ctx *ctx = m->ctx;
   m->elided_slots.clear();
+  m->first_block_slot = -1; m->first_block_image = nullptr;
   for (size_t li = 0; li < m->trunk_exec.size(); ++li) {
     LayerExec &e = m->trunk_exec[li];
     const mpn_layer &L = e.L;
+    if (e.first_block && m->conv_impl == 0) {
+      const LayerExec &c2 = m->trunk_exec[li + 1];
+      ConvProblem pf = c2.prob;
+      pf.pool = c2.pool_out_t; pf.pool_only = 1;
+      MPN_TRY(conv1_block_launch(ctx, image_dev, 1, (int)e.in.H, (int)e.in.W, (const float *)m->weights[L.weight]->f32.p,
+                                 (const float *)m->weights[L.bias]->f32.p, L.relu, pf, c2.plan));
+      m->first_block_slot = L.out_slot; m->first_block_image = image_dev;
+      m->elided_slots.insert(c2.L.out_slot);
+      li += 2;
+      continue;
+    }
     if (e.fused_pool && m->conv_impl == 0) {
       if (e.quant) MPN_TRY(mpn_fp8_quantize_launch(ctx, e.prob.x, const_cast<uint8_t *>(e.prob.x8), const_cast<int *>(e.prob.x8_exp)));
       ConvProblem pf = e.prob;
@@ -466,12 +516,7 @@
     }
     if (L.kind == MPN_LAYER_CONV) {
       if (e.is_direct) {
-        const float *bias = L.bias >= 0 ? (const float *)m->weights[L.bias]->f32.p : nullptr;
-        MPN_TRY(conv_direct_nchw_launch(ctx, image_dev, 1, L.cin, (int)e.in.H, (int)e.in.W,
-                                        (const float *)m->weights[L.weight]->f32.p, bias, L.cout, L.kh, L.kw, L.stride,
-                                        L.pad, L.relu, e.out,
-                                        m->w_host_small[L.weight].empty() ? nullptr : m->w_host_small[L.weight].data(),
-                                        (L.bias >= 0 && !m->w_host_small[L.bias].empty()) ? m->w_host_small[L.bias].data() : nullptr));
+        MPN_TRY(run_first_layer(m, e, image_dev));
       } else {
         MPN_TRY(run_conv(m, e));
       }
@@ -1230,6 +1275,7 @@
   MPN_CHECK_ARG(ctx, m->trunk_valid && slot > 0 && m->trunk_slots.count(slot), "unknown trunk slot or no trunk forward yet");
   MPN_CHECK_ARG(ctx, !m->elided_slots.count(slot),
                 "trunk slot was fused into the following max pool and never written (mpn_model_set_conv_impl(m, 2) disables the fusion)");
+  MPN_TRY(materialise_slot(m, slot));
   const DTensor &t = m->trunk_slots[slot];
   const int64_t n = t.N * t.C * t.H * t.W;
   if (C) *C = (int32_t)t.C; if (H) *H = (int32_t)t.H; if (W) *W = (int32_t)t.W;
@@ -1253,6 +1299,7 @@
   if (tower == -1) {
     MPN_CHECK_ARG(ctx, m->trunk_valid && slot > 0 && m->trunk_slots.count(slot), "unknown trunk slot or no trunk forward yet");
     MPN_CHECK_ARG(ctx, !m->elided_slots.count(slot), "trunk slot was fused into the following max pool and never written");
+    MPN_TRY(materialise_slot(m, slot));
     t = &m->trunk_slots[slot];
     for (const LayerExec &e : m->trunk_exec)
       if (e.L.kind == MPN_LAYER_CONV && !e.is_direct && e.prob.fp8 && e.L.in_slot == slot) qb = m->trunk_q8[slot].get();
diff --git a/multipathnet_b200/csrc/wgmma.cuh b/multipathnet_b200/csrc/wgmma.cuh
--- a/multipathnet_b200/csrc/wgmma.cuh
+++ b/multipathnet_b200/csrc/wgmma.cuh
@@ -55,6 +55,13 @@
   if constexpr (N == 64) wgmma_e4m3_n64(d, da, db, scale_d); else wgmma_e4m3_n128(d, da, db, scale_d);
 }
 
+__device__ __forceinline__ void wgmma_bf16_n64_rs(float (&d)[32], const uint32_t (&a)[4], uint64_t db, uint32_t scale_d) {
+  asm volatile("{\n.reg .pred p;\nsetp.ne.b32 p, %37, 0;\n"
+               "wgmma.mma_async.sync.aligned.m64n64k16.f32.bf16.bf16 {%0, %1, %2, %3, %4, %5, %6, %7, %8, %9, %10, %11, %12, %13, %14, %15, %16, %17, %18, %19, %20, %21, %22, %23, %24, %25, %26, %27, %28, %29, %30, %31}, {%32, %33, %34, %35}, %36, p, 1, 1, 0;\n}\n"
+               : "+f"(d[0]), "+f"(d[1]), "+f"(d[2]), "+f"(d[3]), "+f"(d[4]), "+f"(d[5]), "+f"(d[6]), "+f"(d[7]), "+f"(d[8]), "+f"(d[9]), "+f"(d[10]), "+f"(d[11]), "+f"(d[12]), "+f"(d[13]), "+f"(d[14]), "+f"(d[15]), "+f"(d[16]), "+f"(d[17]), "+f"(d[18]), "+f"(d[19]), "+f"(d[20]), "+f"(d[21]), "+f"(d[22]), "+f"(d[23]), "+f"(d[24]), "+f"(d[25]), "+f"(d[26]), "+f"(d[27]), "+f"(d[28]), "+f"(d[29]), "+f"(d[30]), "+f"(d[31])
+               : "r"(a[0]), "r"(a[1]), "r"(a[2]), "r"(a[3]), "l"(db), "r"(scale_d));
+}
+
 template <int N, bool F16> __device__ __forceinline__ void wgmma_nk16(float (&d)[N / 2], uint64_t da, uint64_t db, uint32_t scale_d) {
   if constexpr (F16) {
     if constexpr (N == 64) wgmma_f16_n64(d, da, db, scale_d); else if constexpr (N == 128) wgmma_f16_n128(d, da, db, scale_d); else wgmma_f16_n256(d, da, db, scale_d);
@@ -69,3 +76,9 @@
 #pragma unroll
   for (int i = 0; i < R; ++i) asm volatile("" : "+f"(d[i])::"memory");
 }
+template <int R> __device__ __forceinline__ void wgmma_fence_regs(uint32_t (&a)[R][4]) {
+#pragma unroll
+  for (int i = 0; i < R; ++i)
+#pragma unroll
+    for (int k = 0; k < 4; ++k) asm volatile("" : "+r"(a[i][k])::"memory");
+}
```

Result: faster. 422,700, median of 6 (+1.6%).
